# ksahlin/IsoCon

Measured on AMD Instinct MI355X. Metric: read x candidate alignments/sec (NN-graph build, 50k x 2.5kb reads), higher is better.
Workload: dtype u64; 1 GPU; C3: 50000 synthetic CCS reads (50000 unique), ~2500 bp, 10 isoforms, seed 30001; 1-set NN graph; edges=78526, graph_digest=65944c838d76a6c9, parallelism=single GPU

## Files before the change

isocon_amd/csrc/common.hpp:

```cpp
#pragma once
#include <hip/hip_runtime.h>
#include <stdint.h>
#include <string>
#include "../../include/isocon_hip.h"

namespace isocon {

struct DevStore {
    const uint64_t *planes;
    const uint64_t *il;
    const int32_t *lens;
    uint32_t n;
    uint32_t nchunks;
};

struct QMap {
    uint32_t begin, end, stride, block_log2;
    __host__ __device__ __forceinline__ uint32_t block() const { return 1u << block_log2; }
    __host__ __device__ __forceinline__ uint64_t entry(uint32_t s) const
    {
        return (uint64_t)begin + (uint64_t)(s >> block_log2) * stride + (s & (block() - 1u));
    }
    __host__ __device__ __forceinline__ bool slot_of(uint32_t x, uint32_t &s) const
    {
        if (x < begin || x >= end) return false;
        const uint32_t d = x - begin, b = d / stride, r = d - b * stride;
        s = (b << block_log2) + r;
        return r < block();
    }
    __host__ __device__ __forceinline__ bool owns(uint32_t x) const { uint32_t s; return slot_of(x, s); }
    __host__ __device__ __forceinline__ uint32_t count() const
    {
        if (end <= begin) return 0u;
        const uint32_t span = end - begin, full = span / stride, rem = span - full * stride;
        return (full << block_log2) + (rem < block() ? rem : block());
    }
    __host__ __device__ __forceinline__ bool same(const QMap &o) const { return begin == o.begin && end == o.end && stride == o.stride && block_log2 == o.block_log2; }
};

extern thread_local std::string g_last_error;

#define ISO_HIP_CHECK(expr)                                                                    \
    do {                                                                                       \
        hipError_t _e = (expr);                                                                \
        if (_e != hipSuccess) {                                                                \
            g_last_error = std::string(#expr) + ": " + hipGetErrorString(_e);                  \
            return ISOCON_E_HIP;                                                               \
        }                                                                                      \
    } while (0)

__device__ __forceinline__ int32_t wave_min_i32(int32_t v)
{
#pragma unroll
    for (int o = 32; o > 0; o >>= 1) {
        const int32_t w = __shfl_xor(v, o, 64);
        v = w < v ? w : v;
    }
    return v;
}

__device__ __forceinline__ int32_t wave_max_i32(int32_t v)
{
#pragma unroll
    for (int o = 32; o > 0; o >>= 1) {
        const int32_t w = __shfl_xor(v, o, 64);
        v = w > v ? w : v;
    }
    return v;
}

__device__ __forceinline__ unsigned long long block_exscan_1024(unsigned long long s, unsigned long long *wave_sums, unsigned long long *total)
{
    const uint32_t lane = threadIdx.x & 63u, wave = threadIdx.x >> 6;
    unsigned long long inc = s;
#pragma unroll
    for (uint32_t d = 1; d < 64; d <<= 1) {
        const unsigned long long o = __shfl_up(inc, d, 64);
        if (lane >= d) inc += o;
    }
    if (lane == 63) wave_sums[wave] = inc;
    __syncthreads();
    unsigned long long off = inc - s, tot = 0;
    for (uint32_t w = 0; w < 16; ++w) {
        if (w < wave) off += wave_sums[w];
        tot += wave_sums[w];
    }
    *total = tot;
    return off;
}

static constexpr uint32_t SCAN_TILE = 2048;

template <int SHIFT>
__global__ __launch_bounds__(256) void k_scan_tiles(const uint32_t *__restrict__ in, uint32_t n, uint32_t *__restrict__ tmp, unsigned long long *__restrict__ tile_sum)
{
    __shared__ unsigned long long wave_sums[4];
    const uint32_t base = blockIdx.x * SCAN_TILE + threadIdx.x * 8u;
    uint32_t v[8];
#pragma unroll
    for (int j = 0; j < 8; ++j) {
        const uint32_t x = base + j < n ? in[base + j] : 0u;
        v[j] = SHIFT ? (x + (1u << SHIFT) - 1u) >> SHIFT : x;
    }
    uint32_t s = 0;
#pragma unroll
    for (int j = 0; j < 8; ++j) s += v[j];
    const uint32_t lane = threadIdx.x & 63u, wave = threadIdx.x >> 6;
    uint32_t inc = s;
#pragma unroll
    for (uint32_t d = 1; d < 64; d <<= 1) {
        const uint32_t o = __shfl_up(inc, d, 64);
        if (lane >= d) inc += o;
    }
    if (lane == 63) wave_sums[wave] = inc;
    __syncthreads();
    uint32_t off = inc - s;
    for (uint32_t w = 0; w < wave; ++w) off += (uint32_t)wave_sums[w];
#pragma unroll
    for (int j = 0; j < 8; ++j) {
        if (base + j < n) tmp[base + j] = off;
        off += v[j];
    }
    if (threadIdx.x == 255) tile_sum[blockIdx.x] = (unsigned long long)off;
}

template <class OUT>
__global__ __launch_bounds__(256) void k_scan_finish(const uint32_t *__restrict__ tmp, uint32_t n, const unsigned long long *__restrict__ tile_sum, uint32_t n_tiles,
                                                      OUT *__restrict__ out, unsigned long long *__restrict__ total_out)
{
    __shared__ unsigned long long part[4];
    unsigned long long s = 0, all = 0;
    for (uint32_t b = threadIdx.x; b < n_tiles; b += 256u) {
        const unsigned long long t = tile_sum[b];
        if (b < blockIdx.x) s += t;
        all += t;
    }
    const bool last = blockIdx.x + 1 == gridDim.x;
    unsigned long long r = last ? all : s, r2 = s;
#pragma unroll
    for (int o = 32; o > 0; o >>= 1) { r += __shfl_xor(r, o, 64); r2 += __shfl_xor(r2, o, 64); }
    if ((threadIdx.x & 63u) == 0) part[threadIdx.x >> 6] = r2;
    __syncthreads();
    const unsigned long long before = part[0] + part[1] + part[2] + part[3];
    __syncthreads();
    if ((threadIdx.x & 63u) == 0) part[threadIdx.x >> 6] = r;
    __syncthreads();
    const uint32_t base = blockIdx.x * SCAN_TILE + threadIdx.x * 8u;
#pragma unroll
    for (int j = 0; j < 8; ++j)
        if (base + j < n) out[base + j] = (OUT)(before + tmp[base + j]);
    if (last && threadIdx.x == 0) {
        const unsigned long long tot = part[0] + part[1] + part[2] + part[3];
        out[n] = (OUT)tot;
        if (total_out) *total_out = tot;
    }
}

__device__ __forceinline__ int32_t uniform_i32(int32_t v) { return __builtin_amdgcn_readfirstlane(v); }

__device__ __forceinline__ int32_t load_relaxed_agent(const int32_t *p)
{
    return __hip_atomic_load(p, __ATOMIC_RELAXED, __HIP_MEMORY_SCOPE_AGENT);
}

}
```

isocon_amd/csrc/isocon_hip.hip:

```cpp
#include <algorithm>
#include <chrono>
#include <cstdio>
#include <cstdlib>
#include <cstring>
#include <numeric>
#include <string>
#include <memory>
#include <mutex>
#include <thread>
#include <vector>

#include "common.hpp"
#include "ed_band.hpp"
#include "ed_full.hpp"
#include "qgram_mm.hpp"
#include "nn.hpp"
#include "nn_list.hpp"
#include "nn_filter.hpp"
#include "nn_finalize.hpp"
#include "nn_finalize_host.hpp"
#include "partition_host.hpp"
#include "sg.hpp"
#include "msa.hpp"
#include "hw.hpp"
#include "hw_tiles.hpp"
#include "hw_full.hpp"
#include "nw_path.hpp"
#include "ed_lanes.hpp"
#include "ed_bytes.hpp"
#include "nn2_depth.hpp"
#include "readtab.hpp"
#include "edgevar.hpp"
#include "pbound.hpp"

namespace isocon {
thread_local std::string g_last_error;
}

using namespace isocon;

static bool variant_lookup(const char *name, std::string *value)
{
    const char *e = getenv("ISOCON_DEBUG_VARIANT");
    if (!e) return false;
    const size_t ln = strlen(name);
    for (const char *p = e; *p;) {
        const char *q = strchr(p, ',');
        const size_t len = q ? (size_t)(q - p) : strlen(p);
        if (len >= ln && strncmp(p, name, ln) == 0 && (len == ln || p[ln] == '=')) {
            if (value) *value = len > ln ? std::string(p + ln + 1, len - ln - 1) : std::string();
            return true;
        }
        p += len + (q ? 1 : 0);
    }
    return false;
}
static bool variant(const char *name) { return variant_lookup(name, nullptr); }
static const char *variant_value(const char *name)
{
    thread_local std::string ring[8];
    thread_local unsigned at = 0;
    std::string &slot = ring[at++ % 8];
    return variant_lookup(name, &slot) ? slot.c_str() : nullptr;
}

struct BoundTag {
    bool valid = false, has_order = false;
    uint64_t serial = 0;
    QMap map = {0, 0, 0, 0};
    uint32_t depth = 0;
    int32_t kcap = 0;
    unsigned long long lb_total = 0;
};
struct MsaBuilt {
    enum By { NONE, SINGLE, BATCH } by = NONE;
    uint64_t serial = 0;
    uint32_t n_parts = 0, n_rows = 0;
    std::vector<uint32_t> ncols, col_base, first_row;
    std::vector<unsigned long long> m_off;
};
struct HeldHits { uint64_t store_serial = 0; uint64_t rows = 0; };

struct ScratchPool {
    struct Slot { void *p = nullptr; size_t cap = 0; };
    Slot slots[160];
    BoundTag bound_tag;
    HeldHits held_hits;
    MsaBuilt msa;
    void *get(int idx, size_t bytes)
    {
        Slot &s = slots[idx];
        if (bytes == 0) bytes = 16;
        if (s.cap < bytes) {
            if (s.p) (void)hipFree(s.p);
            s.p = nullptr; s.cap = 0;
            const size_t want = bytes + bytes / 8;
            if (hipMalloc(&s.p, want) == hipSuccess) s.cap = want;
            else if (hipMalloc(&s.p, bytes) == hipSuccess) s.cap = bytes;
            else { s.p = nullptr; (void)hipGetLastError(); }
        }
        return s.p;
    }
    void release()
    {
        for (Slot &s : slots) { if (s.p) (void)hipFree(s.p); s.p = nullptr; s.cap = 0; }
        bound_tag = BoundTag();
        held_hits = HeldHits();
        msa = MsaBuilt();
    }
};

enum {
    SLOT_ED_TS = 0, SLOT_ED_IDS, SLOT_ED_K, SLOT_ED_OUT, SLOT_FULL_A, SLOT_FULL_B, SLOT_FULL_K, SLOT_FULL_OUT,
    SLOT_NN_BEST, SLOT_NN_QF, SLOT_NN_TF, SLOT_NN_HITS, SLOT_NN_HITCOUNT, SLOT_NN_STATS, SLOT_NN_TS, SLOT_NN_IDS, SLOT_NN_PLANES2, SLOT_NN_PERM, SLOT_NN_IL, SLOT_NN_IL2, SLOT_NN_HITS2, SLOT_NN_HITCOUNT2, SLOT_NN_QPROF, SLOT_NN_QSUM, SLOT_NN_LB, SLOT_NN_LBROW, SLOT_NN_LBLEN, SLOT_NN_SLOTORDER, SLOT_NN_LBCHUNKS, SLOT_NN_ROWMIN, SLOT_NN_COLMIN, SLOT_NN_SEED_A, SLOT_NN_SEED_B, SLOT_NN_SEED_N, SLOT_NN_LBT, SLOT_NN_LBT_OFF, SLOT_NN_LBT_SLO, SLOT_NN_LBT_LEN, SLOT_NN_LBT_PAD, SLOT_NN_SCORE, SLOT_NN_LDEST, SLOT_NN_FIN_HITS, SLOT_NN_FIN_CNT, SLOT_NN_FIN_START, SLOT_NN_FIN_CUR, SLOT_NN_FIN_NB, SLOT_NN_FIN_LEN2, SLOT_NN_FIN_OUT, SLOT_NN_FIN_FLAG, SLOT_NN_FIN_BEST, SLOT_NN_ACC_HITS, SLOT_NN_LTOT, SLOT_NN_LCHUNKS, SLOT_NN_LIST, SLOT_NN_LPA, SLOT_NN_LPB, SLOT_NN_TEXT2, SLOT_NN_LTASKS, SLOT_NN_RECORD,
    SLOT_NN2_STATE, SLOT_NN2_TPOS, SLOT_NN2_EXC, SLOT_NN2_CTR, SLOT_NN2_PAIRS, SLOT_NN2_WIDE,
    SLOT_SG_PAIRS, SLOT_SG_R, SLOT_SG_TRACE, SLOT_SG_END, SLOT_SG_OPS, SLOT_SG_CNT, SLOT_SG_RES, SLOT_SG_OFF, SLOT_SG_DENSE, SLOT_SG_BOUND, SLOT_SG_AOFF, SLOT_SG_ALNA, SLOT_SG_ALNB,
    SLOT_MSA_IN, SLOT_MSA_OUT, SLOT_MSA_DEG, SLOT_MSA_COUNTS, SLOT_MSA_MAJ, SLOT_MSA_FLAGS, SLOT_MSA_TOT, SLOT_MSA_NCAND, SLOT_MSA_LEN, SLOT_MSA_OFF, SLOT_MSA_PACKED, SLOT_MSA_ROWS, SLOT_MSA_OPS, SLOT_MSA_OPTR, SLOT_MSA_LONGEST, SLOT_MSA_WIDTH, SLOT_MSA_CSLOT, SLOT_MSA_LTOT, SLOT_MSA_WIDE, SLOT_MSA_PROW, SLOT_MSA_PCOL, SLOT_MSA_PPTR, SLOT_MSA_PBYTES, SLOT_MSA_PART, SLOT_MSA_FIRST, SLOT_MSA_LM, SLOT_MSA_SBASE, SLOT_MSA_NCOLS, SLOT_MSA_MOFF, SLOT_MSA_CBASE, SLOT_MSA_CBP, SLOT_MSA_CBC, SLOT_MSA_CBR,
    SLOT_HW_Q, SLOT_HW_T, SLOT_HW_K, SLOT_HW_OUT, SLOT_HW_TRACE, SLOT_HW_CTR, SLOT_HW_TILEQ, SLOT_HW_LANES, SLOT_HW_PQ, SLOT_HW_KEY, SLOT_HW_HIST, SLOT_HW_CURSOR, SLOT_HW_TBASE, SLOT_HW_CLS,
    SLOT_PACK_ASCII, SLOT_PACK_OFF, SLOT_PACK_BAD, SLOT_PACK_HIST, SLOT_PACK_FLAGS, SLOT_EB_A, SLOT_EB_B, SLOT_EB_K, SLOT_EB_OUT, SLOT_EB_ROWS, SLOT_SCAN_TMP, SLOT_SCAN_SUMS,
    SLOT_RT_REF, SLOT_RT_IN, SLOT_RT_OUT,
    SLOT_EV_IN, SLOT_EV_OUT, SLOT_EV_SNIP,
    SLOT_PB_IN, SLOT_PB_OUT,
    SLOT_NWP_Q, SLOT_NWP_T, SLOT_NWP_ED, SLOT_NWP_TOFF, SLOT_NWP_ROFF, SLOT_NWP_REV, SLOT_NWP_RUNS, SLOT_NWP_FOFF, SLOT_NWP_OPS, SLOT_NWP_START, SLOT_NWP_COLS,
    SLOT_COUNT
};
static_assert(SLOT_COUNT <= 160, "ScratchPool::slots too small");

static ScratchPool g_scratch;

static uint64_t g_store_serial = 0;

struct isocon_store {
    uint64_t serial = ++g_store_serial;
    DevStore dev;
    explicit isocon_store(bool private_scratch = false) : own_pool(private_scratch ? new ScratchPool() : nullptr), pool(own_pool ? *own_pool : g_scratch) {}
    std::unique_ptr<ScratchPool> own_pool;
    ScratchPool &pool;
    std::vector<int32_t> lens;
    uint64_t device_bytes = 0;
    uint64_t *d_planes = nullptr;
    char alphabet[4] = {'A', 'C', 'G', 'T'};
    bool acgt = true;
    uint8_t *d_bytes = nullptr;
    uint64_t *d_boff = nullptr;
    uint64_t bytes_base = 0;
    std::vector<uint8_t> exc;
    std::vector<uint32_t> exc_count;
    uint32_t n_exc = 0;
    bool is_exc(uint32_t i) const { return n_exc != 0 && exc[i] != 0; }
    int32_t *d_lens = nullptr;
    int32_t maxlen = 0;
    uint64_t last_host_waits = 0;
};

namespace {

struct PinnedStage {
    void *p = nullptr;
    size_t cap = 0;
    void *get(size_t bytes)
    {
        if (cap < bytes) {
            if (p) (void)hipHostFree(p);
            p = nullptr; cap = 0;
            if (hipHostMalloc(&p, bytes, hipHostMallocDefault) == hipSuccess) cap = bytes;
            else { p = nullptr; (void)hipGetLastError(); }
        }
        return p;
    }
    void release() { if (p) (void)hipHostFree(p); p = nullptr; cap = 0; }
};
static PinnedStage g_stage;
static constexpr size_t kStageBytes = (size_t)32 << 20;
static constexpr uint64_t kPackWaves = (uint64_t)1 << 25;
static constexpr size_t kStageMin = (size_t)32 << 10;

static std::vector<std::pair<const char *, size_t>> g_pinned;
static bool is_pinned(const void *p, size_t bytes)
{
    for (const auto &r : g_pinned)
        if ((const char *)p >= r.first && (const char *)p + bytes <= r.first + r.second) return true;
    return false;
}

static thread_local uint64_t g_host_waits = 0;
static hipError_t memcpy_wait(void *dst, const void *src, size_t bytes, hipMemcpyKind kind) { ++g_host_waits; return hipMemcpy(dst, src, bytes, kind); }
static hipError_t memset_wait(void *dst, int value, size_t bytes) { ++g_host_waits; return hipMemset(dst, value, bytes); }
static hipError_t device_wait() { ++g_host_waits; return hipDeviceSynchronize(); }

static hipError_t copy_d2h(void *dst, const void *dsrc, size_t bytes)
{
    if (bytes < kStageMin || is_pinned(dst, bytes)) return memcpy_wait(dst, dsrc, bytes, hipMemcpyDeviceToHost);
    char *st = static_cast<char *>(g_stage.get(kStageBytes));
    if (!st) return memcpy_wait(dst, dsrc, bytes, hipMemcpyDeviceToHost);
    for (size_t off = 0; off < bytes; off += kStageBytes) {
        const size_t len = std::min(kStageBytes, bytes - off);
        const hipError_t e = memcpy_wait(st, static_cast<const char *>(dsrc) + off, len, hipMemcpyDeviceToHost);
        if (e != hipSuccess) return e;
        memcpy(static_cast<char *>(dst) + off, st, len);
    }
    return hipSuccess;
}

static hipError_t copy_h2d(void *ddst, const void *src, size_t bytes)
{
    if (bytes < kStageMin || is_pinned(src, bytes)) return memcpy_wait(ddst, src, bytes, hipMemcpyHostToDevice);
    char *st = static_cast<char *>(g_stage.get(kStageBytes));
    if (!st) return memcpy_wait(ddst, src, bytes, hipMemcpyHostToDevice);
    for (size_t off = 0; off < bytes; off += kStageBytes) {
        const size_t len = std::min(kStageBytes, bytes - off);
        memcpy(st, static_cast<const char *>(src) + off, len);
        const hipError_t e = memcpy_wait(static_cast<char *>(ddst) + off, st, len, hipMemcpyHostToDevice);
        if (e != hipSuccess) return e;
    }
    return hipSuccess;
}

struct SideUpload {
    hipStream_t stream = nullptr;
    hipEvent_t before = nullptr, done = nullptr;
    PinnedStage pinned;
    bool in_flight = false;
    bool ready()
    {
        if (stream) return true;
        if (hipStreamCreateWithFlags(&stream, hipStreamNonBlocking) != hipSuccess) { stream = nullptr; (void)hipGetLastError(); return false; }
        if (hipEventCreateWithFlags(&before, hipEventDisableTiming) != hipSuccess || hipEventCreateWithFlags(&done, hipEventDisableTiming) != hipSuccess) {
            (void)hipGetLastError();
            release();
            return false;
        }
        return true;
    }
    void settle()
    {
        if (!in_flight) return;
        if (hipEventQuery(done) != hipSuccess || hipStreamQuery(stream) != hipSuccess) { (void)hipGetLastError(); ++g_host_waits; (void)hipStreamSynchronize(stream); }
        in_flight = false;
    }
    void release()
    {
        if (stream) { (void)hipStreamSynchronize(stream); (void)hipStreamDestroy(stream); }
        if (before) (void)hipEventDestroy(before);
        if (done) (void)hipEventDestroy(done);
        stream = nullptr; before = done = nullptr; in_flight = false;
        pinned.release();
    }
};
static SideUpload g_side;

struct DevBuf {
    void *p = nullptr;
    ScratchPool *pool = nullptr;
    int slot = -1;
    DevBuf() {}
    DevBuf(ScratchPool *pl, int sl) : pool(pl), slot(sl) {}
    DevBuf(const DevBuf &) = delete;
    DevBuf &operator=(const DevBuf &) = delete;
    ~DevBuf() { if (p && !pool) (void)hipFree(p); }
    template <class T> T *as() { return static_cast<T *>(p); }
    int alloc(size_t bytes)
    {
        if (pool) {
            p = pool->get(slot, bytes);
            if (!p) { g_last_error = "hipMalloc(scratch slot " + std::to_string(slot) + ", " + std::to_string(bytes) + " B) failed"; return ISOCON_E_HIP; }
            return ISOCON_OK;
        }
        if (p) { (void)hipFree(p); p = nullptr; }
        ISO_HIP_CHECK(hipMalloc(&p, bytes ? bytes : 16));
        return ISOCON_OK;
    }
};

template <int SHIFT, class OUT>
static int device_exscan(ScratchPool *pl, const uint32_t *d_in, uint32_t n, OUT *d_out)
{
    DevBuf d_tmp(pl, SLOT_SCAN_TMP), d_sums(pl, SLOT_SCAN_SUMS);
    const uint32_t tiles = std::max<uint32_t>(1, (n + SCAN_TILE - 1) / SCAN_TILE);
    int rc;
    if ((rc = d_tmp.alloc((size_t)std::max<uint32_t>(n, 1) * 4)) || (rc = d_sums.alloc((size_t)tiles * 8))) return rc;
    hipLaunchKernelGGL((k_scan_tiles<SHIFT>), dim3(tiles), dim3(256), 0, 0, d_in, n, d_tmp.as<uint32_t>(), d_sums.as<unsigned long long>());
    hipLaunchKernelGGL((k_scan_finish<OUT>), dim3(tiles), dim3(256), 0, 0, d_tmp.as<uint32_t>(), n, d_sums.as<unsigned long long>(), tiles, d_out, (unsigned long long *)nullptr);
    ISO_HIP_CHECK(hipGetLastError());
    return ISOCON_OK;
}

struct EventPool {
    std::mutex mu;
    std::vector<hipEvent_t> idle;
    hipEvent_t get()
    {
        {
            std::lock_guard<std::mutex> g(mu);
            if (!idle.empty()) { hipEvent_t e = idle.back(); idle.pop_back(); return e; }
        }
        hipEvent_t e = nullptr;
        if (hipEventCreate(&e) != hipSuccess) { (void)hipGetLastError(); return nullptr; }
        return e;
    }
    void put(hipEvent_t e)
    {
        if (!e) return;
        std::lock_guard<std::mutex> g(mu);
        idle.push_back(e);
    }
    void release()
    {
        std::lock_guard<std::mutex> g(mu);
        for (hipEvent_t e : idle) (void)hipEventDestroy(e);
        idle.clear();
    }
};
static EventPool g_events;

struct EventTimer {
    struct Interval { hipEvent_t e0, em, e1; float *acc, *marked_acc; };
    std::vector<Interval> pending;
    hipEvent_t e0 = nullptr, em = nullptr;
    float total = 0.f;
    float marked_total = 0.f;
    const bool sync_phases = variant("nn_sync_phases");
    EventTimer() {}
    EventTimer(const EventTimer &) = delete;
    EventTimer &operator=(const EventTimer &) = delete;
    ~EventTimer()
    {
        g_events.put(e0); g_events.put(em);
        for (const Interval &iv : pending) { g_events.put(iv.e0); g_events.put(iv.em); g_events.put(iv.e1); }
    }
    void start()
    {
        g_events.put(em); em = nullptr;
        if (!e0) e0 = g_events.get();
        if (e0) (void)hipEventRecord(e0, 0);
    }
    void mark()
    {
        if (!e0) return;
        if (!em) em = g_events.get();
        if (em) (void)hipEventRecord(em, 0);
    }
    void stop_later(float *acc, float *marked_acc = nullptr)
    {
        if (!e0) return;
        hipEvent_t e1 = g_events.get();
        if (!e1) { g_events.put(e0); g_events.put(em); e0 = em = nullptr; return; }
        (void)hipEventRecord(e1, 0);
        pending.push_back(Interval{e0, em, e1, acc, marked_acc});
        e0 = em = nullptr;
        if (sync_phases) resolve(true);
    }
    void resolve(bool wait_counts = false)
    {
        if (pending.empty()) return;
        hipEvent_t last = pending.back().e1;
        if (wait_counts || hipEventQuery(last) != hipSuccess) { (void)hipGetLastError(); ++g_host_waits; (void)hipEventSynchronize(last); }
        for (const Interval &iv : pending) {
            float ms = 0.f, part = 0.f;
            if (hipEventElapsedTime(&ms, iv.e0, iv.e1) != hipSuccess) { (void)hipGetLastError(); ms = 0.f; }
            total += ms;
            if (iv.acc) *iv.acc += ms;
            if (iv.em) {
                if (hipEventElapsedTime(&part, iv.em, iv.e1) != hipSuccess) { (void)hipGetLastError(); part = 0.f; }
                if (iv.marked_acc) *iv.marked_acc += part; else marked_total += part;
            }
            g_events.put(iv.e0); g_events.put(iv.em); g_events.put(iv.e1);
        }
        pending.clear();
    }
    float stop()
    {
        float ms = 0.f;
        stop_later(&ms);
        resolve(true);
        return ms;
    }
};

struct PackMap { uint8_t sym[4]; };

__global__ __launch_bounds__(256) void k_byte_histogram(const uint8_t *__restrict__ ascii, uint64_t total, unsigned long long *__restrict__ hist)
{
    __shared__ uint32_t h[256];
    h[threadIdx.x] = 0;
    __syncthreads();
    for (uint64_t i = (uint64_t)blockIdx.x * 256 + threadIdx.x; i < total; i += (uint64_t)gridDim.x * 256) atomicAdd(&h[ascii[i]], 1u);
    __syncthreads();
    if (h[threadIdx.x]) atomicAdd(hist + threadIdx.x, (unsigned long long)h[threadIdx.x]);
}

__global__ __launch_bounds__(256) void k_pack_planes(const uint8_t *__restrict__ ascii, const uint64_t *__restrict__ offsets, uint64_t base, uint32_t n,
                                                      uint32_t nchunks, uint64_t *__restrict__ planes, unsigned long long *__restrict__ first_bad, PackMap map,
                                                      uint32_t fold, uint64_t w0)
{
    const uint64_t w = w0 + (uint64_t)blockIdx.x * 4 + (threadIdx.x >> 6);
    if (w >= (uint64_t)nchunks * n) return;
    const uint32_t lane = threadIdx.x & 63;
    const uint32_t chunk = (uint32_t)(w / n), seq = (uint32_t)(w % n);
    const uint64_t off = offsets[seq] - base, len = offsets[seq + 1] - offsets[seq];
    const uint64_t pos = (uint64_t)chunk * 64 + lane;
    int cd = 0;
    bool bad = false;
    if (pos < len) {
        uint8_t ch = ascii[off + pos];
        if (fold && ch >= 'a' && ch <= 'z') ch = (uint8_t)(ch - 32);
        cd = ch == map.sym[0] ? 0 : ch == map.sym[1] ? 1 : ch == map.sym[2] ? 2 : ch == map.sym[3] ? 3 : -1;
        bad = cd < 0 && !fold;
    }
    const unsigned long long lo = __ballot(!bad && (cd & 1)), hi = __ballot(!bad && (cd & 2)), bm = __ballot(bad);
    if (lane == 0) {
        planes[((size_t)chunk * n + seq) * 2] = lo;
        planes[((size_t)chunk * n + seq) * 2 + 1] = hi;
        if (bm) atomicMin(first_bad, ((unsigned long long)seq << 32) | ((unsigned long long)chunk * 64 + (unsigned long long)(__ffsll((long long)bm) - 1)));
    }
}

}

extern "C" {

const char *isocon_strerror(int status)
{
    switch (status) {
    case ISOCON_OK: return "ok";
    case ISOCON_E_ARG: return "bad argument";
    case ISOCON_E_ALPHABET: return "sequence contains a symbol outside ACGT";
    case ISOCON_E_HIP: return "HIP runtime error";
    case ISOCON_E_CAPACITY: return "output buffer too small";
    case ISOCON_E_NODEVICE: return "no usable GPU";
    case ISOCON_E_UNSUPPORTED: return "unsupported request";
    default: return "unknown status";
    }
}

const char *isocon_last_error(void) { return g_last_error.c_str(); }
// ... 413 lines not shown
            if (!lanes_p.empty()) {
                const size_t np = lanes_p.size();
                std::vector<uint32_t> la(np), lb2(np);
                std::vector<int32_t> lk(np), res(np, -1);
                for (size_t i = 0; i < np; ++i) {
                    const uint64_t p = lanes_p[i];
                    la[i] = a[p]; lb2[i] = b[p];
                    const int32_t kr = k ? k[p] : -1;
                    lk[i] = kr < 0 ? kcap : std::min(kr, kcap);
                }
                DevBuf d_a(&st->pool, SLOT_ED_TS), d_b(&st->pool, SLOT_ED_IDS), d_k(&st->pool, SLOT_ED_K), d_out(&st->pool, SLOT_ED_OUT);
                int rc;
                if ((rc = d_a.alloc(np * 4)) || (rc = d_b.alloc(np * 4)) || (rc = d_k.alloc(np * 4)) || (rc = d_out.alloc(np * 4))) return rc;
                ISO_HIP_CHECK(copy_h2d(d_a.p, la.data(), np * 4));
                ISO_HIP_CHECK(copy_h2d(d_b.p, lb2.data(), np * 4));
                ISO_HIP_CHECK(copy_h2d(d_k.p, lk.data(), np * 4));
                NNParams none;
                memset(&none, 0, sizeof(none));
                tm.start();
                hipLaunchKernelGGL(k_ed_lanes<false>, dim3((unsigned)((np + 255) / 256)), dim3(256), 0, 0, st->dev, none, d_a.as<uint32_t>(), d_b.as<uint32_t>(),
                                   d_k.as<int32_t>(), (uint64_t)np, d_out.as<int32_t>());
                ISO_HIP_CHECK(hipGetLastError());
                tm.stop();
                ISO_HIP_CHECK(copy_d2h(res.data(), d_out.p, np * 4));
                for (size_t i = 0; i < np; ++i) {
                    const uint64_t p = lanes_p[i];
                    const int32_t kr = k ? k[p] : -1;
                    if (res[i] >= 0) out_ed[p] = res[i];
                    else if (kr >= 0 && kr <= kcap) out_ed[p] = -1;
                    else next.push_back(p);
                }
            }
            todo.swap(tiles_p);
        }
        for (int round = 0; round < 2 && !todo.empty(); ++round) {
            std::vector<uint32_t> ts, ids;
            std::vector<int32_t> ks;
            std::vector<uint64_t> slot_pair;
            size_t i = 0;
            while (i < todo.size()) {
                size_t j = i;
                const uint32_t s0 = sh(todo[i]);
                const size_t lim = round == 0 ? 64 : 1;
                while (j < todo.size() && j - i < lim && sh(todo[j]) == s0) ++j;
                ts.push_back(s0);
                for (size_t l = 0; l < 64; ++l) {
                    if (i + l < j) {
                        const uint64_t p = todo[i + l];
                        ids.push_back(ln(p));
                        const int32_t kr = k ? k[p] : -1;
                        ks.push_back(kr < 0 ? kcap : std::min(kr, kcap));
                        slot_pair.push_back(p);
                    } else {
                        ids.push_back(0xffffffffu);
                        ks.push_back(-1);
                        slot_pair.push_back(~(uint64_t)0);
                    }
                }
                i = j;
            }
            std::vector<int32_t> res;
            int rc = run_band_stage(W, st, st->dev, ts, ids, ks, res, tm);
            if (rc) return rc;
            std::vector<uint64_t> retry;
            for (size_t sidx = 0; sidx < slot_pair.size(); ++sidx) {
                const uint64_t p = slot_pair[sidx];
                if (p == ~(uint64_t)0) continue;
                const int32_t r = res[sidx];
                const int32_t kr = k ? k[p] : -1;
                if (r >= 0) out_ed[p] = r;
                else if (r == -2) retry.push_back(p);
                else if (kr >= 0 && kr <= kcap) out_ed[p] = -1;
                else next.push_back(p);
            }
            todo.swap(retry);
        }
        if (!todo.empty()) { g_last_error = "internal: single-lane tile undetermined"; return ISOCON_E_HIP; }
        pending.swap(next);
    }
    if (full_pairs) *full_pairs = pending.size();
    if (!pending.empty()) {
        std::vector<uint32_t> fa, fb;
        std::vector<int32_t> fk, res;
        for (uint64_t p : pending) { fa.push_back(a[p]); fb.push_back(b[p]); fk.push_back(k ? k[p] : -1); }
        int rc = run_full(st, fa, fb, fk, res, tm);
        if (rc) return rc;
        for (size_t i = 0; i < pending.size(); ++i) out_ed[pending[i]] = res[i];
    }
    if (kernel_ms) *kernel_ms = tm.total;
    return ISOCON_OK;
}

}

__global__ __launch_bounds__(256) void k_store_digest(const uint64_t *__restrict__ planes, size_t n_words, const int32_t *__restrict__ lens, uint32_t n,
                                                      unsigned long long *__restrict__ out)
{
    unsigned long long acc = 0;
    const size_t stride = (size_t)gridDim.x * blockDim.x;
    for (size_t i = (size_t)blockIdx.x * blockDim.x + threadIdx.x; i < n_words + n; i += stride) {
        unsigned long long v = i < n_words ? planes[i] : (unsigned long long)(uint32_t)lens[i - n_words];
        v ^= (unsigned long long)i * 0xD6E8FEB86659FD93ull;
        v ^= v >> 32; v *= 0x9E3779B97F4A7C15ull; v ^= v >> 29; v *= 0xBF58476D1CE4E5B9ull; v ^= v >> 32;
        acc += v;
    }
    for (int o = 32; o > 0; o >>= 1) acc += __shfl_xor(acc, o, 64);
    if ((threadIdx.x & 63) == 0 && acc) atomicAdd(out, acc);
}

extern "C" int isocon_store_digest(const isocon_store *s, uint64_t *out)
{
    if (!s || !out) return ISOCON_E_ARG;
    DevBuf d_acc;
    int rc;
    if ((rc = d_acc.alloc(8))) return rc;
    ISO_HIP_CHECK(hipMemset(d_acc.p, 0, 8));
    const size_t n_words = (size_t)s->dev.nchunks * std::max<uint32_t>(s->dev.n, 1) * 2;
    hipLaunchKernelGGL(k_store_digest, dim3(1024), dim3(256), 0, 0, s->d_planes, n_words, s->d_lens, s->dev.n, d_acc.as<unsigned long long>());
    ISO_HIP_CHECK(hipGetLastError());
    ISO_HIP_CHECK(hipMemcpy(out, d_acc.p, 8, hipMemcpyDeviceToHost));
    return ISOCON_OK;
}

extern "C" int isocon_ed_pairs(isocon_store *s, const uint32_t *a, const uint32_t *b, const int32_t *k, uint64_t n_pairs,
                               int32_t *out_ed, float *kernel_ms)
{
    if (!s || (n_pairs && (!a || !b || !out_ed))) return ISOCON_E_ARG;
    if (kernel_ms) *kernel_ms = 0.f;
    if (!n_pairs) return ISOCON_OK;
    return ed_pairs_impl(s, a, b, k, n_pairs, out_ed, kernel_ms, nullptr, false);
}

extern "C" int isocon_qgram_params(int32_t *out)
{
    if (out) { out[0] = QG_Q; out[1] = QG_B0; out[2] = QG_B1; out[3] = QG_CAP; }
    return QM_K;
}

namespace isocon {
int qgram_bounds_for_pairs(isocon_store *s, const uint32_t *a, const uint32_t *b, uint64_t n_pairs, int32_t *out_bound, float *kernel_ms)
{
    const uint32_t n = s->dev.n;
    const uint32_t n_pad = std::max<uint32_t>(QM_TILE, ((n + QM_TILE - 1) / QM_TILE) * QM_TILE);
    DevBuf d_prof(&s->pool, SLOT_NN_QPROF), d_sum(&s->pool, SLOT_NN_QSUM), d_a(&s->pool, SLOT_ED_TS), d_b(&s->pool, SLOT_ED_IDS), d_out(&s->pool, SLOT_ED_OUT);
    int rc;
    if ((rc = d_prof.alloc((size_t)n_pad * (QM_K / 2))) || (rc = d_sum.alloc((size_t)n * 4)) || (rc = d_a.alloc(n_pairs * 4)) || (rc = d_b.alloc(n_pairs * 4)) ||
        (rc = d_out.alloc(n_pairs * 4)))
        return rc;
    s->pool.bound_tag.valid = false;
    ISO_HIP_CHECK(copy_h2d(d_a.p, a, n_pairs * 4));
    ISO_HIP_CHECK(copy_h2d(d_b.p, b, n_pairs * 4));
    EventTimer tm;
    tm.start();
    hipLaunchKernelGGL(k_qgram_profile4, dim3((n + QP_SEQS - 1) / QP_SEQS), dim3(256), 0, 0, s->dev, d_prof.as<uint8_t>(), d_sum.as<uint32_t>(), n_pad);
    ISO_HIP_CHECK(hipGetLastError());
    for (uint64_t at = 0; at < n_pairs; at += (uint64_t)1 << 24) {
        const uint64_t cnt = std::min<uint64_t>((uint64_t)1 << 24, n_pairs - at);
        hipLaunchKernelGGL(k_qgram_lb_pairs, dim3((unsigned)((cnt + 3) / 4)), dim3(256), 0, 0, d_prof.as<uint8_t>(), d_sum.as<uint32_t>(), n_pad, d_a.as<uint32_t>() + at,
                           d_b.as<uint32_t>() + at, cnt, d_out.as<int32_t>() + at);
        ISO_HIP_CHECK(hipGetLastError());
    }
    const float ms = tm.stop();
    if (kernel_ms) *kernel_ms = ms;
    ISO_HIP_CHECK(copy_d2h(out_bound, d_out.p, n_pairs * 4));
    return ISOCON_OK;
}
}

extern "C" int isocon_qgram_bound_pairs(isocon_store *s, const uint32_t *a, const uint32_t *b, uint64_t n_pairs, int32_t *out_bound)
{
    if (!s || (n_pairs && (!a || !b || !out_bound))) return ISOCON_E_ARG;
    if (!n_pairs) return ISOCON_OK;
    if (s->n_exc) { g_last_error = "q-gram bounds are defined on the 2-bit planes: the set holds more than four distinct symbols"; return ISOCON_E_ALPHABET; }
    const uint32_t n = s->dev.n;
    for (uint64_t i = 0; i < n_pairs; ++i)
        if (a[i] >= n || b[i] >= n) { g_last_error = "pair index out of range"; return ISOCON_E_ARG; }
    return qgram_bounds_for_pairs(s, a, b, n_pairs, out_bound, nullptr);
}

extern "C" int isocon_block_bound_pairs(isocon_store *s, const uint32_t *owner, const uint32_t *partner, uint64_t n_pairs, int32_t probe_stride, int32_t *out_count)
{
    if (probe_stride != 4 && probe_stride != 2) return ISOCON_E_ARG;
    if (!s || (n_pairs && (!owner || !partner || !out_count))) return ISOCON_E_ARG;
    if (!n_pairs) return ISOCON_OK;
    if (s->n_exc) { g_last_error = "block bounds are defined on the 2-bit planes: the set holds more than four distinct symbols"; return ISOCON_E_ALPHABET; }
    const uint32_t n = s->dev.n;
    if (n_pairs >= ((uint64_t)1 << 31)) return ISOCON_E_ARG;
    for (uint64_t i = 0; i < n_pairs; ++i)
        if (owner[i] >= n || partner[i] >= n) { g_last_error = "pair index out of range"; return ISOCON_E_ARG; }
    const uint32_t stride = nnf_text2_stride(s->maxlen);
    DevBuf d_text(&s->pool, SLOT_NN_TEXT2), d_a(&s->pool, SLOT_ED_TS), d_b(&s->pool, SLOT_ED_IDS), d_out(&s->pool, SLOT_ED_OUT);
    int rc;
    if ((rc = d_text.alloc((size_t)n * stride * 4)) || (rc = d_a.alloc(n_pairs * 4)) || (rc = d_b.alloc(n_pairs * 4)) || (rc = d_out.alloc(n_pairs * 4))) return rc;
    ISO_HIP_CHECK(copy_h2d(d_a.p, owner, n_pairs * 4));
    ISO_HIP_CHECK(copy_h2d(d_b.p, partner, n_pairs * 4));
    hipLaunchKernelGGL(k_build_text2, dim3(n), dim3(256), 0, 0, s->dev, d_text.as<uint32_t>(), stride);
    hipLaunchKernelGGL(k_nn_block_count_pairs, dim3((unsigned)n_pairs), dim3(256), 0, 0, d_text.as<uint32_t>(), stride, s->dev.lens, d_a.as<uint32_t>(), d_b.as<uint32_t>(), d_out.as<int32_t>(), probe_stride);
    ISO_HIP_CHECK(hipGetLastError());
    ISO_HIP_CHECK(copy_d2h(out_count, d_out.p, n_pairs * 4));
    return ISOCON_OK;
}

extern "C" int isocon_block_filter_chunks(isocon_store *s, const int32_t *thr, uint32_t n_chunks, const uint32_t *owner, const uint8_t *narrow, const uint64_t *chunk_ptr,
                                          const uint32_t *words, int32_t kcap, uint32_t list_min, int32_t second_pass, uint32_t *out_slot, uint32_t *out_count,
                                          uint64_t *out_begin, uint64_t chunks_cap, uint32_t *out_list, uint64_t list_cap, uint32_t *out_pa, uint32_t *out_pb, uint64_t pairs_cap,
                                          uint64_t *out_counters)
{
    if (!s || !out_counters || (second_pass != 0 && second_pass != 1) || list_min == 0) return ISOCON_E_ARG;
    for (int i = 0; i < 9; ++i) out_counters[i] = 0;
    if (!n_chunks) return ISOCON_OK;
    if (!thr || !owner || !narrow || !chunk_ptr || !words || !out_slot || !out_count || !out_begin || !out_list || !out_pa || !out_pb) return ISOCON_E_ARG;
    if (s->n_exc) { g_last_error = "block bounds are defined on the 2-bit planes: the set holds more than four distinct symbols"; return ISOCON_E_ALPHABET; }
    const uint32_t n = s->dev.n;
    if (n >= (1u << 30) || s->maxlen >= 16384) return ISOCON_E_ARG;
    for (uint32_t i = 0; i < n; ++i)
        if (thr[i] < 0 || thr[i] > 64) { g_last_error = "threshold outside 0 .. 64"; return ISOCON_E_ARG; }
    static_assert(NN_LIST_CHUNK + 63 <= NN_STAGE, "a chunk fits the filter's staging buffer");
    if (chunk_ptr[0] != 0) return ISOCON_E_ARG;
    uint32_t n_narrow = 0;
    for (uint32_t c = 0; c < n_chunks; ++c) {
        if (owner[c] >= n || narrow[c] > 1) { g_last_error = "chunk owner out of range"; return ISOCON_E_ARG; }
        if (chunk_ptr[c + 1] <= chunk_ptr[c] || chunk_ptr[c + 1] - chunk_ptr[c] > NN_LIST_CHUNK + 63) { g_last_error = "chunk count outside 1 .. NN_LIST_CHUNK + 63"; return ISOCON_E_ARG; }
        n_narrow += narrow[c];
    }
    const uint64_t total = chunk_ptr[n_chunks];
    for (uint64_t i = 0; i < total; ++i)
        if ((words[i] & 0x3fffffffu) >= n) { g_last_error = "partner index out of range"; return ISOCON_E_ARG; }
    if (chunks_cap < n_chunks || list_cap < total || pairs_cap < total) { g_last_error = "an output capacity below the worst case (every pair kept)"; return ISOCON_E_ARG; }
    const uint64_t cap_in = n_chunks, cap_out = n_chunks;
    const uint64_t tasks_cap = second_pass ? 2 * cap_in + total / 64 + 1 : 0;
    std::vector<uint32_t> meta((size_t)n + NN_META_PAD, 0u);
    for (uint32_t i = 0; i < n; ++i) meta[i] = ((uint32_t)s->lens[i] & 0x3fffu) | ((uint32_t)thr[i] << 14);
    std::vector<NNChunk> chunks(2 * (size_t)cap_in);
    NNPlanTotals tot;
    memset(&tot, 0, sizeof(tot));
    for (uint32_t c = 0; c < n_chunks; ++c) {
        NNChunk ch; ch.slot = owner[c]; ch.count = (uint32_t)(chunk_ptr[c + 1] - chunk_ptr[c]); ch.begin = chunk_ptr[c];
        chunks[narrow[c] ? cap_in + tot.n_chunks_narrow++ : tot.n_chunks++] = ch;
    }
    const uint32_t stride = nnf_text2_stride(s->maxlen);
    DevBuf d_text(&s->pool, SLOT_NN_TEXT2), d_meta(&s->pool, SLOT_NN_LDEST), d_tot(&s->pool, SLOT_NN_LTOT), d_chunks(&s->pool, SLOT_NN_LCHUNKS), d_list(&s->pool, SLOT_NN_LIST),
        d_pa(&s->pool, SLOT_NN_LPA), d_pb(&s->pool, SLOT_NN_LPB), d_tasks(&s->pool, SLOT_NN_LTASKS);
    int rc;
    if ((rc = d_text.alloc((size_t)n * stride * 4)) || (rc = d_meta.alloc(meta.size() * 4)) || (rc = d_tot.alloc(sizeof(NNPlanTotals))) ||
        (rc = d_chunks.alloc((size_t)(2 * cap_in + 2 * cap_out) * sizeof(NNChunk))) || (rc = d_list.alloc((size_t)total * 4)) || (rc = d_pa.alloc((size_t)total * 4)) ||
        (rc = d_pb.alloc((size_t)total * 4)) || (rc = d_tasks.alloc((size_t)std::max<uint64_t>(tasks_cap, 1) * sizeof(NNFTask))))
        return rc;
    ISO_HIP_CHECK(copy_h2d(d_meta.p, meta.data(), meta.size() * 4));
    ISO_HIP_CHECK(copy_h2d(d_tot.p, &tot, sizeof(tot)));
    ISO_HIP_CHECK(copy_h2d(d_chunks.p, chunks.data(), chunks.size() * sizeof(NNChunk)));
    ISO_HIP_CHECK(copy_h2d(d_list.p, words, (size_t)total * 4));
    NNChunk *left = d_chunks.as<NNChunk>() + 2 * cap_in;
    hipLaunchKernelGGL(k_build_text2, dim3(n), dim3(256), 0, 0, s->dev, d_text.as<uint32_t>(), stride);
    ISO_HIP_CHECK(hipGetLastError());
    ISO_HIP_CHECK(nnf_launch_filter(d_text.as<uint32_t>(), stride, s->dev.lens, d_meta.as<uint32_t>(), kcap, d_list.as<uint32_t>(), d_chunks.as<NNChunk>(), cap_in, left, cap_out,
                                    d_pa.as<uint32_t>(), d_pb.as<uint32_t>(), total, d_tot.as<NNPlanTotals>(), list_min, second_pass ? d_tasks.as<NNFTask>() : (NNFTask *)nullptr,
                                    tasks_cap));
    ISO_HIP_CHECK(memcpy_wait(&tot, d_tot.p, sizeof(tot), hipMemcpyDeviceToHost));
    const uint64_t counters[9] = {tot.f_chunks, tot.f_chunks_narrow, tot.n_small, tot.f_rejected, tot.f_rejected2, tot.f_listed, tot.f_narrow_listed, tot.f_tasks, tot.overflow};
    for (int i = 0; i < 9; ++i) out_counters[i] = counters[i];
    if (tot.overflow || tot.f_chunks > cap_in - n_narrow || tot.f_chunks_narrow > n_narrow || tot.n_small > total) { g_last_error = "the block filter left more than it was given"; return ISOCON_E_HIP; }
    std::vector<NNChunk> out((size_t)(tot.f_chunks + tot.f_chunks_narrow));
    if (tot.f_chunks) ISO_HIP_CHECK(copy_d2h(out.data(), left, (size_t)tot.f_chunks * sizeof(NNChunk)));
    if (tot.f_chunks_narrow) ISO_HIP_CHECK(copy_d2h(out.data() + tot.f_chunks, left + cap_out, (size_t)tot.f_chunks_narrow * sizeof(NNChunk)));
    for (size_t i = 0; i < out.size(); ++i) { out_slot[i] = out[i].slot; out_count[i] = out[i].count; out_begin[i] = out[i].begin; }
    ISO_HIP_CHECK(copy_d2h(out_list, d_list.p, (size_t)total * 4));
    if (tot.n_small) {
        ISO_HIP_CHECK(copy_d2h(out_pa, d_pa.p, (size_t)tot.n_small * 4));
        ISO_HIP_CHECK(copy_d2h(out_pb, d_pb.p, (size_t)tot.n_small * 4));
    }
    return ISOCON_OK;
}

#include "nn_context.inc"
#include "nn_bounds.inc"
#include "nn_lists.inc"
#include "nn_main.inc"
#include "nn_wide.inc"
#include "nn_images.inc"
#include "nn_entry.inc"
#include "nn2_depth.inc"
#include "sg_host.inc"
#include "msa_host.inc"
#include "hw_host.inc"
#include "hw_full_host.inc"
#include "nw_path_host.inc"
#include "hw_path_host.inc"
#include "readtab_host.inc"
#include "edgevar_host.inc"
#include "pbound_host.inc"

extern "C" int isocon_partition_ids(uint32_t n, const int32_t *degree, uint64_t n_edges, const uint32_t *edge_a, const uint32_t *edge_b,
                                    const uint32_t *rank, int32_t nbr_tiebreak, uint32_t *out_centre, int64_t *out_weight,
                                    uint64_t *out_member_ptr, uint32_t *out_members, uint32_t *n_parts)
{
    if (!out_member_ptr || !n_parts || (n && (!degree || !rank || !out_centre || !out_weight || !out_members)) || (n_edges && (!edge_a || !edge_b))) return ISOCON_E_ARG;
    return partition_ids_impl(n, degree, n_edges, edge_a, edge_b, rank, nbr_tiebreak, out_centre, out_weight, out_member_ptr, out_members, n_parts);
}
```

isocon_amd/csrc/nn_bounds.inc:

```

namespace {

int NNContext::build_bounds(const QMap &Q, int32_t kcap, NNParams &P, bool want_seeds)
{
    const uint32_t q_begin = Q.begin, q_end = Q.end;
    P.lb = nullptr;
    P.lb_row = nullptr;
    P.slot_order = nullptr;
    if (variant("nn_no_qgram") || n < 2 || n >= (1u << 30) || q_begin >= q_end) return ISOCON_OK;
    if (!want_seeds && st->pool.bound_tag.valid && st->pool.bound_tag.serial == st->serial && st->pool.bound_tag.map.same(Q) &&
        st->pool.bound_tag.depth == depth && st->pool.bound_tag.kcap == kcap) {
        P.lb = static_cast<const uint8_t *>(st->pool.slots[SLOT_NN_LB].p);
        P.lb_row = static_cast<const unsigned long long *>(st->pool.slots[SLOT_NN_LBROW].p);
        if (st->pool.bound_tag.has_order && use_slot_order(Q.count())) P.slot_order = static_cast<const uint32_t *>(st->pool.slots[SLOT_NN_SLOTORDER].p);
        lb_total = st->pool.bound_tag.lb_total;
        return ISOCON_OK;
    }
    st->pool.bound_tag.valid = false;
    const uint32_t nq = Q.count();
    const std::vector<int32_t> &lens = st->lens;
    const uint32_t n_pad = std::max<uint32_t>(QM_TILE, ((n + QM_TILE - 1) / QM_TILE) * QM_TILE);
    const size_t prof_bytes = (size_t)n_pad * (QM_K / 2);
    d_qprof.pool = d_qsum.pool = &st->pool;
    d_qprof.slot = SLOT_NN_QPROF; d_qsum.slot = SLOT_NN_QSUM;
    HostClock bclk;
    {
        size_t free_b = 0;
        if (!free_mem(free_b) || prof_bytes > free_b / 2 + st->pool.slots[SLOT_NN_QPROF].cap) return ISOCON_OK;
        if (d_qprof.alloc(prof_bytes) || d_qsum.alloc((size_t)n * 4)) return ISOCON_OK;
    }
    bclk.lap("bounds: memory check + profile buffers");
    const bool side = !variant("nn_sync_uploads") && g_side.ready() && hipEventRecord(g_side.before, 0) == hipSuccess;
    tm.start();
    hipLaunchKernelGGL(k_qgram_profile4, dim3((n + QP_SEQS - 1) / QP_SEQS), dim3(256), 0, 0, st->dev, d_qprof.as<uint8_t>(), d_qsum.as<uint32_t>(), n_pad);
    ISO_HIP_CHECK(hipGetLastError());
    struct StopTimer { NNContext &c; bool armed = true; ~StopTimer() { if (armed) c.tm.stop_later(&c.stats.bound_kernel_ms); } } stop_timer{*this};
    std::vector<unsigned long long> &off = lb_off_host;
    std::vector<uint32_t> &rlen = lb_len_host;
    off.assign(nq, 0);
    rlen.assign(nq, 0);
    unsigned long long total = 0, sum_rlen = 0;
    uint64_t hi = 0;
    const uint32_t nrb = (nq + QM_TILE - 1) / QM_TILE;
    std::vector<uint64_t> rb_lo(nrb, ~(uint64_t)0), rb_hi(nrb, 0);
    for (uint32_t s = 0; s < nq; ++s) {
        const uint64_t q = Q.entry(s);
        if (hi < q + 1) hi = q + 1;
        while (hi < n && lens[hi] - lens[q] <= kcap) ++hi;
        uint64_t len = hi - q - 1;
        if (len > depth) len = depth;
        const uint64_t pal = (q + 1) & ~(uint64_t)15;
        off[s] = total + (q + 1 - pal);
        rlen[s] = (uint32_t)len;
        sum_rlen += len;
        if (len) {
            total += ((q + 1 + len + 15) & ~(uint64_t)15) - pal;
            rb_lo[s / QM_TILE] = std::min<uint64_t>(rb_lo[s / QM_TILE], q + 1);
            rb_hi[s / QM_TILE] = std::max<uint64_t>(rb_hi[s / QM_TILE], q + len);
        }
    }
    if (total == 0) return ISOCON_OK;
    bclk.lap("bounds: profile launch + rows (host)");
    const unsigned long long totalT = sum_rlen + 30ull * n;
    bclk.lap("bounds: transposed rows (host)");
    size_t free_b = 0;
    const size_t need = (size_t)total + (size_t)totalT + prof_bytes + (size_t)n * 24 + (size_t)nq * 12;
    if (!free_mem(free_b) || need > free_b / 2 + st->pool.slots[SLOT_NN_LB].cap + st->pool.slots[SLOT_NN_QPROF].cap) return ISOCON_OK;
    bclk.lap("bounds: memory check 2");
    std::vector<uint2> tiles;
    for (uint32_t g = 0; g * 4 < nrb; ++g) {
        uint64_t jmin = ~(uint64_t)0, jmax = 0;
        bool any = false;
        for (uint32_t I = g * 4; I < std::min(nrb, g * 4 + 4); ++I)
            if (rb_lo[I] != ~(uint64_t)0) { any = true; jmin = std::min(jmin, rb_lo[I] / QM_TILE); jmax = std::max(jmax, rb_hi[I] / QM_TILE); }
        if (!any) continue;
        for (uint64_t j0 = jmin; j0 <= jmax; j0 += 8)
            for (uint32_t ri = 0; ri < 4; ++ri)
                for (uint32_t cj = 0; cj < 8; ++cj) {
                    const uint32_t I = g * 4 + ri;
                    const uint64_t J = j0 + cj;
                    const bool have = I < nrb && rb_lo[I] != ~(uint64_t)0 && J >= rb_lo[I] / QM_TILE && J <= rb_hi[I] / QM_TILE;
                    tiles.push_back(have ? make_uint2(I, (uint32_t)J) : make_uint2(0xffffffffu, 0xffffffffu));
                }
    }
    while (tiles.size() % 256) tiles.push_back(make_uint2(0xffffffffu, 0xffffffffu));
    if (tiles.size() > 0x7fffffffull) return ISOCON_OK;
    bclk.lap("bounds: tile table (host)");
    d_lb.pool = d_lbrow.pool = d_lblen.pool = &st->pool;
    d_lb.slot = SLOT_NN_LB; d_lbrow.slot = SLOT_NN_LBROW; d_lblen.slot = SLOT_NN_LBLEN;
    int rc;
    if ((rc = d_lb.alloc((size_t)total + 16)) ||
        (rc = d_lbrow.alloc((size_t)nq * 8)) || (rc = d_lblen.alloc((size_t)nq * 4)))
        return ISOCON_OK;
    d_lbt.pool = d_offT.pool = d_sloT.pool = d_lenT.pool = d_score.pool = &st->pool;
    d_lbt.slot = SLOT_NN_LBT; d_offT.slot = SLOT_NN_LBT_OFF; d_sloT.slot = SLOT_NN_LBT_SLO; d_lenT.slot = SLOT_NN_LBT_LEN; d_score.slot = SLOT_NN_SCORE;
    DevBuf d_padT(&st->pool, SLOT_NN_LBT_PAD);
    if (d_lbt.alloc((size_t)totalT + 16) || d_offT.alloc(((size_t)n + 1) * 8) || d_sloT.alloc((size_t)n * 4) || d_lenT.alloc((size_t)n * 4) || d_score.alloc((size_t)n * 4) ||
        d_padT.alloc((size_t)n * 4))
        return ISOCON_OK;
    ISO_HIP_CHECK(hipMemsetAsync(d_score.p, 0, (size_t)n * 4, 0));
    d_chunks.pool = &st->pool;
    d_chunks.slot = SLOT_NN_LBCHUNKS;
    if (d_chunks.alloc(tiles.size() * sizeof(uint2))) return ISOCON_OK;
    const size_t b_tiles = (tiles.size() * sizeof(uint2) + 15) & ~(size_t)15, b_off = ((size_t)nq * 8 + 15) & ~(size_t)15, b_len = (size_t)nq * 4;
    char *pin = nullptr;
    if (side) { g_side.settle(); pin = static_cast<char *>(g_side.pinned.get(b_tiles + b_off + b_len)); }
    if (pin) {
        memcpy(pin, tiles.data(), tiles.size() * sizeof(uint2));
        memcpy(pin + b_tiles, off.data(), (size_t)nq * 8);
        memcpy(pin + b_tiles + b_off, rlen.data(), (size_t)nq * 4);
        g_side.in_flight = true;
        ISO_HIP_CHECK(hipStreamWaitEvent(g_side.stream, g_side.before, 0));
        ISO_HIP_CHECK(hipMemcpyAsync(d_chunks.p, pin, tiles.size() * sizeof(uint2), hipMemcpyHostToDevice, g_side.stream));
        ISO_HIP_CHECK(hipMemcpyAsync(d_lbrow.p, pin + b_tiles, (size_t)nq * 8, hipMemcpyHostToDevice, g_side.stream));
        ISO_HIP_CHECK(hipMemcpyAsync(d_lblen.p, pin + b_tiles + b_off, (size_t)nq * 4, hipMemcpyHostToDevice, g_side.stream));
        ISO_HIP_CHECK(hipEventRecord(g_side.done, g_side.stream));
        ISO_HIP_CHECK(hipStreamWaitEvent(0, g_side.done, 0));
    } else {
        ISO_HIP_CHECK(copy_h2d(d_chunks.p, tiles.data(), tiles.size() * sizeof(uint2)));
        ISO_HIP_CHECK(copy_h2d(d_lbrow.p, off.data(), (size_t)nq * 8));
        ISO_HIP_CHECK(copy_h2d(d_lblen.p, rlen.data(), (size_t)nq * 4));
    }
    hipLaunchKernelGGL(k_lbt_rows, dim3((n + 255) / 256), dim3(256), 0, 0, Q, nq, d_lblen.as<uint32_t>(), n, d_sloT.as<uint32_t>(), d_lenT.as<uint32_t>(), d_padT.as<uint32_t>());
    if ((rc = device_exscan<0, unsigned long long>(&st->pool, d_padT.as<uint32_t>(), n, d_offT.as<unsigned long long>()))) return ISOCON_OK;
    hipLaunchKernelGGL(k_lbt_offsets, dim3((n + 255) / 256), dim3(256), 0, 0, n, d_sloT.as<uint32_t>(), d_offT.as<unsigned long long>());
    ISO_HIP_CHECK(hipGetLastError());
    bclk.lap("bounds: alloc + uploads");
    if (use_slot_order(nq)) {
        std::vector<uint32_t> order(nq);
        std::iota(order.begin(), order.end(), 0u);
        std::stable_sort(order.begin(), order.end(), [&](uint32_t x, uint32_t y) { return rlen[x] > rlen[y]; });
        d_order.pool = &st->pool;
        d_order.slot = SLOT_NN_SLOTORDER;
        if (d_order.alloc((size_t)nq * 4)) return ISOCON_OK;
        ISO_HIP_CHECK(copy_h2d(d_order.p, order.data(), (size_t)nq * 4));
    }
    unsigned long long *rowmin = nullptr, *colmin = nullptr;
    if (want_seeds) {
        d_rowmin.pool = d_colmin.pool = d_seed_a.pool = d_seed_b.pool = &st->pool;
        d_rowmin.slot = SLOT_NN_ROWMIN; d_colmin.slot = SLOT_NN_COLMIN; d_seed_a.slot = SLOT_NN_SEED_A; d_seed_b.slot = SLOT_NN_SEED_B;
        if (!(d_rowmin.alloc((size_t)nq * 8 * QM_SEEDS) || d_colmin.alloc((size_t)n_pad * 8 * QM_SEEDS) || d_seed_a.alloc((size_t)n * 8 * QM_SEEDS) || d_seed_b.alloc((size_t)n * 8 * QM_SEEDS))) {
            ISO_HIP_CHECK(hipMemsetAsync(d_rowmin.p, 0xff, (size_t)nq * 8 * QM_SEEDS, 0));
            ISO_HIP_CHECK(hipMemsetAsync(d_colmin.p, 0xff, (size_t)n_pad * 8 * QM_SEEDS, 0));
            rowmin = d_rowmin.as<unsigned long long>();
            colmin = d_colmin.as<unsigned long long>();
        }
    }
    bclk.lap("bounds: slot order + seed buffers");
    static bool lds_attr_set = false;
    if (!lds_attr_set) {
        ISO_HIP_CHECK(hipFuncSetAttribute((const void *)k_qgram_mm, hipFuncAttributeMaxDynamicSharedMemorySize, (int)QM_LDS_BYTES));
        lds_attr_set = true;
    }
    tm.mark();
    hipLaunchKernelGGL(k_qgram_mm, dim3((unsigned)tiles.size()), dim3(512), QM_LDS_BYTES, 0, d_qprof.as<uint8_t>(), d_qsum.as<uint32_t>(), n, n_pad,
                       d_chunks.as<uint2>(), d_lbrow.as<unsigned long long>(), d_lblen.as<uint32_t>(), d_lb.as<uint8_t>(), Q, nq,
                       d_qf.as<uint8_t>(), d_tf.as<uint8_t>(), rowmin, colmin, d_offT.as<unsigned long long>(), d_sloT.as<uint32_t>(), d_lenT.as<uint32_t>(),
                       d_lbt.as<uint8_t>(), d_score.as<uint32_t>());
    ISO_HIP_CHECK(hipGetLastError());
    stop_timer.armed = false;
    tm.stop_later(&stats.bound_kernel_ms, &stats.mm_kernel_ms);
    bclk.lap("bounds: k_qgram_mm (enqueued)");
#ifdef ISOCON_QM_TIMELINE
    {
        const size_t nt = std::min<size_t>(tiles.size(), 16384);
        std::vector<unsigned long long> tl(nt * 8);
        ISO_HIP_CHECK(hipMemcpyFromSymbol(tl.data(), HIP_SYMBOL(g_qm_timeline), nt * 64));
        double sum[5] = {0, 0, 0, 0, 0};
        unsigned long long t_min = ~0ull, t_max = 0;
        size_t cnt = 0;
        for (size_t b = 0; b < nt; ++b) {
            if (tiles[b].x == 0xffffffffu) continue;
            const unsigned long long *t = tl.data() + b * 8;
            for (int k = 0; k < 5; ++k) sum[k] += (double)(t[k + 1] - t[k]);
            t_min = std::min(t_min, t[0]); t_max = std::max(t_max, t[5]);
            ++cnt;
        }
        fprintf(stderr, "[qm timeline] %zu tiles: prologue %.2f us, K loop %.2f us, E1 %.2f us, E2 %.2f us, E3 %.2f us per tile; first start to last end %.3f ms\n", cnt,
                sum[0] / cnt / 100.0, sum[1] / cnt / 100.0, sum[2] / cnt / 100.0, sum[3] / cnt / 100.0, sum[4] / cnt / 100.0, (double)(t_max - t_min) / 1e5);
    }
#endif
    for (const uint2 &t : tiles) stats.bound_tiles += t.x != 0xffffffffu;
    P.lb = d_lb.as<uint8_t>();
    P.lb_row = d_lbrow.as<unsigned long long>();
    if (use_slot_order(nq)) P.slot_order = d_order.as<uint32_t>();
    seeds_ready = rowmin != nullptr;
    seed_nq = nq;
    lb_total = total;
    st->pool.bound_tag.valid = true;
    st->pool.bound_tag.lb_total = total;
    st->pool.bound_tag.has_order = use_slot_order(nq);
    st->pool.bound_tag.serial = st->serial;
    st->pool.bound_tag.map = Q; st->pool.bound_tag.depth = depth; st->pool.bound_tag.kcap = kcap;
    return ISOCON_OK;
}

int NNContext::run_bound_seeds(const QMap &Q)
{
    if (!seeds_ready) return ISOCON_OK;
    tm.start();
    const uint64_t np = (uint64_t)2 * QM_SEEDS * n;
    const uint32_t ranks = std::max<uint32_t>(1u, Q.stride >> Q.block_log2);
    uint32_t col_classes = QM_SEEDS;
    while (col_classes > 1 && col_classes * ranks > (uint32_t)QM_SEEDS) col_classes >>= 1;
    if (const char *e = variant_value("nn_seed_classes")) { const int v = atoi(e); if (v == 1 || v == 2 || v == QM_SEEDS) col_classes = (uint32_t)v; }
    DevBuf d_seed_n(&st->pool, SLOT_NN_SEED_N);
    int rc;
    if ((rc = d_seed_n.alloc(8))) return rc;
    ISO_HIP_CHECK(hipMemsetAsync(d_seed_n.p, 0, 8, 0));
    ISO_HIP_CHECK(hipMemsetAsync(d_seed_a.p, 0xff, (size_t)np * 4, 0));
    ISO_HIP_CHECK(hipMemsetAsync(d_seed_b.p, 0xff, (size_t)np * 4, 0));
    hipLaunchKernelGGL(k_qgram_seed_pairs, dim3((n + 255) / 256), dim3(256), 0, 0, d_rowmin.as<unsigned long long>(), d_colmin.as<unsigned long long>(),
                       n, Q, seed_nq, col_classes, d_seed_a.as<uint32_t>(), d_seed_b.as<uint32_t>(), d_seed_n.as<unsigned long long>());
    ISO_HIP_CHECK(hipGetLastError());
    hipLaunchKernelGGL(k_ed_lanes<true>, dim3((unsigned)((np + 255) / 256)), dim3(256), 0, 0, st->dev, params(63), d_seed_a.as<uint32_t>(), d_seed_b.as<uint32_t>(),
                       (const int32_t *)nullptr, np, (int32_t *)nullptr);
    ISO_HIP_CHECK(hipGetLastError());
    tm.stop_later(&stats.seed_kernel_ms);
    return ISOCON_OK;
}

}
```

isocon_amd/csrc/nn_context.inc:

```

namespace {

struct HostClock {
    std::chrono::steady_clock::time_point t0 = std::chrono::steady_clock::now();
    const bool on = getenv("ISOCON_DEBUG") != nullptr;
    void lap(const char *what)
    {
        if (!on) return;
        const auto t1 = std::chrono::steady_clock::now();
        fprintf(stderr, "[isocon] %-28s %8.2f ms\n", what, std::chrono::duration<double, std::milli>(t1 - t0).count());
        t0 = t1;
    }
};

struct NNContext {
    isocon_store *st = nullptr;
    uint32_t n = 0;
    std::vector<uint8_t> qflag, tflag;
    bool two_set = false;
    bool depth_binds = false;
    std::vector<uint8_t> wide_mask;
    int32_t min_d = 1;
    uint32_t depth = 0x7fffffffu;
    DevBuf d_best, d_qf, d_tf, d_hits, d_hit_count, d_stats;
    DevBuf d_text;
    uint32_t text_stride = 0;
    bool text_ready = false;
    DevBuf d_qprof, d_qsum, d_lb, d_lbrow, d_lblen;
    DevBuf d_chunks;
    DevBuf d_lbt, d_offT, d_sloT, d_lenT, d_score;
    DevBuf d_order;
    DevBuf d_rowmin, d_colmin, d_seed_a, d_seed_b;
    uint64_t hits_cap = 0;
    std::vector<int32_t> best;
    std::vector<int32_t> hits;
    isocon_nn_stats stats;
    EventTimer tm;

    size_t free_bytes = 0;
    int free_state = 0;
    bool free_mem(size_t &free_b)
    {
        if (free_state == 0) {
            size_t total_b = 0;
            free_state = hipMemGetInfo(&free_bytes, &total_b) == hipSuccess ? 1 : -1;
            if (free_state < 0) (void)hipGetLastError();
        }
        free_b = free_bytes;
        return free_state > 0;
    }
    bool text_room = false;
    bool text_affordable()
    {
        if (text_ready || text_room) return true;
        text_stride = (uint32_t)NN_TEXT_PAD_FRONT + (uint32_t)((st->maxlen + 7) / 8) + (uint32_t)NN_TEXT_PAD_BACK;
        size_t free_b = 0;
        if (!free_mem(free_b) || (size_t)n * text_stride * 4 > free_b / 2) return false;
        d_text.pool = &st->pool;
        d_text.slot = SLOT_NN_IL;
        if (d_text.alloc((size_t)std::max<uint32_t>(n, 1) * text_stride * 4) != ISOCON_OK) return false;
        text_room = true;
        return true;
    }
    bool build_text()
    {
        if (text_ready) return true;
        if (!text_room) return false;
        hipLaunchKernelGGL(k_build_nibble_text, dim3(std::max<uint32_t>(n, 1)), dim3(256), 0, 0, st->dev, d_text.as<uint32_t>(), text_stride);
        if (hipGetLastError() != hipSuccess) { g_last_error = "k_build_nibble_text: launch failed"; return false; }
        text_ready = true;
        return true;
    }
    bool ensure_text() { return text_affordable() && build_text(); }
    DevBuf d_text2;
    uint32_t text2_stride = 0;
    bool text2_ready = false;
    bool ensure_text2()
    {
        if (text2_ready) return true;
        text2_stride = nnf_text2_stride(st->maxlen);
        size_t free_b = 0;
        if (!free_mem(free_b) || (size_t)n * text2_stride * 4 > free_b / 2 + st->pool.slots[SLOT_NN_TEXT2].cap) return false;
        d_text2.pool = &st->pool;
        d_text2.slot = SLOT_NN_TEXT2;
        if (d_text2.alloc((size_t)std::max<uint32_t>(n, 1) * text2_stride * 4) != ISOCON_OK) return false;
        hipLaunchKernelGGL(k_build_text2, dim3(std::max<uint32_t>(n, 1)), dim3(256), 0, 0, st->dev, d_text2.as<uint32_t>(), text2_stride);
        if (hipGetLastError() != hipSuccess) return false;
        text2_ready = true;
        return true;
    }
    static bool use_slot_order(uint32_t nq)
    {
        if (const char *e = variant_value("nn_order")) return atoi(e) != 0;
        return nq <= 16384;
    }
    int build_bounds(const QMap &Q, int32_t kcap, NNParams &P, bool want_seeds = false);
    std::vector<unsigned long long> lb_off_host;
    std::vector<uint32_t> lb_len_host;
    unsigned long long lb_total = 0;
    bool seeds_ready = false;
    uint32_t seed_nq = 0;
    int run_bound_seeds(const QMap &Q);
    DevBuf d_ltot, d_lchunks, d_list, d_lpa, d_lpb, d_lmeta, d_ltasks;
    struct ListPlan {
        bool listed = false;
        unsigned long long n_chunks = 0, n_chunks_narrow = 0, n_small = 0;
        unsigned long long conv_a = 0, conv_b = 0, conv_pairs = 0;
        NNChunk *a = nullptr, *b = nullptr, *sorted_a = nullptr, *sorted_b = nullptr;
    };
    int plan_lists(const QMap &Q, uint32_t nq, const NNParams &PR, ListPlan &L);
    NNParams params(int32_t kcap)
    {
        NNParams P;
        P.best = d_best.as<int32_t>();
        P.qflag = d_qf.as<uint8_t>();
        P.tflag = d_tf.as<uint8_t>();
        P.hits = d_hits.as<int32_t>();
        P.hit_count = d_hit_count.as<unsigned long long>();
        P.stats = d_stats.as<unsigned long long>();
        P.hits_cap = hits_cap;
        P.kcap = kcap;
        P.min_d = image_pass ? 0 : min_d;
        P.depth = depth;
        P.fixed = fixed ? 1 : 0;
        P.q_list = nullptr;
        P.own = QMap{0u, n, 1u, 0u};
        P.lb = nullptr;
        P.lb_row = nullptr;
        P.slot_order = nullptr;
        P.wg_base = 0;
        P.chunks = nullptr;
        P.list = nullptr;
        return P;
    }

    bool fill_best = false;
    bool best_on_host = true;
    int upload_best()
    {
        if (fill_best) {
            fill_best = false;
            if (n) ISO_HIP_CHECK(hipMemsetD32Async((hipDeviceptr_t)d_best.p, NN_INF, n, 0));
            return ISOCON_OK;
        }
        ISO_HIP_CHECK(copy_h2d(d_best.p, best.data(), (size_t)n * 4));
        return ISOCON_OK;
    }
    int download_best() { ISO_HIP_CHECK(copy_d2h(best.data(), d_best.p, (size_t)n * 4)); best_on_host = true; return ISOCON_OK; }
    static constexpr uint32_t N_COUNTERS = 2 * (NN_COUNTER_SLOTS * 4 + 1);
    int reset_counters()
    {
        ISO_HIP_CHECK(hipMemsetAsync(d_hit_count.p, 0, 8, 0));
        ISO_HIP_CHECK(hipMemsetAsync(d_stats.p, 0, N_COUNTERS * 8, 0));
        return ISOCON_OK;
    }
    void add_counters(const unsigned long long *sc2)
    {
        for (int blk = 0; blk < 2; ++blk) {
            const unsigned long long *sc = sc2 + blk * (NN_COUNTER_SLOTS * 4 + 1);
            stats.pairs_prefiltered += sc[NN_COUNTER_SLOTS * 4];
            for (int i = 0; i < NN_COUNTER_SLOTS; ++i) {
                stats.pairs_evaluated += sc[i * 4 + 0];
                stats.cells_columns += sc[i * 4 + 1];
                stats.tiles += sc[i * 4 + 2];
                stats.live_columns += sc[i * 4 + 3];
                if (blk == 1) stats.narrow_columns += sc[i * 4 + 1];
            }
        }
    }
    bool keep_dev = false;
    const int32_t *dev_hits = nullptr;
    uint64_t dev_hit_count = 0;
    int collect(std::vector<int32_t> &out, uint64_t *needed, bool filter = false, bool to_device = false)
    {
        unsigned long long cnt = 0;
        ISO_HIP_CHECK(memcpy_wait(&cnt, d_hit_count.p, 8, hipMemcpyDeviceToHost));
        unsigned long long sc2[N_COUNTERS];
        ISO_HIP_CHECK(memcpy_wait(sc2, d_stats.p, sizeof(sc2), hipMemcpyDeviceToHost));
        add_counters(sc2);
        if (needed) *needed = cnt;
        if (cnt > hits_cap) return ISOCON_E_CAPACITY;
        stats.hits += cnt;
        const void *src = d_hits.p;
        if (filter && cnt > 4096 && dev_hit_count == 0) {
            DevBuf d_h2(&st->pool, SLOT_NN_HITS2), d_c2(&st->pool, SLOT_NN_HITCOUNT2);
            int rc;
            if ((rc = d_h2.alloc((size_t)cnt * 12)) || (rc = d_c2.alloc(8))) return rc;
            ISO_HIP_CHECK(hipMemsetAsync(d_c2.p, 0, 8, 0));
            const unsigned blocks = (unsigned)std::min<unsigned long long>((cnt + 255) / 256, 4096);
            hipLaunchKernelGGL(k_filter_hits, dim3(blocks), dim3(256), 0, 0, d_hits.as<int32_t>(), cnt, d_best.as<int32_t>(), d_h2.as<int32_t>(),
                               d_c2.as<unsigned long long>());
            ISO_HIP_CHECK(hipGetLastError());
            ISO_HIP_CHECK(memcpy_wait(&cnt, d_c2.p, 8, hipMemcpyDeviceToHost));
            src = d_h2.p;
        }
        if (to_device) {
            dev_hits = static_cast<const int32_t *>(src);
            dev_hit_count = cnt;
            return ISOCON_OK;
        }
        const size_t base = out.size();
        out.resize(base + (size_t)cnt * 3);
        if (cnt) ISO_HIP_CHECK(copy_d2h(out.data() + base, src, (size_t)cnt * 12));
        return ISOCON_OK;
    }
    bool csr_follows = false;
    bool wide_needed = false;
    int collect_record(uint64_t *needed)
    {
        DevBuf d_rec(&st->pool, SLOT_NN_RECORD);
        int rc;
        if ((rc = d_rec.alloc((2 + N_COUNTERS) * 8))) return rc;
        ISO_HIP_CHECK(hipMemsetAsync(d_rec.p, 0, 16, 0));
        hipLaunchKernelGGL(k_nn_step_record, dim3(std::max<uint32_t>(1, (n + 255) / 256)), dim3(256), 0, 0, d_hit_count.as<unsigned long long>(), d_stats.as<unsigned long long>(),
                           N_COUNTERS, d_best.as<int32_t>(), d_qf.as<uint8_t>(), st->dev.lens, n, d_rec.as<unsigned long long>());
        ISO_HIP_CHECK(hipGetLastError());
        unsigned long long rec[2 + N_COUNTERS];
        ISO_HIP_CHECK(memcpy_wait(rec, d_rec.p, sizeof(rec), hipMemcpyDeviceToHost));
        add_counters(rec + 2);
        if (needed) *needed = rec[0];
        if (rec[0] > hits_cap) return ISOCON_E_CAPACITY;
        stats.hits += rec[0];
        wide_needed = rec[1] != 0;
        dev_hits = d_hits.as<int32_t>();
        dev_hit_count = rec[0];
        best_on_host = false;
        return ISOCON_OK;
    }
    int pull_dev_hits()
    {
        if (dev_hit_count) {
            const size_t base = hits.size();
            hits.resize(base + (size_t)dev_hit_count * 3);
            ISO_HIP_CHECK(copy_d2h(hits.data() + base, dev_hits, (size_t)dev_hit_count * 12));
        }
        dev_hits = nullptr;
        dev_hit_count = 0;
        return ISOCON_OK;
    }
    bool is_exc(uint32_t q) const { return st->n_exc != 0 && st->exc[q] != 0; }
    bool mask_exc = true;
    bool image_pass = false;
    bool fixed = false;
    bool dev_excluded(uint32_t q) const { return mask_exc && is_exc(q); }
    bool flags_dirty = false;
    bool roles_uniform = false;
    int upload_flags(bool fresh = false)
    {
        if (!n) return ISOCON_OK;
        if (fresh && roles_uniform && !st->n_exc) {
            ISO_HIP_CHECK(hipMemsetAsync(d_qf.p, 1, n, 0));
            ISO_HIP_CHECK(hipMemsetAsync(d_tf.p, 1, n, 0));
            return ISOCON_OK;
        }
        if (!st->n_exc || !mask_exc) {
            ISO_HIP_CHECK(copy_h2d(d_qf.p, qflag.data(), n));
            ISO_HIP_CHECK(copy_h2d(d_tf.p, tflag.data(), n));
            return ISOCON_OK;
        }
        std::vector<uint8_t> q2(qflag), t2(tflag);
        for (uint32_t i = 0; i < n; ++i)
            if (st->exc[i]) q2[i] = t2[i] = 0;
        ISO_HIP_CHECK(copy_h2d(d_qf.p, q2.data(), n));
        ISO_HIP_CHECK(copy_h2d(d_tf.p, t2.data(), n));
        return ISOCON_OK;
    }
    bool admissible(uint32_t x, uint32_t y) const { return qflag[x] && tflag[y]; }
    void apply(uint32_t s, uint32_t p, int32_t d)
    {
        if (d < min_d) return;
        const int32_t ls = st->lens[s], lp = st->lens[p];
        if (admissible(s, p) && d <= ls && d <= best[s]) { if (!fixed) best[s] = d; hits.push_back((int32_t)s); hits.push_back((int32_t)p); hits.push_back(d); }
        if (admissible(p, s) && d <= lp && d <= best[p]) { if (!fixed) best[p] = d; hits.push_back((int32_t)p); hits.push_back((int32_t)s); hits.push_back(d); }
    }
};

template <int W>
int launch_nn_tiles(NNContext &C, const std::vector<uint32_t> &ts, const std::vector<uint32_t> &ids, int32_t kcap, float *ms_out)
{
    const size_t nt = ts.size();
    if (!nt) return ISOCON_OK;
    DevBuf d_ts(&C.st->pool, SLOT_NN_TS), d_ids(&C.st->pool, SLOT_NN_IDS);
    int rc;
    if ((rc = d_ts.alloc(nt * 4)) || (rc = d_ids.alloc(nt * 64 * 4))) return rc;
    ISO_HIP_CHECK(copy_h2d(d_ts.p, ts.data(), nt * 4));
    ISO_HIP_CHECK(copy_h2d(d_ids.p, ids.data(), nt * 64 * 4));
    C.tm.start();
    hipLaunchKernelGGL(k_nn_tiles<W>, dim3((unsigned)((nt + 3) / 4)), dim3(256), 0, 0, C.st->dev, C.params(kcap),
                       d_ts.as<uint32_t>(), d_ids.as<uint32_t>(), (uint32_t)nt);
    ISO_HIP_CHECK(hipGetLastError());
    const float ms = C.tm.stop();
    if (ms_out) *ms_out += ms;
    return ISOCON_OK;
}

int run_nn_tiles(int W, NNContext &C, const std::vector<uint32_t> &ts, const std::vector<uint32_t> &ids, float *ms_out)
{
    switch (W) {
    case 1: return launch_nn_tiles<1>(C, ts, ids, 63, ms_out);
    case 2: return launch_nn_tiles<2>(C, ts, ids, 127, ms_out);
    case 4: return launch_nn_tiles<4>(C, ts, ids, 255, ms_out);
    case 8: return launch_nn_tiles<8>(C, ts, ids, 511, ms_out);
    default: return ISOCON_E_ARG;
    }
}

void push_tiles(std::vector<uint32_t> &ts, std::vector<uint32_t> &ids, uint32_t shared, const std::vector<uint32_t> &lanes)
{
    for (size_t i = 0; i < lanes.size(); i += 64) {
        ts.push_back(shared);
        for (size_t l = 0; l < 64; ++l) ids.push_back(i + l < lanes.size() ? lanes[i + l] : 0xffffffffu);
    }
}

void length_window(const std::vector<int32_t> &lens, uint32_t x, int32_t w, uint32_t &lo, uint32_t &hi)
{
    const int32_t L = lens[x];
    lo = (uint32_t)(std::lower_bound(lens.begin(), lens.end(), L - w) - lens.begin());
    hi = (uint32_t)(std::upper_bound(lens.begin(), lens.end(), L + w) - lens.begin());
}

int nn_setup(NNContext &C, isocon_store *s, const uint8_t *is_converged, const uint8_t *is_target, uint64_t depth,
             const int32_t *best_in, bool depth_walk = false)
{
    C.st = s;
    C.n = s->dev.n;
    C.d_best.pool = C.d_qf.pool = C.d_tf.pool = C.d_hits.pool = C.d_hit_count.pool = C.d_stats.pool = &s->pool;
    C.d_best.slot = SLOT_NN_BEST; C.d_qf.slot = SLOT_NN_QF; C.d_tf.slot = SLOT_NN_TF; C.d_hits.slot = SLOT_NN_HITS;
    C.d_hit_count.slot = SLOT_NN_HITCOUNT; C.d_stats.slot = SLOT_NN_STATS;
    const uint32_t n = C.n;
    for (uint32_t i = 1; i < n; ++i)
        if (s->lens[i] < s->lens[i - 1]) { g_last_error = "nearest-neighbour entry points need a length-sorted store"; return ISOCON_E_ARG; }
    C.two_set = is_target != nullptr;
    C.roles_uniform = !C.two_set && !is_converged;
    C.min_d = C.two_set ? 0 : 1;
    C.qflag.assign(n, 0);
    C.tflag.assign(n, 0);
    uint64_t n_targets = 0;
    for (uint32_t i = 0; i < n; ++i) {
        if (C.two_set) { C.tflag[i] = is_target[i] ? 1 : 0; C.qflag[i] = is_target[i] ? 0 : 1; n_targets += C.tflag[i]; }
        else { C.tflag[i] = 1; C.qflag[i] = (is_converged && is_converged[i]) ? 0 : 1; }
    }
    if (C.two_set) {
        C.depth_binds = depth < n_targets;
        if (C.depth_binds && !depth_walk) { g_last_error = "2-set search with neighbor_search_depth < number of targets is not supported"; return ISOCON_E_UNSUPPORTED; }
        C.depth = 0x7fffffffu;
    } else {
        if (depth == 0) { g_last_error = "neighbor_search_depth must be >= 1"; return ISOCON_E_ARG; }
        C.depth = depth > 0x7fffffffull ? 0x7fffffffu : (uint32_t)depth;
    }
    HostClock clk;
    C.best.assign(std::max<uint32_t>(n, 1), NN_INF);
    if (best_in) std::copy(best_in, best_in + n, C.best.begin());
    clk.lap("setup: host arrays");
    memset(&C.stats, 0, sizeof(C.stats));
    C.hits_cap = ((uint64_t)1 << 20) + (uint64_t)n * 48;
    if (const char *e = variant_value("hits_cap")) C.hits_cap = std::max<uint64_t>(16, strtoull(e, nullptr, 10));
    int rc;
    if ((rc = C.d_best.alloc((size_t)std::max<uint32_t>(n, 1) * 4)) || (rc = C.d_qf.alloc(std::max<uint32_t>(n, 1))) ||
        (rc = C.d_tf.alloc(std::max<uint32_t>(n, 1))) || (rc = C.d_hits.alloc(C.hits_cap * 12)) || (rc = C.d_hit_count.alloc(8)) ||
        (rc = C.d_stats.alloc(2 * (NN_COUNTER_SLOTS * 4 + 1) * 8)))
        return rc;
    clk.lap("setup: pool");
    if ((rc = C.upload_flags(true))) return rc;
    clk.lap("setup: role flags");
    return ISOCON_OK;
}

bool qmap_args_ok(uint32_t q_stride, uint32_t q_block) { return q_stride != 0 && q_block != 0 && (q_block & (q_block - 1)) == 0 && q_block <= q_stride; }
QMap qmap_of(uint32_t q_begin, uint32_t q_end, uint32_t q_stride, uint32_t q_block)
{
    uint32_t lg = 0;
    while ((1u << lg) < q_block) ++lg;
    return QMap{q_begin, q_end, q_stride, lg};
}

}
```

isocon_amd/csrc/nn_entry.inc:

```

namespace {

int nn_phase_a(NNContext &C, const QMap &Q, bool allow_regroup = false, bool do_seed = true, bool do_main = true, bool seeded_before = false)
{
    if (!C.st->n_exc || !do_main) return nn_phase_a_planes(C, Q, allow_regroup, do_seed, do_main, seeded_before);
    return nn_phase_a_images(C, Q, allow_regroup, do_seed, seeded_before);
}

int nn_phase_b(NNContext &C, const QMap &Q)
{
    return C.st->n_exc ? nn_phase_b_images(C, Q) : nn_phase_b_planes(C, Q);
}


struct WaitScope {
    isocon_store *s;
    explicit WaitScope(isocon_store *st) : s(st) { g_host_waits = 0; }
    ~WaitScope() { if (s) s->last_host_waits = g_host_waits; }
};

int nn_finalize_device_core(ScratchPool *pl, uint32_t n, const int32_t *d_best, const int32_t *best_host, const int32_t *d_hits, uint64_t n_hits,
                            int32_t *out_best, uint64_t *out_row_ptr, uint32_t *out_cols, uint64_t cols_cap, uint64_t *n_cols_needed)
{
    DevBuf d_cnt(pl, SLOT_NN_FIN_CNT), d_start(pl, SLOT_NN_FIN_START), d_cur(pl, SLOT_NN_FIN_CUR), d_nb(pl, SLOT_NN_FIN_NB),
// ... 42 lines not shown
        if (total) ISO_HIP_CHECK(copy_d2h(out_cols, d_cols, (size_t)total * 4));
        if (!best_src) {
            best_tmp.resize(std::max<uint32_t>(n, 1));
            if (n) ISO_HIP_CHECK(copy_d2h(best_tmp.data(), d_best_out, (size_t)n * 4));
            best_src = best_tmp.data();
        }
    }
    for (uint32_t i = 0; i < n; ++i) out_best[i] = out_row_ptr[i + 1] > out_row_ptr[i] ? best_src[i] : -1;
    return ISOCON_OK;
}

int nn_finalize_device(isocon_store *st, uint32_t n, const int32_t *best, const int32_t *hits, uint64_t n_hits, int32_t *out_best,
                       uint64_t *out_row_ptr, uint32_t *out_cols, uint64_t cols_cap, uint64_t *n_cols_needed)
{
    ScratchPool *pl = &st->pool;
    DevBuf d_hits(pl, SLOT_NN_FIN_HITS), d_best(pl, SLOT_NN_FIN_BEST);
    int rc;
    if ((rc = d_hits.alloc((size_t)n_hits * 12)) || (rc = d_best.alloc((size_t)n * 4))) return rc;
    ISO_HIP_CHECK(copy_h2d(d_hits.p, hits, (size_t)n_hits * 12));
    ISO_HIP_CHECK(copy_h2d(d_best.p, best, (size_t)n * 4));
    return nn_finalize_device_core(pl, n, d_best.as<int32_t>(), best, d_hits.as<int32_t>(), n_hits, out_best, out_row_ptr, out_cols, cols_cap, n_cols_needed);
}

int nn2_depth_graph(NNContext &C, uint64_t depth, int32_t *out_best, uint64_t *out_row_ptr, uint32_t *out_cols, uint64_t cols_cap,
                    uint64_t *n_cols_needed, isocon_nn_stats *stats);


}

extern "C" int isocon_nn_partial(isocon_store *s, const uint8_t *is_converged, const uint8_t *is_target, uint64_t depth,
                                 uint32_t q_begin, uint32_t q_end, uint32_t q_stride, uint32_t q_block, int32_t phase, int32_t *best_inout,
                                 int32_t *out_hits, uint64_t hits_cap, uint64_t *n_hits, isocon_nn_stats *stats, const uint8_t *wide_queries)
{
    if (!s || !best_inout || !n_hits || (hits_cap && !out_hits) || phase < 0 || phase > 3 || !qmap_args_ok(q_stride, q_block)) return ISOCON_E_ARG;
    const uint32_t n = s->dev.n;
    if (q_end > n) q_end = n;
    const QMap Q = qmap_of(q_begin, q_end, q_stride, q_block);
    WaitScope waits(s);
    NNContext C;
    int rc = nn_setup(C, s, is_converged, is_target, depth, best_inout);
    if (rc) return rc;
    if (phase == 2 && wide_queries) C.wide_mask.assign(wide_queries, wide_queries + n);
    rc = phase == 2 ? nn_phase_b(C, Q) : nn_phase_a(C, Q, false, phase == 0 || phase == 3, phase == 1 || phase == 3, phase == 1);
    if (rc) return rc;
    C.tm.resolve();
    C.stats.kernel_ms = C.tm.total; C.stats.narrow_kernel_ms = C.tm.marked_total;
    if (stats) *stats = C.stats;
    std::copy(C.best.begin(), C.best.begin() + n, best_inout);
    *n_hits = C.hits.size() / 3;
    if (*n_hits > hits_cap) return ISOCON_E_CAPACITY;
    if (!C.hits.empty()) memcpy(out_hits, C.hits.data(), C.hits.size() * 4);
    return ISOCON_OK;
}

extern "C" int isocon_nn_finalize(uint32_t n, const int32_t *best, const int32_t *hits, uint64_t n_hits,
                                  int32_t *out_best, uint64_t *out_row_ptr, uint32_t *out_cols, uint64_t cols_cap,
                                  uint64_t *n_cols_needed)
{
    if ((n && (!best || !out_best)) || !out_row_ptr || (n_hits && !hits) || (cols_cap && !out_cols)) return ISOCON_E_ARG;
    return nn_finalize_impl(n, best, hits, n_hits, out_best, out_row_ptr, out_cols, cols_cap, n_cols_needed);
}

extern "C" int isocon_nn_partial_dev(isocon_store *s, const uint8_t *is_converged, const uint8_t *is_target, uint64_t depth,
                                     uint32_t q_begin, uint32_t q_end, uint32_t q_stride, uint32_t q_block, int32_t phase, int32_t *best_inout_dev,
                                     int32_t keep_hits, uint64_t *n_hits_held, isocon_nn_stats *stats, const uint8_t *wide_queries)
{
    if (!s || !best_inout_dev || !n_hits_held || phase < 0 || phase > 3 || !qmap_args_ok(q_stride, q_block)) return ISOCON_E_ARG;
    const uint32_t n = s->dev.n;
    if (q_end > n) q_end = n;
    const QMap Q = qmap_of(q_begin, q_end, q_stride, q_block);
    WaitScope waits(s);
    std::vector<int32_t> best(std::max<uint32_t>(n, 1), NN_INF);
    if (n) ISO_HIP_CHECK(copy_d2h(best.data(), best_inout_dev, (size_t)n * 4));
    NNContext C;
    int rc = nn_setup(C, s, is_converged, is_target, depth, best.data());
    if (rc) return rc;
    if (phase == 2 && wide_queries) C.wide_mask.assign(wide_queries, wide_queries + n);
    C.keep_dev = phase != 2;
    rc = phase == 2 ? nn_phase_b(C, Q) : nn_phase_a(C, Q, false, phase == 0 || phase == 3, phase == 1 || phase == 3, phase == 1);
    if (rc) return rc;
    C.tm.resolve();
    C.stats.kernel_ms = C.tm.total; C.stats.narrow_kernel_ms = C.tm.marked_total;
    if (stats) *stats = C.stats;
    if (n) ISO_HIP_CHECK(copy_h2d(best_inout_dev, C.best.data(), (size_t)n * 4));
    if (!keep_hits || s->pool.held_hits.store_serial != s->serial) s->pool.held_hits = HeldHits{s->serial, 0};
    const uint64_t add_host = C.hits.size() / 3, add = add_host + C.dev_hit_count, have = s->pool.held_hits.rows;
    ScratchPool::Slot &slot = s->pool.slots[SLOT_NN_ACC_HITS];
    if ((have + add) * 12 > slot.cap) {
        void *bigger = nullptr;
        const size_t want = (size_t)(have + add) * 12 * 2 + ((size_t)1 << 20);
        ISO_HIP_CHECK(hipMalloc(&bigger, want));
        if (have) ISO_HIP_CHECK(memcpy_wait(bigger, slot.p, (size_t)have * 12, hipMemcpyDeviceToDevice));
        if (slot.p) (void)hipFree(slot.p);
        slot.p = bigger; slot.cap = want;
    }
    if (add_host) ISO_HIP_CHECK(copy_h2d(static_cast<char *>(slot.p) + (size_t)have * 12, C.hits.data(), (size_t)add_host * 12));
    if (C.dev_hit_count)
        ISO_HIP_CHECK(memcpy_wait(static_cast<char *>(slot.p) + (size_t)(have + add_host) * 12, C.dev_hits, (size_t)C.dev_hit_count * 12, hipMemcpyDeviceToDevice));
    s->pool.held_hits.rows = have + add;
    *n_hits_held = s->pool.held_hits.rows;
    return ISOCON_OK;
}

extern "C" int isocon_nn_hits_dev(isocon_store *s, const int32_t *best_dev, int32_t *out_hits_dev, uint64_t cap_rows, uint64_t *n_kept)
{
    if (!s || !best_dev || (cap_rows && !out_hits_dev)) return ISOCON_E_ARG;
    uint64_t rows = s->pool.held_hits.store_serial == s->serial ? s->pool.held_hits.rows : 0;
    if (s->pool.slots[SLOT_NN_ACC_HITS].cap < rows * 12) rows = 0;
    if (rows > cap_rows) return ISOCON_E_CAPACITY;
    if (cap_rows) ISO_HIP_CHECK(hipMemsetAsync(out_hits_dev, 0xff, (size_t)cap_rows * 12, 0));
    unsigned long long kept = 0;
    if (rows) {
        DevBuf d_c(&s->pool, SLOT_NN_HITCOUNT2);
        int rc;
        if ((rc = d_c.alloc(8))) return rc;
        ISO_HIP_CHECK(hipMemsetAsync(d_c.p, 0, 8, 0));
        const unsigned blocks = (unsigned)std::min<unsigned long long>((rows + 255) / 256, 4096);
        hipLaunchKernelGGL(k_filter_hits, dim3(blocks), dim3(256), 0, 0, static_cast<const int32_t *>(s->pool.slots[SLOT_NN_ACC_HITS].p), (unsigned long long)rows,
                           best_dev, out_hits_dev, d_c.as<unsigned long long>());
        ISO_HIP_CHECK(hipGetLastError());
        if (n_kept) ISO_HIP_CHECK(memcpy_wait(&kept, d_c.p, 8, hipMemcpyDeviceToHost));
    }
    if (n_kept) *n_kept = kept;
    return ISOCON_OK;
}

extern "C" int isocon_nn_finalize_dev(isocon_store *s, const int32_t *best_dev, const int32_t *hits_dev, uint64_t n_rows,
                                      int32_t *out_best, uint64_t *out_row_ptr, uint32_t *out_cols, uint64_t cols_cap, uint64_t *n_cols_needed)
{
    if (!s || !out_row_ptr || (n_rows && !hits_dev) || (cols_cap && !out_cols)) return ISOCON_E_ARG;
    const uint32_t n = s->dev.n;
    if (n && (!best_dev || !out_best)) return ISOCON_E_ARG;
    std::vector<int32_t> best(std::max<uint32_t>(n, 1));
    if (n) ISO_HIP_CHECK(copy_d2h(best.data(), best_dev, (size_t)n * 4));
    int rc = nn_finalize_device_core(&s->pool, n, best_dev, best.data(), hits_dev, n_rows, out_best, out_row_ptr, out_cols, cols_cap, n_cols_needed);
    if (rc != ISOCON_E_UNSUPPORTED) return rc;
    std::vector<int32_t> hits((size_t)n_rows * 3);
    if (n_rows) ISO_HIP_CHECK(copy_d2h(hits.data(), hits_dev, (size_t)n_rows * 12));
    return nn_finalize_impl(n, best.data(), hits.data(), n_rows, out_best, out_row_ptr, out_cols, cols_cap, n_cols_needed);
}

extern "C" int isocon_nn_graph(isocon_store *s, const uint8_t *is_converged, const uint8_t *is_target, uint64_t depth,
                               int32_t *out_best, uint64_t *out_row_ptr, uint32_t *out_cols, uint64_t cols_cap,
                               uint64_t *n_cols_needed, isocon_nn_stats *stats)
{
    if (!s || !out_best || !out_row_ptr || (cols_cap && !out_cols)) return ISOCON_E_ARG;
    const uint32_t n = s->dev.n;
    HostClock clk0;
    if (getenv("ISOCON_DEBUG")) { (void)hipDeviceSynchronize(); clk0.lap("sync at entry"); }
    struct Total { std::chrono::steady_clock::time_point t = std::chrono::steady_clock::now();
                   ~Total() { if (getenv("ISOCON_DEBUG")) fprintf(stderr, "[isocon] %-28s %8.2f ms\n", "isocon_nn_graph total", std::chrono::duration<double, std::milli>(std::chrono::steady_clock::now() - t).count()); } } total;
    WaitScope waits(s);
    NNContext C;
    int rc = nn_setup(C, s, is_converged, is_target, depth, nullptr, true);
    if (rc) return rc;
    clk0.lap("setup");
    if (getenv("ISOCON_DEBUG")) { (void)hipDeviceSynchronize(); clk0.lap("sync after setup"); }
    if (C.two_set && (C.depth_binds || variant("nn_2set_walk"))) return nn2_depth_graph(C, depth, out_best, out_row_ptr, out_cols, cols_cap, n_cols_needed, stats);
    C.keep_dev = n >= 1024 && !variant("nn_host_finalize");
    C.csr_follows = C.keep_dev;
    C.fill_best = !s->n_exc;
    if ((rc = nn_phase_a(C, QMap{0u, n, 1u, 0u}, true, true, true))) return rc;
    HostClock clk;
    C.keep_dev = C.csr_follows = C.fill_best = false;
    bool run_b = true;
    if (!C.best_on_host) {
        if (C.wide_needed || !C.dev_hit_count) {
            if ((rc = C.download_best()) || (rc = C.pull_dev_hits())) return rc;
        } else run_b = false;
    }
    if (run_b && (rc = nn_phase_b(C, QMap{0u, n, 1u, 0u}))) return rc;
    clk.lap("phaseB");
    C.tm.resolve();
    if (C.dev_hit_count) {
        if (C.hits.empty()) {
            C.stats.kernel_ms = C.tm.total; C.stats.narrow_kernel_ms = C.tm.marked_total;
            if (stats) *stats = C.stats;
            rc = nn_finalize_device_core(&s->pool, n, C.d_best.as<int32_t>(), C.best_on_host ? C.best.data() : nullptr, C.dev_hits, C.dev_hit_count, out_best, out_row_ptr, out_cols, cols_cap, n_cols_needed);
            clk.lap("finalize (device hits)");
            if (rc != ISOCON_E_UNSUPPORTED && rc != ISOCON_E_HIP) return rc;
        }
        if (!C.best_on_host && (rc = C.download_best())) return rc;
        if ((rc = C.pull_dev_hits())) return rc;
    }
    C.stats.kernel_ms = C.tm.total; C.stats.narrow_kernel_ms = C.tm.marked_total;
    if (stats) *stats = C.stats;
    struct Lap { HostClock &c; ~Lap() { c.lap("finalize"); } } lap{clk};
    if (C.hits.size() / 3 >= 4096 && n >= 1024 && !variant("nn_host_finalize")) {
        rc = nn_finalize_device(s, n, C.best.data(), C.hits.data(), C.hits.size() / 3, out_best, out_row_ptr, out_cols, cols_cap, n_cols_needed);
        if (rc != ISOCON_E_UNSUPPORTED && rc != ISOCON_E_HIP) return rc;
    }
    return nn_finalize_impl(n, C.best.data(), C.hits.data(), C.hits.size() / 3, out_best, out_row_ptr, out_cols, cols_cap, n_cols_needed);
}

extern "C" int isocon_qgram_bound_matrix(isocon_store *s, uint32_t q_begin, uint32_t q_end, uint32_t q_stride, uint32_t q_block, uint64_t depth,
                                         uint64_t *out_row_ptr, uint8_t *out_bounds, uint64_t bounds_cap, uint64_t *n_bounds_needed)
{
    if (!s || !out_row_ptr || !qmap_args_ok(q_stride, q_block) || (bounds_cap && !out_bounds)) return ISOCON_E_ARG;
    if (s->n_exc) { g_last_error = "q-gram bounds are defined on the 2-bit planes: the set holds more than four distinct symbols"; return ISOCON_E_ALPHABET; }
    const uint32_t n = s->dev.n;
    if (q_end > n) q_end = n;
    NNContext C;
    int rc = nn_setup(C, s, nullptr, nullptr, depth, nullptr);
    if (rc) return rc;
    NNParams P = C.params(63);
    s->pool.bound_tag.valid = false;
    const QMap Q = qmap_of(q_begin, q_end, q_stride, q_block);
    const uint32_t nq = Q.count();
    if ((rc = C.build_bounds(Q, 63, P))) return rc;
    ISO_HIP_CHECK(device_wait());
    C.tm.resolve();
    s->pool.bound_tag.valid = false;
    uint64_t total = 0;
    if (P.lb == nullptr) {
        for (uint32_t r = 0; r <= nq; ++r) out_row_ptr[r] = 0;
        if (n_bounds_needed) *n_bounds_needed = 0;
        bool any = false;
        for (uint32_t r = 0; r < C.lb_len_host.size(); ++r) any = any || C.lb_len_host[r] != 0;
        if (any) { g_last_error = "bound matrix not built (memory)"; return ISOCON_E_UNSUPPORTED; }
        return ISOCON_OK;
    }
    for (uint32_t r = 0; r < nq; ++r) { out_row_ptr[r] = total; total += C.lb_len_host[r]; }
    out_row_ptr[nq] = total;
    if (n_bounds_needed) *n_bounds_needed = total;
    if (total > bounds_cap) return ISOCON_E_CAPACITY;
    std::vector<uint8_t> raw((size_t)C.lb_total);
    ISO_HIP_CHECK(copy_d2h(raw.data(), P.lb, (size_t)C.lb_total));
    for (uint32_t r = 0; r < nq; ++r)
        if (C.lb_len_host[r]) memcpy(out_bounds + out_row_ptr[r], raw.data() + C.lb_off_host[r], C.lb_len_host[r]);
    if (C.d_lbt.p != nullptr) {
        std::vector<unsigned long long> offT(n);
        std::vector<uint32_t> sloT(n), lenT(n);
        ISO_HIP_CHECK(copy_d2h(offT.data(), C.d_offT.p, (size_t)n * 8));
        ISO_HIP_CHECK(copy_d2h(sloT.data(), C.d_sloT.p, (size_t)n * 4));
        ISO_HIP_CHECK(copy_d2h(lenT.data(), C.d_lenT.p, (size_t)n * 4));
        unsigned long long endT = 0, cells = 0;
        for (uint32_t p = 0; p < n; ++p) if (lenT[p]) endT = std::max(endT, offT[p] + lenT[p]);
        std::vector<uint8_t> rawT((size_t)endT + 1);
        if (endT) ISO_HIP_CHECK(copy_d2h(rawT.data(), C.d_lbt.p, (size_t)endT));
        for (uint32_t p = 0; p < n; ++p)
            for (uint32_t i = 0; i < lenT[p]; ++i) {
                const uint32_t r = sloT[p] + i;
                const uint64_t q = Q.entry(r);
                if (r >= nq || q >= p || p - q - 1 >= C.lb_len_host[r] || rawT[offT[p] + i] != raw[C.lb_off_host[r] + (p - q - 1)]) {
                    g_last_error = "transposed bound matrix differs from the matrix at entry " + std::to_string(p) + ", slot " + std::to_string(r);
                    return ISOCON_E_HIP;
                }
                ++cells;
            }
        if (cells != total) { g_last_error = "transposed bound matrix holds " + std::to_string(cells) + " cells, the matrix " + std::to_string(total); return ISOCON_E_HIP; }
    }
    return ISOCON_OK;
}
```

isocon_amd/csrc/nn_filter.hpp:

```cpp
#pragma once
#include "nn_list.hpp"

namespace isocon {

static constexpr int NNF_BATCH = 16;
#ifndef ISOCON_NNF_GROUP
#define ISOCON_NNF_GROUP 2
#endif
static constexpr int NNF_GROUP = ISOCON_NNF_GROUP;
static constexpr uint32_t NNF_LIST_MIN = 32;
static constexpr uint32_t NNF_TABLE_CHUNKS = 1024;
static constexpr uint32_t NNF_GRID = 256 * 8;
static constexpr uint32_t NNF_PASS2_MIN = 16;
static constexpr uint32_t NNF_GRID2 = 256 * 4;

struct NNFTask { uint32_t owner, count; unsigned long long begin; };

__host__ __device__ __forceinline__ uint32_t nnf_text2_stride(int32_t maxlen)
{
    const uint32_t dw = ((uint32_t)maxlen + 15u) / 16u;
    return ((dw + NNF_BATCH - 1) / NNF_BATCH + 1u) * NNF_BATCH + 4u;
}

__device__ __forceinline__ uint32_t nnf_spread16(uint32_t x)
{
    x = (x | (x << 8)) & 0x00ff00ffu;
    x = (x | (x << 4)) & 0x0f0f0f0fu;
    x = (x | (x << 2)) & 0x33333333u;
    x = (x | (x << 1)) & 0x55555555u;
    return x;
}

__global__ __launch_bounds__(256) void k_build_text2(DevStore S, uint32_t *__restrict__ text, uint32_t stride)
{
    const uint32_t i = blockIdx.x;
    if (i >= S.n) return;
    const int32_t len = S.lens[i];
    uint32_t *row = text + (size_t)i * stride;
    for (uint32_t j = threadIdx.x; j < stride; j += 256) {
        uint32_t v = 0;
        const int32_t c0 = (int32_t)j * 16;
        if (c0 < len) {
            const size_t at = ((size_t)(c0 >> 6) * S.n + i) * 2;
            const uint32_t lo = (uint32_t)(S.planes[at] >> (c0 & 63)) & 0xffffu, hi = (uint32_t)(S.planes[at + 1] >> (c0 & 63)) & 0xffffu;
            v = nnf_spread16(lo) | (nnf_spread16(hi) << 1);
        }
        row[j] = v;
    }
}

__device__ __forceinline__ unsigned long long nnf_uniform64(unsigned long long v)
{
    return ((unsigned long long)(uint32_t)__builtin_amdgcn_readfirstlane((int)(v >> 32)) << 32) | (uint32_t)__builtin_amdgcn_readfirstlane((int)(uint32_t)v);
}

__device__ __forceinline__ uint32_t nnf_absent(const uint32_t *bitmap, uint32_t c)
{
    const uint32_t word = *reinterpret_cast<const uint32_t *>(reinterpret_cast<const char *>(bitmap) + ((c >> 3) & 0x1ffcu));
    return (word >> (c & 31u)) & 1u;
}

__device__ __forceinline__ void nnf_add_grams(uint32_t *bitmap, const uint32_t *rx, int32_t len, int32_t tid = (int32_t)threadIdx.x, int32_t nthreads = 256)
{
    const int32_t ng = len - 7;
    for (int32_t j = tid; j * 16 < ng; j += nthreads) {
        const uint32_t w0 = rx[j], w1 = rx[j + 1];
        const uint64_t ww = ((uint64_t)w1 << 32) | w0;
#pragma unroll
        for (int t = 0; t < 16; ++t) {
            if (j * 16 + t < ng) {
                const uint32_t code = (uint32_t)(ww >> (2 * t)) & 0xffffu;
                atomicAnd(&bitmap[code >> 5], ~(1u << (code & 31u)));
            }
        }
    }
}

template <int S>
__host__ __device__ __forceinline__ int32_t nnf_dwords(int32_t len) { return len >= 24 - S ? (len - (24 - S)) / 16 + 1 : 0; }

template <int S>
__device__ __forceinline__ uint32_t nnf_count(const uint32_t *bitmap, const uint32_t *row, int32_t nd, int32_t k, bool active)
{
    static_assert(S == 4 || S == 2, "probe stride");
    const int32_t nb = wave_max_i32((nd + NNF_BATCH - 1) / NNF_BATCH);
    uint32_t cnt = 0;
    uint32_t r1 = 0, r2 = 0, r3 = 0;
    auto load17 = [](const uint32_t *p, uint32_t (&d)[17]) {
#pragma unroll
        for (int q = 0; q < 4; ++q) {
            const uint4 t = reinterpret_cast<const uint4 *>(p)[q];
            d[4 * q] = t.x; d[4 * q + 1] = t.y; d[4 * q + 2] = t.z; d[4 * q + 3] = t.w;
        }
        d[16] = p[16];
    };
    auto piece = [&](const uint32_t (&w)[17], int32_t b) {
        int32_t rem = nd - b * NNF_BATCH;
        rem = rem < 0 ? 0 : rem > 16 ? 16 : rem;
        const uint32_t lm = (1u << rem) - 1u;
#pragma unroll
        for (int jj = 0; jj < 16; ++jj) {
            const uint32_t lv = (lm >> jj) & 1u;
            uint32_t sum = 0;
#pragma unroll
            for (int t = 0; t < 16 / S; ++t) {
                const int sh = 2 * S * t;
                const uint32_t c = sh == 0 ? w[jj] : sh <= 16 ? w[jj] >> sh : __builtin_amdgcn_alignbit(w[jj + 1], w[jj], sh);
                const uint32_t a = nnf_absent(bitmap, c);
                const uint32_t h = S == 4 ? a & ~r1 & lv : a & ~(r1 | r2 | r3) & lv;
                r3 = r2; r2 = r1; r1 = h;
                sum += h;
            }
            cnt += sum;
            if ((jj & (S == 4 ? NNF_GROUP - 1 : 0)) == (S == 4 ? NNF_GROUP - 1 : 0)) __builtin_amdgcn_sched_barrier(0);
        }
    };
    uint32_t w[17];
#pragma unroll 1
    for (int32_t b = 0; b < nb; ++b) {
        load17(row + (size_t)b * NNF_BATCH, w);
        piece(w, b);
        if (__ballot(active && (int32_t)cnt <= k) == 0) break;
    }
    return cnt;
}

#ifndef ISOCON_NNF_WAVES
#define ISOCON_NNF_WAVES 4
#endif
__global__ __launch_bounds__(256, ISOCON_NNF_WAVES) void k_nn_block_filter(const uint32_t *__restrict__ text, uint32_t stride, const int32_t *__restrict__ lens, const uint32_t *__restrict__ meta,
                                                          int32_t kcap, uint32_t *__restrict__ list, const NNChunk *__restrict__ chunks_in, unsigned long long cap_in,
                                                          NNChunk *__restrict__ chunks_out, unsigned long long cap_out, uint32_t *__restrict__ pa, uint32_t *__restrict__ pb,
                                                          unsigned long long small_cap, NNPlanTotals *__restrict__ totals, uint32_t list_min, NNFTask *__restrict__ tasks,
                                                          unsigned long long tasks_cap)
{
    __shared__ uint32_t bitmap[2048];
    __shared__ uint32_t pass[NN_STAGE];
    __shared__ uint32_t s_npass;
    __shared__ unsigned long long s_chunk, s_base;
    const int lane = threadIdx.x & 63;
    if (totals->overflow) return;
    const unsigned long long nA = totals->n_chunks < cap_in ? totals->n_chunks : cap_in;
    const unsigned long long nB = totals->n_chunks_narrow < cap_in ? totals->n_chunks_narrow : cap_in;
    for (;;) {
        __syncthreads();
        if (threadIdx.x == 0) { s_chunk = atomicAdd(&totals->f_next, 1ull); s_npass = 0; }
        for (uint32_t i = threadIdx.x; i < 2048; i += 256) bitmap[i] = 0xffffffffu;
        __syncthreads();
        const unsigned long long c = nnf_uniform64(s_chunk);
        if (c >= nA + nB) break;
        const bool narrow = c >= nA;
        const NNChunk ch = narrow ? chunks_in[cap_in + (c - nA)] : chunks_in[c];
        const uint32_t x = ch.slot;
        nnf_add_grams(bitmap, text + (size_t)x * stride, lens[x]);
        __syncthreads();
        const uint32_t mx = meta[x];
        const int32_t kx0 = nn_meta_thr(mx);
        uint32_t rejected = 0;
        auto threshold = [&](uint32_t word) {
            int32_t k = -1;
            if (word & 0x40000000u) k = kx0;
            if (word & 0x80000000u) { const int32_t ky = nn_meta_thr(meta[word & 0x3fffffffu]); k = ky > k ? ky : k; }
            return k > kcap ? kcap : k;
        };
        for (uint32_t i0 = (threadIdx.x >> 6) * 64u; i0 < ch.count; i0 += 256u) {
            const uint32_t i = i0 + (uint32_t)lane;
            const bool active = i < ch.count;
            const uint32_t word = active ? list[ch.begin + i] : 0u;
            const uint32_t y = word & 0x3fffffffu;
            const int32_t k = active ? threshold(word) : -1;
            const uint32_t cnt = nnf_count<4>(bitmap, text + (size_t)y * stride, active ? nnf_dwords<4>(lens[y]) : 0, k, active);
            const bool keep = active && (int32_t)cnt <= k;
            rejected += (uint32_t)__popcll(__ballot(active && !keep));
            if (keep) pass[atomicAdd(&s_npass, 1u)] = word;
        }
        __syncthreads();
        const uint32_t np = (uint32_t)__builtin_amdgcn_readfirstlane((int)s_npass);
        const bool to_table = np >= list_min && (tasks == nullptr || 2u * np >= ch.count);
        if (threadIdx.x == 0) {
            unsigned long long base = 0;
            if (to_table) {
                const unsigned long long ci = atomicAdd(narrow ? &totals->f_chunks_narrow : &totals->f_chunks, 1ull);
                if (ci < cap_out) { NNChunk o; o.slot = x; o.count = np; o.begin = ch.begin; chunks_out[(narrow ? cap_out : 0ull) + ci] = o; }
                else { atomicOr(&totals->overflow, 1ull); base = ~0ull; }
                if (narrow) atomicAdd(&totals->f_narrow_listed, (unsigned long long)np);
                atomicAdd(&totals->f_listed, (unsigned long long)np);
            } else if (tasks != nullptr && np >= NNF_PASS2_MIN) {
                const uint32_t nt = (np + 63u) / 64u;
                base = atomicAdd(&totals->f_tasks, (unsigned long long)nt);
                if (base + nt > tasks_cap) { atomicOr(&totals->overflow, 1ull); base = ~0ull; }
            } else if (np) {
                base = atomicAdd(&totals->n_small, (unsigned long long)np);
                if (base + np > small_cap) { atomicOr(&totals->overflow, 1ull); base = ~0ull; }
            }
            s_base = base;
        }
        if ((threadIdx.x & 63) == 0 && rejected) atomicAdd(&totals->f_rejected, (unsigned long long)rejected);
        __syncthreads();
        const unsigned long long base = nnf_uniform64(s_base);
        if (base != ~0ull) {
            if (to_table) { for (uint32_t i = threadIdx.x; i < np; i += 256) list[ch.begin + i] = pass[i]; }
// ... 112 lines not shown
```

isocon_amd/csrc/nn_finalize.hpp:

```cpp
#pragma once
#include "nn_list.hpp"

namespace isocon {

static constexpr uint32_t NN_FIN_MAX_ROW = 256;

__device__ __forceinline__ bool nn_fin_valid(const int32_t *__restrict__ hits, unsigned long long h, const int32_t *__restrict__ best, uint32_t n,
                                             uint32_t &e, uint32_t &o)
{
    const int32_t a = hits[h * 3], b = hits[h * 3 + 1], d = hits[h * 3 + 2];
    if (a < 0 || b < 0 || (uint32_t)a >= n || (uint32_t)b >= n || d < 0 || d != best[a]) return false;
    e = (uint32_t)a; o = (uint32_t)b;
    return true;
}

__global__ __launch_bounds__(256) void k_fin_count(const int32_t *__restrict__ hits, unsigned long long n_hits, const int32_t *__restrict__ best, uint32_t n,
                                                    uint32_t *__restrict__ cnt)
{
    const unsigned long long h = (unsigned long long)blockIdx.x * 256u + threadIdx.x;
    uint32_t e, o;
    if (h < n_hits && nn_fin_valid(hits, h, best, n, e, o)) atomicAdd(cnt + e, 1u);
}

__global__ __launch_bounds__(256) void k_fin_scatter(const int32_t *__restrict__ hits, unsigned long long n_hits, const int32_t *__restrict__ best, uint32_t n,
                                                      const unsigned long long *__restrict__ start, uint32_t *__restrict__ cursor, uint32_t *__restrict__ nb)
{
    const unsigned long long h = (unsigned long long)blockIdx.x * 256u + threadIdx.x;
    uint32_t e, o;
    if (h < n_hits && nn_fin_valid(hits, h, best, n, e, o)) nb[start[e] + atomicAdd(cursor + e, 1u)] = o;
}

__global__ __launch_bounds__(256) void k_fin_rows(uint32_t n, const unsigned long long *__restrict__ start, uint32_t *__restrict__ nb, uint32_t *__restrict__ len2,
                                                   uint32_t *__restrict__ too_long)
{
    const uint32_t i = blockIdx.x * 256u + threadIdx.x;
    if (i >= n) return;
    uint32_t *b = nb + start[i];
    const uint32_t len = (uint32_t)(start[i + 1] - start[i]);
    if (len > NN_FIN_MAX_ROW) { atomicOr(too_long, 1u); len2[i] = len; return; }
    auto before = [i](uint32_t x, uint32_t y) {
        const uint32_t ox = x > i ? x - i : i - x, oy = y > i ? y - i : i - y;
        return ox != oy ? ox < oy : x < y;
    };
    for (uint32_t a = 1; a < len; ++a) {
        const uint32_t v = b[a];
        uint32_t c = a;
        while (c > 0 && before(v, b[c - 1])) { b[c] = b[c - 1]; --c; }
        b[c] = v;
    }
    uint32_t w = 0;
    for (uint32_t a = 0; a < len; ++a)
        if (a == 0 || b[a] != b[a - 1]) b[w++] = b[a];
    len2[i] = w;
}

__global__ __launch_bounds__(256) void k_fin_gather(uint32_t n, const unsigned long long *__restrict__ start, const uint32_t *__restrict__ nb,
                                                     const unsigned long long *__restrict__ row_ptr, uint32_t *__restrict__ cols)
{
    const uint32_t i = blockIdx.x * 256u + threadIdx.x;
    if (i >= n) return;
    const uint32_t len = (uint32_t)(row_ptr[i + 1] - row_ptr[i]);
    const uint32_t *src = nb + start[i];
    uint32_t *dst = cols + row_ptr[i];
    for (uint32_t a = 0; a < len; ++a) dst[a] = src[a];
}

__global__ __launch_bounds__(256) void k_fin_pack(uint32_t n, const unsigned long long *__restrict__ row_ptr, unsigned long long *__restrict__ rec,
                                                   const int32_t *__restrict__ best, int32_t *__restrict__ best_out)
{
    const uint32_t i = blockIdx.x * 256u + threadIdx.x;
    if (i == 0) rec[1] = row_ptr[n];
    if (best_out != nullptr && i < n) best_out[i] = best[i];
}

__global__ __launch_bounds__(256) void k_nn_step_record(const unsigned long long *__restrict__ hit_count, const unsigned long long *__restrict__ stats, uint32_t n_stats,
                                                         const int32_t *__restrict__ best, const uint8_t *__restrict__ qflag, const int32_t *__restrict__ lens,
                                                         uint32_t n, unsigned long long *__restrict__ rec)
{
    const uint32_t i = blockIdx.x * 256u + threadIdx.x;
    if (blockIdx.x == 0) {
        if (threadIdx.x == 0) rec[0] = *hit_count;
        for (uint32_t k = threadIdx.x; k < n_stats; k += 256u) rec[2 + k] = stats[k];
    }
    const bool wide = i < n && qflag[i] != 0 && best[i] == NN_INF && lens[i] > 63;
    if (__ballot(wide) != 0 && (threadIdx.x & 63u) == 0) atomicOr(rec + 1, 1ull);
}

}
```

isocon_amd/csrc/nn_lists.inc:

```

namespace {

int NNContext::plan_lists(const QMap &Q, uint32_t nq, const NNParams &PR, ListPlan &L)
{
    L = ListPlan();
    if (PR.lb == nullptr || nq == 0 || variant("nn_no_list") || st->pool.slots[SLOT_NN_LBT].p == nullptr || st->maxlen >= 16384) return ISOCON_OK;
    unsigned long long pairs_cap = std::min<unsigned long long>(lb_total, std::max<unsigned long long>(1ull << 22, lb_total / 8));
    if (const char *e = variant_value("nn_list_cap")) pairs_cap = std::max<unsigned long long>(1, strtoull(e, nullptr, 10));
    const bool filter = !variant("nn_no_block_filter") && ensure_text2();
    uint32_t list_min = NN_LIST_MIN;
    if (const char *e = variant_value("nn_list_min")) list_min = (uint32_t)std::max(1, atoi(e));
    const uint32_t build_min = filter ? std::min<uint32_t>(list_min, NNF_LIST_MIN) : list_min;
    const unsigned long long cap_in = pairs_cap / build_min + 1, cap_out = filter ? pairs_cap / list_min + 1 : cap_in;
    size_t free_b = 0;
    if (!free_mem(free_b) || pairs_cap * 12 > free_b / 2 + st->pool.slots[SLOT_NN_LIST].cap * 3) return ISOCON_OK;
    DevBuf *bufs[] = {&d_ltot, &d_lchunks, &d_list, &d_lpa, &d_lpb, &d_lmeta, &d_ltasks};
    const int slots[] = {SLOT_NN_LTOT, SLOT_NN_LCHUNKS, SLOT_NN_LIST, SLOT_NN_LPA, SLOT_NN_LPB, SLOT_NN_LDEST, SLOT_NN_LTASKS};
    for (int i = 0; i < 7; ++i) { bufs[i]->pool = &st->pool; bufs[i]->slot = slots[i]; }
    const bool second = filter && !variant("nn_filter_one_pass");
    const unsigned long long tasks_cap = second ? 2 * cap_in + pairs_cap / 64 + 1 : 0;
    if (second && d_ltasks.alloc((size_t)tasks_cap * sizeof(NNFTask))) return ISOCON_OK;
    const size_t n_records = (size_t)(filter ? 2 * cap_in : 0) + 4 * (size_t)cap_out;
    if (d_lmeta.alloc(((size_t)n + NN_META_PAD) * 4) || d_ltot.alloc(sizeof(NNPlanTotals)) || d_lchunks.alloc(n_records * sizeof(NNChunk)) || d_list.alloc((size_t)pairs_cap * 4) ||
        d_lpa.alloc((size_t)pairs_cap * 4) || d_lpb.alloc((size_t)pairs_cap * 4))
        return ISOCON_OK;
    NNChunk *built = d_lchunks.as<NNChunk>();
    L.a = built + (filter ? 2 * cap_in : 0);
    L.b = L.a + cap_out;
    L.sorted_a = L.b + cap_out;
    L.sorted_b = L.sorted_a + cap_out;
    ISO_HIP_CHECK(hipMemsetAsync(d_ltot.p, 0, sizeof(NNPlanTotals), 0));
    NNBoundRows B;
    B.lb = PR.lb; B.row_off = PR.lb_row; B.row_len = static_cast<const uint32_t *>(st->pool.slots[SLOT_NN_LBLEN].p);
    B.lbT = static_cast<const uint8_t *>(st->pool.slots[SLOT_NN_LBT].p);
    B.offT = static_cast<const unsigned long long *>(st->pool.slots[SLOT_NN_LBT_OFF].p);
    B.sloT = static_cast<const uint32_t *>(st->pool.slots[SLOT_NN_LBT_SLO].p);
    B.lenT = static_cast<const uint32_t *>(st->pool.slots[SLOT_NN_LBT_LEN].p);
    B.score = static_cast<const uint32_t *>(st->pool.slots[SLOT_NN_SCORE].p);
    tm.start();
    int32_t class_mode = 0;
    if (const char *e = variant_value("nn_narrow")) class_mode = atoi(e) > 0 ? 1 : -1;
    hipLaunchKernelGGL(k_nn_entry_meta, dim3((n + NN_META_PAD + 255) / 256), dim3(256), 0, 0, st->dev, PR, B.score, d_lmeta.as<uint32_t>(), d_ltot.as<NNPlanTotals>());
    ISO_HIP_CHECK(hipGetLastError());
    hipLaunchKernelGGL(k_nn_survivors, dim3((n + NN_SURV_WAVES - 1) / NN_SURV_WAVES), dim3(64 * NN_SURV_WAVES), 0, 0, st->dev, PR, B, d_lmeta.as<uint32_t>(), Q, nq, d_list.as<uint32_t>(), pairs_cap,
                       filter ? built : L.a, cap_in, d_lpa.as<uint32_t>(), d_lpb.as<uint32_t>(), pairs_cap, d_ltot.as<NNPlanTotals>(), build_min, class_mode);
    ISO_HIP_CHECK(hipGetLastError());
    if (filter) {
        tm.mark();
        ISO_HIP_CHECK(nnf_launch_filter(d_text2.as<uint32_t>(), text2_stride, st->dev.lens, d_lmeta.as<uint32_t>(), PR.kcap, d_list.as<uint32_t>(), built, cap_in, L.a, cap_out,
                                        d_lpa.as<uint32_t>(), d_lpb.as<uint32_t>(), pairs_cap, d_ltot.as<NNPlanTotals>(), list_min,
                                        second ? d_ltasks.as<NNFTask>() : (NNFTask *)nullptr, tasks_cap));
    }
    tm.stop_later(&stats.list_kernel_ms, &stats.filter_kernel_ms);
    NNPlanTotals tot;
    ISO_HIP_CHECK(memcpy_wait(&tot, d_ltot.p, sizeof(tot), hipMemcpyDeviceToHost));
    if (tot.overflow) return ISOCON_OK;
    stats.pairs_prefiltered += tot.n_filtered;
    stats.pairs_block_rejected += tot.f_rejected + tot.f_rejected2;
    L.listed = true;
    L.n_chunks = filter ? tot.f_chunks : tot.n_chunks;
    L.n_chunks_narrow = filter ? tot.f_chunks_narrow : tot.n_chunks_narrow;
    L.n_small = tot.n_small;
    stats.pairs_wide_to_lanes += tot.n_wide_pairs;
    unsigned long long table_chunks = NNF_TABLE_CHUNKS;
    if (const char *e = variant_value("nn_table_chunks")) table_chunks = strtoull(e, nullptr, 10);
    if (filter && L.n_chunks + L.n_chunks_narrow > 0 && L.n_chunks + L.n_chunks_narrow < table_chunks) {
        if (tot.n_small + tot.f_listed > pairs_cap) return ISOCON_OK;
        L.conv_a = L.n_chunks; L.conv_b = L.n_chunks_narrow; L.conv_pairs = tot.f_listed;
        L.n_chunks = L.n_chunks_narrow = 0;
        return ISOCON_OK;
    }
    stats.pairs_narrow += filter ? tot.f_narrow_listed : tot.n_narrow_listed;
    return ISOCON_OK;
}

}
```

isocon_amd/csrc/nn_main.inc:

```

namespace {

template <int NW, bool HALF>
int launch_refill_as(NNContext &C, const NNRefillShape &sh, unsigned grid, const NNParams &P, const QMap &Q, int32_t first_tile)
{
    if (sh.raise_limit) ISO_HIP_CHECK(hipFuncSetAttribute((const void *)k_nn_scan_refill<NW, 1, HALF>, hipFuncAttributeMaxDynamicSharedMemorySize, (int)sh.lds));
    hipLaunchKernelGGL((k_nn_scan_refill<NW, 1, HALF>), dim3(grid), dim3(NW * 64), sh.lds, 0, C.st->dev, P, C.d_text.as<uint32_t>(), C.text_stride, Q, first_tile);
    ISO_HIP_CHECK(hipGetLastError());
    return ISOCON_OK;
}

int launch_refill(NNContext &C, const NNRefillShape &sh, bool half, unsigned grid, const NNParams &P, const QMap &Q, int32_t first_tile)
{
    switch (sh.waves) {
    case 4: return half ? launch_refill_as<4, true>(C, sh, grid, P, Q, first_tile) : launch_refill_as<4, false>(C, sh, grid, P, Q, first_tile);
    case 8: return half ? launch_refill_as<8, true>(C, sh, grid, P, Q, first_tile) : launch_refill_as<8, false>(C, sh, grid, P, Q, first_tile);
    default: return half ? launch_refill_as<16, true>(C, sh, grid, P, Q, first_tile) : launch_refill_as<16, false>(C, sh, grid, P, Q, first_tile);
    }
}

struct Regrouped {
    std::vector<uint32_t> perm;
    std::vector<int32_t> seed_got;
    bool seed_collected = false;
// ... 156 lines not shown

int run_unlisted_pass(NNContext &C, const QMap &Q, const PhaseAPass &P, bool refill)
{
    const uint32_t nq = Q.count();
    const int32_t first_tile = (P.G.perm.empty() && ((P.do_seed && !P.bound_seeded) || (P.seeded_before && !P.bounds_wanted))) ? 1 : 0;
    if (refill) {
        if (!C.build_text()) return ISOCON_E_HIP;
        const char *wv = variant_value("nn_waves");
        const bool four = wv ? atoi(wv) == 4 : P.PR.lb != nullptr;
        return launch_refill(C, nn_refill_shape(C.st->maxlen, four ? 4 : 8, false), false, nq, P.PR, Q, first_tile);
    }
    DevStore S = C.st->dev;
    if (P.G.planes) S.planes = P.G.planes;
    const NNTileScan kernel = nn_tile_scan(C.st->maxlen);
    const size_t lds = nn_tile_scan_lds(C.st->maxlen);
    if (kernel == NN_SCAN_WINDOW) {
        hipLaunchKernelGGL(k_nn_scan_up<1>, dim3(nq), dim3(256), 0, 0, S, C.params(63), Q, first_tile, 0x7fffffff, 4);
        return ISOCON_OK;
    }
    DevBuf d_il(&C.st->pool, SLOT_NN_IL2);
    const size_t total = (size_t)C.n * C.st->dev.nchunks;
    int rc;
    if ((rc = d_il.alloc(total * 16))) return rc;
    hipLaunchKernelGGL(k_interleave_planes, dim3(2048), dim3(256), 0, 0, reinterpret_cast<const ulonglong2 *>(S.planes), d_il.as<ulonglong2>(), total);
    S.il = d_il.as<uint64_t>();
    if (kernel == NN_SCAN_LDS8) {
        hipLaunchKernelGGL(k_nn_scan_lds<8>, dim3(nq), dim3(512), lds, 0, S, C.params(63), Q, first_tile, 0x7fffffff);
    } else {
        ISO_HIP_CHECK(hipFuncSetAttribute((const void *)k_nn_scan_lds<16>, hipFuncAttributeMaxDynamicSharedMemorySize, (int)lds));
        hipLaunchKernelGGL(k_nn_scan_lds<16>, dim3(nq), dim3(1024), lds, 0, S, C.params(63), Q, first_tile, 0x7fffffff);
    }
    return ISOCON_OK;
}

int phase_a_main(NNContext &C, const QMap &Q, PhaseAPass &P, HostClock &clk)
{
    int rc;
    if (C.n >= (1u << 30)) { g_last_error = "store too large for the packed neighbour queue"; return ISOCON_E_ARG; }
    C.tm.start();
    const bool refill = P.refill_main && P.G.perm.empty() && C.text_affordable();
    NNParams &PR = P.PR;
    if (refill && P.bounds_wanted && !P.bounds_built) {
        C.tm.stop_later(&C.stats.scan_kernel_ms);
        if ((rc = C.build_bounds(Q, 63, PR))) return rc;
        clk.lap("phaseA: q-gram bounds");
        C.tm.start();
    }
    if (!refill) { PR.lb = nullptr; PR.lb_row = nullptr; PR.slot_order = nullptr; }
    NNContext::ListPlan LP;
    if (refill && PR.lb != nullptr) {
        C.tm.stop_later(&C.stats.scan_kernel_ms);
        if ((rc = C.plan_lists(Q, Q.count(), PR, LP))) return rc;
        clk.lap("phaseA: survivor lists");
        C.tm.start();
    }
    P.no_markers = LP.listed && P.seeds_clean;
    if ((rc = LP.listed ? run_listed_pass(C, Q, PR, LP) : run_unlisted_pass(C, Q, P, refill))) return rc;
    ISO_HIP_CHECK(hipGetLastError());
    C.tm.stop_later(&C.stats.scan_kernel_ms);
    C.stats.scan_launches += 1;
    return ISOCON_OK;
}

int phase_a_two_set_unbounded(NNContext &C, const QMap &Q)
{
    C.tm.start();
    if (!C.build_text()) return ISOCON_E_HIP;
    int rc;
    if ((rc = launch_refill(C, nn_refill_shape(C.st->maxlen, 8, false), false, Q.count(), C.params(63), Q, 0))) return rc;
    C.tm.stop_later(&C.stats.scan_kernel_ms);
    C.stats.scan_launches += 1;
    return ISOCON_OK;
}

int phase_a_two_set_tiles(NNContext &C, const QMap &Q, bool do_main)
{
    std::vector<uint32_t> ts, ids, lanes;
    for (uint32_t c = 0; c < C.n && do_main; ++c) {
        if (!C.tflag[c] || C.dev_excluded(c)) continue;
        uint32_t lo, hi;
        length_window(C.st->lens, c, 63, lo, hi);
        lo = std::max(lo, Q.begin);
        hi = std::min(hi, Q.end);
        lanes.clear();
        for (uint32_t p = lo; p < hi; ++p)
            if (C.qflag[p] && !C.dev_excluded(p) && Q.owns(p)) lanes.push_back(p);
        push_tiles(ts, ids, c, lanes);
    }
    float ms = 0.f;
    int rc;
    if ((rc = run_nn_tiles(1, C, ts, ids, &ms))) return rc;
    C.stats.scan_launches += 1;
    C.stats.scan_kernel_ms += ms;
    return ISOCON_OK;
}

int nn_end_pass(NNContext &C, int32_t kcap, bool no_markers, const Regrouped &G, HostClock *clk, bool &again)
{
    auto lap = [&](const char *what) { if (clk) clk->lap(what); };
    again = false;
    uint64_t needed = 0;
    std::vector<int32_t> got;
    const bool in_place = G.perm.empty();
    const bool dev_ok = C.keep_dev && no_markers && in_place && !G.seed_collected && C.hits.empty();
    const bool one_record = dev_ok && C.csr_follows && !C.st->n_exc && !C.flags_dirty;
    int rc = one_record ? C.collect_record(&needed) : C.collect(got, &needed, in_place, dev_ok);
    C.tm.resolve();
    if (rc == ISOCON_E_CAPACITY) {
        C.hits_cap = needed + needed / 2 + 1024;
        if ((rc = C.d_hits.alloc(C.hits_cap * 12))) return rc;
        again = true;
        if (in_place) return C.download_best();
        C.best = *G.best_at_entry;
        return C.upload_flags();
    }
    if (rc) return rc;
    if (one_record) { lap("phaseA: hits and bounds stay on the device"); return ISOCON_OK; }
    if ((rc = C.download_best())) return rc;
    if (dev_ok) { lap("phaseA: hits stay on the device"); return ISOCON_OK; }
    if (!in_place && (rc = G.unpermute(C, got))) return rc;
    if (G.seed_collected) got.insert(got.end(), G.seed_got.begin(), G.seed_got.end());
    lap("phaseA: collect+unpermute");
    std::vector<uint32_t> ra, rb;
    for (size_t i = 0; i + 2 < got.size(); i += 3) {
        if (got[i + 2] == -2) { ra.push_back((uint32_t)got[i]); rb.push_back((uint32_t)got[i + 1]); }
        else C.hits.insert(C.hits.end(), got.begin() + i, got.begin() + i + 3);
    }
    if (!ra.empty()) {
        std::vector<int32_t> kk(ra.size(), kcap), dd(ra.size(), -1);
        float ems = 0.f;
        if ((rc = ed_pairs_impl(C.st, ra.data(), rb.data(), kk.data(), ra.size(), dd.data(), &ems, nullptr, C.image_pass))) return rc;
        C.tm.total += ems;
        for (size_t i = 0; i < ra.size(); ++i)
            if (dd[i] >= 0) C.apply(ra[i], rb[i], dd[i]);
    }
    lap("phaseA: markers");
    return ISOCON_OK;
}

int nn_phase_a_planes(NNContext &C, const QMap &Q, bool allow_regroup = false,
                      bool do_seed = true, bool do_main = true, bool seeded_before = false)
{
    const uint32_t n = C.n;
    if (Q.begin >= Q.end) return ISOCON_OK;
    const std::vector<int32_t> best0 = C.best;
    HostClock clk;
    const bool fits = nn_refill64_fits(C.st->maxlen);
    const bool two_set_many = C.two_set && do_main && !variant("nn_tiles") && n < (1u << 30) && fits &&
                              (size_t)std::count(C.tflag.begin(), C.tflag.end(), (uint8_t)1) > 512;
    const bool two_set_lists = two_set_many && !variant("nn_no_qgram");
    const bool whole_set = Q.begin == 0 && Q.end == n && Q.stride == 1 && Q.block_log2 == 0 && C.depth >= n;
    for (;;) {
        int rc;
        if ((rc = C.upload_best()) || (rc = C.reset_counters())) return rc;
        clk.lap("phaseA: upload/reset");
        PhaseAPass P(do_seed, do_main, seeded_before);
        if (!C.two_set || two_set_lists) {
            P.refill_main = !variant("nn_tiles") && fits;
            P.bounds_wanted = P.refill_main && !variant("nn_no_qgram");
            P.PR = C.params(63);
            if (do_seed && (rc = phase_a_seeds(C, Q, P, clk))) return rc;
            if (allow_regroup && !P.refill_main && do_seed && do_main && whole_set && n > 128 && (rc = regroup_by_seed_hits(C, best0, P.G, clk))) return rc;
            if (do_main && (rc = phase_a_main(C, Q, P, clk))) return rc;
            if (!do_main) P.no_markers = do_seed && P.seeds_clean;
            clk.lap("phaseA: main kernel");
        } else if (two_set_many && C.text_affordable()) {
            if ((rc = phase_a_two_set_unbounded(C, Q))) return rc;
        } else if ((rc = phase_a_two_set_tiles(C, Q, do_main))) return rc;
        bool again = false;
        if ((rc = nn_end_pass(C, 63, P.no_markers, P.G, &clk, again))) return rc;
        if (!again) return ISOCON_OK;
    }
}

}
```

isocon_amd/csrc/qgram_mm.hpp:

```cpp
#pragma once
#include "common.hpp"

namespace isocon {

#ifndef ISOCON_QG_Q
#define ISOCON_QG_Q 9
#endif
static constexpr int QG_Q = ISOCON_QG_Q;
#ifndef ISOCON_QG_B0
#define ISOCON_QG_B0 12288
#endif
static constexpr int QG_B0 = ISOCON_QG_B0;
#ifndef ISOCON_QG_B1
#define ISOCON_QG_B1 2048
#endif
#ifndef ISOCON_QG_CAP
#define ISOCON_QG_CAP 2
#endif
static constexpr int QG_B1 = ISOCON_QG_B1;
static constexpr int QG_CAP = ISOCON_QG_CAP;
static constexpr int QM_K = QG_B0 + QG_B1 * QG_CAP;
static constexpr int QM_KBE = 128;
static constexpr int QM_ROWB = QM_KBE / 2;
static constexpr int QM_SLOTS = QM_ROWB / 16;
static constexpr int QM_NKB = QM_K / QM_KBE;
static constexpr int QM_TILE = 256;
static constexpr int QM_STAGES = 4;
static constexpr int QM_STAGE_BYTES = 2 * QM_TILE * QM_ROWB;
static constexpr int QM_OUT_STRIDE = QM_TILE + 8;
static constexpr int QM_OUTT_STRIDE = QM_TILE + 32;
static constexpr int QM_EPI_BYTES = QM_TILE * (QM_OUT_STRIDE + QM_OUTT_STRIDE);
static constexpr int QM_META_BYTES = 256 * (4 + 4 + 4 + 4 + 8 + 4) + 3 * 16 * 2 + 256 * (4 + 4 + 8) + 4 * 256 * 4;
#ifndef ISOCON_QM_SEEDS
#define ISOCON_QM_SEEDS 4
#endif
static constexpr int QM_SEEDS = ISOCON_QM_SEEDS;
static constexpr uint32_t QM_HUB_BOUND = 36;
static constexpr int QM_META_OFF = QM_STAGES * QM_STAGE_BYTES > QM_EPI_BYTES ? QM_STAGES * QM_STAGE_BYTES : QM_EPI_BYTES;
static constexpr size_t QM_LDS_BYTES = (size_t)QM_META_OFF + QM_META_BYTES;
static_assert(QG_B0 % 128 == 0 && QG_B1 % 256 == 0 && QG_B0 % QG_B1 == 0, "K-blocks of 128 elements; excess bin = presence bin mod QG_B1");
static_assert(QM_K % QM_KBE == 0 && QM_NKB >= QM_STAGES && QM_STAGES == 4, "whole K-blocks; the K loop's tail is written for a ring of four");
static_assert(QM_META_OFF % 16 == 0 && QM_LDS_BYTES <= 160 * 1024, "the epilogue's byte tiles reuse the ring; the tile's row / column tables sit behind both");

__host__ __device__ __forceinline__ uint32_t qg_bin(uint32_t g)
{
    return (QG_B0 == (1 << (2 * QG_Q))) ? g : ((g * 0x9E3779B1u) >> 7) % (uint32_t)QG_B0;
}

__device__ __forceinline__ uint32_t qg_spread8(uint32_t x)
{
    uint32_t y = (x | (x << 12)) & 0x000F000Fu;
    y = (y | (y << 6)) & 0x03030303u;
    y = (y | (y << 3)) & 0x11111111u;
    return y << 1;
}

static constexpr int QP_SEQS = 4;

__global__ __launch_bounds__(256) void k_qgram_profile4(DevStore S, uint8_t *__restrict__ prof4, uint32_t *__restrict__ psum, uint32_t n_pad)
{
    __shared__ uint32_t bits[QP_SEQS][QM_K / 32];
    __shared__ uint32_t exh[QG_B1];
    __shared__ uint32_t s_sum[QP_SEQS];
    const uint32_t i0 = blockIdx.x * (uint32_t)QP_SEQS;
    if (i0 >= S.n) return;
    const uint32_t cnt = S.n - i0 < (uint32_t)QP_SEQS ? S.n - i0 : (uint32_t)QP_SEQS;
    for (int e = threadIdx.x; e < QP_SEQS * (QM_K / 32); e += 256) (&bits[0][0])[e] = 0;
    if (threadIdx.x < QP_SEQS) s_sum[threadIdx.x] = 0;
    for (uint32_t r = 0; r < cnt; ++r) {
        const uint32_t i = i0 + r;
        for (int e = threadIdx.x; e < QG_B1; e += 256) exh[e] = 0;
        __syncthreads();
        const int32_t ngrams = S.lens[i] - QG_Q + 1;
        for (int32_t j = threadIdx.x; j < ngrams; j += 256) {
            const int32_t c = j >> 6, o = j & 63;
            const size_t at = ((size_t)c * S.n + i) * 2;
            uint64_t lo = S.planes[at] >> o, hi = S.planes[at + 1] >> o;
            if (o > 64 - QG_Q) {
                const size_t at2 = ((size_t)(c + 1) * S.n + i) * 2;
                lo |= S.planes[at2] << (64 - o);
                hi |= S.planes[at2 + 1] << (64 - o);
            }
            const uint32_t mask = (1u << QG_Q) - 1u;
            const uint32_t bin = qg_bin(((uint32_t)lo & mask) | (((uint32_t)hi & mask) << QG_Q));
            const uint32_t bit = 1u << (bin & 31u);
            const uint32_t old = atomicOr(&bits[r][bin >> 5], bit);
            if (old & bit) atomicAdd(&exh[bin % (uint32_t)QG_B1], 1u);
        }
        __syncthreads();
        for (int j0 = (threadIdx.x & ~63); j0 < QG_B1; j0 += 256) {
            const uint32_t v = exh[j0 + (threadIdx.x & 63)];
#pragma unroll
            for (int t = 0; t < QG_CAP; ++t) {
                const unsigned long long m = __ballot(v > (uint32_t)t);
                if ((threadIdx.x & 63) == 0) {
                    bits[r][(QG_B0 + t * QG_B1 + j0) / 32] = (uint32_t)m;
                    bits[r][(QG_B0 + t * QG_B1 + j0) / 32 + 1] = (uint32_t)(m >> 32);
                }
            }
        }
        __syncthreads();
    }
    uint32_t local[QP_SEQS];
#pragma unroll
    for (int r = 0; r < QP_SEQS; ++r) local[r] = 0;
    for (int e = threadIdx.x; e < QP_SEQS * (QM_K / 32); e += 256) {
        const int kb = e / (QP_SEQS * QM_SLOTS), r = (e / QM_SLOTS) % QP_SEQS, sl = e % QM_SLOTS;
        const uint32_t w = bits[r][kb * QM_SLOTS + sl];
#pragma unroll
        for (int rr = 0; rr < QP_SEQS; ++rr) local[rr] += rr == r ? (uint32_t)__popc(w) : 0u;
        if ((uint32_t)r < cnt) {
            uint4 o;
            o.x = qg_spread8(w & 0xffu); o.y = qg_spread8((w >> 8) & 0xffu); o.z = qg_spread8((w >> 16) & 0xffu); o.w = qg_spread8(w >> 24);
            *reinterpret_cast<uint4 *>(prof4 + ((size_t)kb * n_pad + i0 + (uint32_t)r) * QM_ROWB + (size_t)sl * 16) = o;
        }
    }
#pragma unroll
    for (int r = 0; r < QP_SEQS; ++r) if (local[r]) atomicAdd(&s_sum[r], local[r]);
    __syncthreads();
    if (threadIdx.x < cnt) psum[i0 + threadIdx.x] = s_sum[threadIdx.x];
}

#ifdef ISOCON_QM_TIMELINE
__device__ unsigned long long g_qm_timeline[16384 * 8];
#define QM_STAMP(k) do { if (threadIdx.x == 0 && blockIdx.x < 16384u) g_qm_timeline[blockIdx.x * 8u + (k)] = __builtin_amdgcn_s_memtime(); } while (0)
#else
#define QM_STAMP(k) do { } while (0)
#endif

typedef int qm_v8i __attribute__((ext_vector_type(8)));
typedef float qm_v16f __attribute__((ext_vector_type(16)));

__device__ __forceinline__ void qm_glds16(const uint8_t *gsrc, uint32_t lds_dst)
{
    uint32_t keep;
    asm volatile("s_mov_b32 %0, m0\n\ts_mov_b32 m0, %2\n\ts_nop 0\n\tglobal_load_lds_dwordx4 %1, off\n\ts_mov_b32 m0, %0"
                 : "=&s"(keep) : "v"(gsrc), "s"(lds_dst) : "memory");
}

typedef unsigned short qm_us2 __attribute__((ext_vector_type(2)));

template <int S> __device__ __forceinline__ uint32_t qm_quad_bcast(uint32_t w)
{
    return (uint32_t)__builtin_amdgcn_update_dpp(0, (int)w, S * 0x55, 0xf, 0xf, true);
}
template <int CTRL> __device__ __forceinline__ uint32_t qm_dpp_min(uint32_t x)
{
    const uint32_t y = (uint32_t)__builtin_amdgcn_update_dpp(-1, (int)x, CTRL, 0xf, 0xf, false);
    return y < x ? y : x;
}
template <int CTRL> __device__ __forceinline__ uint32_t qm_dpp_add(uint32_t x)
{
    return x + (uint32_t)__builtin_amdgcn_update_dpp(0, (int)x, CTRL, 0xf, 0xf, false);
}
__device__ __forceinline__ uint32_t qm_row_min(uint32_t x) { x = qm_dpp_min<0x111>(x); x = qm_dpp_min<0x112>(x); x = qm_dpp_min<0x114>(x); return qm_dpp_min<0x118>(x); }
__device__ __forceinline__ uint32_t qm_row_add(uint32_t x) { x = qm_dpp_add<0x111>(x); x = qm_dpp_add<0x112>(x); x = qm_dpp_add<0x114>(x); return qm_dpp_add<0x118>(x); }

__device__ __forceinline__ void qm_chunk_stats(const uint4 v, uint32_t inside, uint32_t eligible, uint32_t base, uint32_t &key, uint32_t &hub)
{
    const uint32_t wv[4] = {v.x, v.y, v.z, v.w};
    if (inside == 0xffffu) {
        uint32_t cnt = 0;
#pragma unroll
        for (int d = 0; d < 4; ++d) {
            const uint32_t w = wv[d];
            const uint32_t gt = (((w & 0x7f7f7f7fu) + 0x01010101u * (127u - QM_HUB_BOUND)) | w) & 0x80808080u;
            cnt += (uint32_t)__builtin_popcount(gt ^ 0x80808080u);
        }
        hub += cnt;
    } else {
#pragma unroll
        for (int k = 0; k < 16; ++k) {
            const uint32_t bd = (wv[k >> 2] >> (8 * (k & 3))) & 0xffu;
            hub += ((inside >> k) & 1u) && bd <= QM_HUB_BOUND ? 1u : 0u;
        }
    }
    if (eligible == 0xffffu) {
        qm_us2 m = {0xffff, 0xffff};
#pragma unroll
        for (int d = 0; d < 4; ++d) {
            const uint32_t w = wv[d];
            const uint32_t b4 = base + 4u * (uint32_t)d;
            const uint32_t ke = ((w << 8) & 0xff00ff00u) | (b4 | ((b4 + 2u) << 16)), ko = (w & 0xff00ff00u) | ((b4 + 1u) | ((b4 + 3u) << 16));
            qm_us2 e, o;
            __builtin_memcpy(&e, &ke, 4);
            __builtin_memcpy(&o, &ko, 4);
            m = __builtin_elementwise_min(m, __builtin_elementwise_min(e, o));
        }
        const uint32_t k16 = m.x < m.y ? m.x : m.y;
        key = k16 < key ? k16 : key;
    } else if (eligible != 0u) {
#pragma unroll
        for (int k = 0; k < 16; ++k) {
            const uint32_t bd = (wv[k >> 2] >> (8 * (k & 3))) & 0xffu;
            const uint32_t cand = (bd << 8) | (base + (uint32_t)k);
            if ((eligible >> k) & 1u) key = cand < key ? cand : key;
        }
    }
}

__global__ __launch_bounds__(512, 2) void k_qgram_mm(const uint8_t *__restrict__ prof4, const uint32_t *__restrict__ psum, uint32_t n, uint32_t n_pad,
                                                      const uint2 *__restrict__ tiles, const unsigned long long *__restrict__ row_off,
                                                      const uint32_t *__restrict__ row_len, uint8_t *__restrict__ lb, QMap Q, uint32_t nq,
                                                      const uint8_t *__restrict__ qflag, const uint8_t *__restrict__ tflag,
                                                      unsigned long long *__restrict__ rowmin, unsigned long long *__restrict__ colmin,
                                                      const unsigned long long *__restrict__ offT, const uint32_t *__restrict__ sloT, const uint32_t *__restrict__ lenT,
                                                      uint8_t *__restrict__ lbT, uint32_t *__restrict__ score)
{
    extern __shared__ __attribute__((aligned(16))) uint8_t qm_lds[];
    const uint32_t b = blockIdx.x;
    const uint2 tl = tiles[(((b >> 3) >> 5) * 8u + (b & 7u)) * 32u + ((b >> 3) & 31u)];
    if (tl.x == 0xffffffffu) return;
    const uint32_t I = tl.x, J = tl.y;
    const int tid = threadIdx.x;
    const int lane = tid & 63;
    const int wave = __builtin_amdgcn_readfirstlane(tid >> 6);
    const int wp = wave & 1, wq = wave >> 1;
    QM_STAMP(0);
    const int r = lane & 31, h = lane >> 5;

    uint8_t *meta = qm_lds + (size_t)QM_META_OFF;
    float *m_sA = reinterpret_cast<float *>(meta);
    float *m_sB = m_sA + 256;
    uint32_t *m_q = reinterpret_cast<uint32_t *>(m_sB + 256);
    uint32_t *m_len = m_q + 256;
    unsigned long long *m_off = reinterpret_cast<unsigned long long *>(m_len + 256);
    uint32_t *m_flB = reinterpret_cast<uint32_t *>(m_off + 256);
    uint16_t *m_tA = reinterpret_cast<uint16_t *>(m_flB + 256);
    uint16_t *m_qA = m_tA + 16;
    uint16_t *m_tB = m_qA + 16;
    uint32_t *m_slo = reinterpret_cast<uint32_t *>(m_tB + 16);
    uint32_t *m_lenT = m_slo + 256;
    unsigned long long *m_offT = reinterpret_cast<unsigned long long *>(m_lenT + 256);
    uint32_t *m_rkey = reinterpret_cast<uint32_t *>(m_offT + 256);
    uint32_t *m_rhub = m_rkey + 256;
    uint32_t *m_ckey = m_rhub + 256;
    uint32_t *m_chub = m_ckey + 256;

    const uint32_t lds0 = (uint32_t)(uintptr_t)(__attribute__((address_space(3))) uint8_t *)qm_lds;
    const uint8_t *gsrc[4];
    uint32_t ldst[4];
#pragma unroll
    for (int it = 0; it < 4; ++it) {
        const int c = (it & 1) * 512 + tid;
        const int row = c >> 2, ps = c & 3, ls = ps ^ ((row >> 2) & 3);
        uint64_t ent;
        if (it < 2) ent = (uint64_t)J * QM_TILE + row;
        else {
            ent = Q.entry(I * QM_TILE + (uint32_t)row);
            if (ent >= n_pad) ent = n_pad - 1;
        }
#ifdef ISOCON_QM_SAMEPANEL
        ent = (uint64_t)row;
#endif
        gsrc[it] = prof4 + ent * QM_ROWB + ls * 16;
        ldst[it] = lds0 + (uint32_t)((it >> 1) * (QM_TILE * QM_ROWB) + ((it & 1) * 512 + wave * 64) * 16);
    }
    const size_t kb_stride = (size_t)n_pad * QM_ROWB;
    auto issue = [&](int kb) {
        const uint32_t st = (uint32_t)(kb % QM_STAGES) * QM_STAGE_BYTES;
#pragma unroll
        for (int it = 0; it < 4; ++it) qm_glds16(gsrc[it] + (size_t)kb * kb_stride, (uint32_t)__builtin_amdgcn_readfirstlane((int)(ldst[it] + st)));
    };
#pragma unroll
    for (int kb = 0; kb < QM_STAGES - 1; ++kb) issue(kb);

    if (tid < 256) {
        const uint64_t p = (uint64_t)J * QM_TILE + tid;
        m_sA[tid] = p < n ? (float)psum[p] : 0.f;
        const bool tp = lbT != nullptr && p < n;
        m_slo[tid] = tp ? sloT[p] : 0u;
// ... 77 lines not shown
        }
    } else {
        for (int kb = 0; kb < QM_NKB - (QM_STAGES - 1); ++kb) {
            dma_piece(kb + 3, 0); mfma_group(0);
            dma_piece(kb + 3, 1); mfma_group(1);
            asm volatile("s_waitcnt vmcnt(6)" ::: "memory");
            __builtin_amdgcn_s_barrier();
            asm volatile("" ::: "memory");
            read_frags(kb + 1, 0);
            dma_piece(kb + 3, 2); mfma_group(2);
            dma_piece(kb + 3, 3); mfma_group(3);
            read_frags(kb + 1, 1);
        }
    }
#pragma unroll
    for (int t = 3; t >= 1; --t) {
        const int kb = QM_NKB - t;
        mfma_group(0);
        mfma_group(1);
        if (t > 1) {
            if (t == 3) asm volatile("s_waitcnt vmcnt(4)" ::: "memory");
            else asm volatile("s_waitcnt vmcnt(0)" ::: "memory");
            __builtin_amdgcn_s_barrier();
            asm volatile("" ::: "memory");
            read_frags(kb + 1, 0);
        }
        mfma_group(2);
        mfma_group(3);
        if (t > 1) read_frags(kb + 1, 1);
    }
    __syncthreads();
    QM_STAMP(2);

    uint32_t *out32 = reinterpret_cast<uint32_t *>(qm_lds);
    uint32_t *outT32 = reinterpret_cast<uint32_t *>(qm_lds + QM_TILE * QM_OUT_STRIDE);
    {
        const uint32_t t4 = (uint32_t)lane & 3u;
        const uint32_t sel_lo = 0x0c0c0000u | ((4u + t4) << 8) | t4, sel_hi = 0x00000c0cu | ((4u + t4) << 24) | (t4 << 16);
        const uint32_t *m_sAu = reinterpret_cast<const uint32_t *>(m_sA), *m_sBu = reinterpret_cast<const uint32_t *>(m_sB);
        uint32_t sbf[2];
#pragma unroll
        for (int j = 0; j < 2; ++j) sbf[j] = m_sBu[wq * 64 + j * 32 + r];
#pragma unroll
        for (int i = 0; i < 4; ++i) {
#pragma unroll
            for (int g = 0; g < 4; ++g) {
                const int pl = wp * 128 + i * 32 + 8 * g + 4 * h;
                const uint4 sa = *reinterpret_cast<const uint4 *>(m_sAu + pl);
                const uint32_t sav[4] = {sa.x, sa.y, sa.z, sa.w};
#pragma unroll
                for (int j = 0; j < 2; ++j) {
                    const int ql = wq * 64 + j * 32 + r;
                    uint32_t w = 0;
#pragma unroll
                    for (int k = 0; k < 4; ++k) {
                        const float t = __uint_as_float(sav[k] > sbf[j] ? sav[k] : sbf[j]) - acc[i][j][4 * g + k];
                        const float z = __builtin_fmaf(t, 1.0f / (float)QG_Q, (((float)QG_Q - 0.5f) / (float)QG_Q) - 0.5f);
                        w = __builtin_amdgcn_cvt_pk_u8_f32(z, (uint32_t)k, w);
                    }
                    out32[ql * (QM_OUT_STRIDE / 4) + (pl >> 2)] = w;
                    const uint32_t a0 = qm_quad_bcast<0>(w), a1 = qm_quad_bcast<1>(w), a2 = qm_quad_bcast<2>(w), a3 = qm_quad_bcast<3>(w);
                    outT32[(pl + (int)t4) * (QM_OUTT_STRIDE / 4) + ((ql & ~3) >> 2)] = __builtin_amdgcn_perm(a1, a0, sel_lo) | __builtin_amdgcn_perm(a3, a2, sel_hi);
                }
            }
        }
    }
    __syncthreads();
    QM_STAMP(3);

    {
        const int chunk = tid & 15;
        const int32_t p0 = (int32_t)(J * QM_TILE) + chunk * 16;
        const uint32_t tmask = m_tA[chunk];
        const int32_t nn = (int32_t)n - p0;
        for (int rr = 0; rr < 8; ++rr) {
            const int ql = rr * 32 + (tid >> 4);
            const uint32_t qe = m_q[ql];
            int32_t lo = 0, hi = 0;
            if (qe != 0xffffffffu) {
                const int32_t first = (int32_t)qe + 1 - p0, last = first + (int32_t)m_len[ql];
                lo = first < 0 ? 0 : (first > 16 ? 16 : first);
                hi = last < nn ? last : nn;
                hi = hi < 0 ? 0 : (hi > 16 ? 16 : hi);
            }
            uint32_t key = 0xffffffffu, hub = 0;
            if (hi > lo) {
                const uint2 v0 = *reinterpret_cast<const uint2 *>(qm_lds + ql * QM_OUT_STRIDE + chunk * 16);
                const uint2 v1 = *reinterpret_cast<const uint2 *>(qm_lds + ql * QM_OUT_STRIDE + chunk * 16 + 8);
                uint4 v; v.x = v0.x; v.y = v0.y; v.z = v1.x; v.w = v1.y;
                *reinterpret_cast<uint4 *>(lb + (m_off[ql] + (unsigned long long)(long long)(p0 - (int32_t)qe - 1))) = v;
                const uint32_t inside = ((1u << hi) - 1u) & ~((1u << lo) - 1u);
                qm_chunk_stats(v, inside, (m_flB[ql] & 1u) ? (inside & tmask) : 0u, (uint32_t)(chunk * 16), key, hub);
            }
            key = qm_row_min(key);
            hub = qm_row_add(hub);
            if (chunk == 15) { m_rkey[ql] = key; m_rhub[ql] = hub; }
        }
    }
#ifdef ISOCON_QM_TIMELINE
    __syncthreads();
    QM_STAMP(4);
#endif
    const bool columns = lbT != nullptr || colmin != nullptr;
    if (columns) {
        const int chunk = tid & 15;
        const int32_t s0 = (int32_t)(I * QM_TILE) + chunk * 16;
        const uint32_t tmask = m_tB[chunk];
        const uint8_t *outT = qm_lds + QM_TILE * QM_OUT_STRIDE;
        for (int rr = 0; rr < 8; ++rr) {
            const int pl = rr * 32 + (tid >> 4);
            const int32_t slo = (int32_t)m_slo[pl];
            const int32_t first = slo - s0, last = first + (int32_t)m_lenT[pl];
            const int32_t lo = first < 0 ? 0 : (first > 16 ? 16 : first), hi = last < 0 ? 0 : (last > 16 ? 16 : last);
            uint32_t key = 0xffffffffu, hub = 0;
            if (hi > lo) {
                const uint4 v = *reinterpret_cast<const uint4 *>(outT + pl * QM_OUTT_STRIDE + chunk * 16);
                if (lbT != nullptr) *reinterpret_cast<uint4 *>(lbT + (m_offT[pl] + (unsigned long long)(long long)(s0 - slo))) = v;
                const uint32_t inside = ((1u << hi) - 1u) & ~((1u << lo) - 1u);
                const bool p_isq = colmin != nullptr && ((m_qA[pl >> 4] >> (pl & 15)) & 1u) != 0;
                qm_chunk_stats(v, inside, p_isq ? (inside & tmask) : 0u, (uint32_t)(chunk * 16), key, hub);
            }
            key = qm_row_min(key);
            hub = qm_row_add(hub);
            if (chunk == 15) { m_ckey[pl] = key; m_chub[pl] = hub; }
        }
    }
    __syncthreads();
    if (tid < 256) {
        const uint32_t key = m_rkey[tid], hub = m_rhub[tid], qe = m_q[tid];
        if (rowmin != nullptr && key != 0xffffffffu) {
            const uint64_t e = (uint64_t)J * QM_TILE + (key & 0xffu) - (uint64_t)qe - 1;
            atomicMin(rowmin + ((size_t)I * QM_TILE + (uint32_t)tid) * QM_SEEDS + (J % QM_SEEDS), ((unsigned long long)(key >> 8) << 32) | (unsigned long long)e);
        }
        if (score != nullptr && hub) atomicAdd(score + qe, hub);
    } else if (columns) {
        const int pl = tid - 256;
        const uint32_t key = m_ckey[pl], hub = m_chub[pl];
        const uint64_t p = (uint64_t)J * QM_TILE + (uint64_t)pl;
        if (colmin != nullptr && key != 0xffffffffu)
            atomicMin(colmin + p * QM_SEEDS + (I % QM_SEEDS), ((unsigned long long)(key >> 8) << 32) | (unsigned long long)m_q[key & 0xffu]);
        if (score != nullptr && hub && p < n) atomicAdd(score + p, hub);
    }
#ifdef ISOCON_QM_TIMELINE
    __syncthreads();
    QM_STAMP(5);
    if (threadIdx.x == 0 && blockIdx.x < 16384u) {
        uint32_t hw;
        asm volatile("s_getreg_b32 %0, hwreg(HW_REG_HW_ID)" : "=s"(hw));
        g_qm_timeline[blockIdx.x * 8u + 6] = hw;
    }
#endif
}

__global__ __launch_bounds__(256) void k_lbt_rows(QMap Q, uint32_t nq, const uint32_t *__restrict__ row_len, uint32_t n, uint32_t *__restrict__ sloT,
                                                   uint32_t *__restrict__ lenT, uint32_t *__restrict__ padT)
{
    const uint32_t p = blockIdx.x * 256u + threadIdx.x;
    if (p >= n) return;
    QMap below = Q;
    below.end = Q.end < p ? Q.end : p;
    uint32_t b = below.count();
    if (b > nq) b = nq;
    uint32_t lo = 0, hi = b;
    while (lo < hi) {
        const uint32_t mid = (lo + hi) >> 1;
        if (Q.entry(mid) + row_len[mid] < (uint64_t)p) lo = mid + 1; else hi = mid;
    }
    sloT[p] = lo;
    lenT[p] = b - lo;
    padT[p] = b > lo ? ((b + 15u) & ~15u) - (lo & ~15u) : 0u;
}

__global__ __launch_bounds__(256) void k_lbt_offsets(uint32_t n, const uint32_t *__restrict__ sloT, unsigned long long *__restrict__ offT)
{
    const uint32_t p = blockIdx.x * 256u + threadIdx.x;
    if (p < n) offT[p] += sloT[p] & 15u;
}

__global__ __launch_bounds__(256) void k_qgram_seed_pairs(const unsigned long long *__restrict__ rowmin, const unsigned long long *__restrict__ colmin,
                                                           uint32_t n, QMap Q, uint32_t nq, uint32_t col_classes,
                                                           uint32_t *__restrict__ pa, uint32_t *__restrict__ pb, unsigned long long *__restrict__ count)
{
    const uint32_t x = blockIdx.x * 256u + threadIdx.x;
    const int lane = threadIdx.x & 63;
    uint32_t sa[2 * QM_SEEDS], sb[2 * QM_SEEDS];
    uint32_t m = 0;
    if (x < n) {
        uint32_t s = 0u;
        const bool has_row = Q.slot_of(x, s) && s < nq;
        if (has_row) {
#pragma unroll
            for (int c = 0; c < QM_SEEDS; ++c) {
                const unsigned long long kr = rowmin[(size_t)s * QM_SEEDS + c];
                if (kr != ~0ull) { sa[m] = x; sb[m] = x + 1u + (uint32_t)kr; ++m; }
            }
        }
        const uint32_t per = (uint32_t)QM_SEEDS / col_classes;
        for (uint32_t g = 0; g < col_classes; ++g) {
            unsigned long long kc = ~0ull;
            for (uint32_t c = g; c < g + per * col_classes; c += col_classes) {
                const unsigned long long v = colmin[(size_t)x * QM_SEEDS + c];
                kc = v < kc ? v : kc;
            }
            if (kc != ~0ull) {
                const uint32_t q = (uint32_t)kc;
                uint32_t sq = 0u;
                (void)Q.slot_of(q, sq);
                const unsigned long long kq = rowmin[(size_t)sq * QM_SEEDS + (x / QM_TILE) % QM_SEEDS];
                if (kq == ~0ull || q + 1u + (uint32_t)kq != x) { sa[m] = q; sb[m] = x; ++m; }
            }
        }
    }
    uint32_t inc = m;
#pragma unroll
    for (uint32_t d = 1; d < 64; d <<= 1) {
        const uint32_t o = (uint32_t)__shfl_up((int)inc, d, 64);
        if ((uint32_t)lane >= d) inc += o;
    }
    const uint32_t wave_total = (uint32_t)__shfl((int)inc, 63, 64);
    if (wave_total == 0) return;
    unsigned long long base = 0;
    if (lane == 63) base = atomicAdd(count, (unsigned long long)wave_total);
    base = ((unsigned long long)(uint32_t)__shfl((int)(uint32_t)(base >> 32), 63, 64) << 32) | (uint32_t)__shfl((int)(uint32_t)base, 63, 64);
    const unsigned long long at = base + (inc - m);
#pragma unroll
    for (uint32_t i = 0; i < 2 * QM_SEEDS; ++i)
        if (i < m) { pa[at + i] = sa[i]; pb[at + i] = sb[i]; }
}

__global__ __launch_bounds__(256) void k_qgram_lb_pairs(const uint8_t *__restrict__ prof4, const uint32_t *__restrict__ psum, uint32_t n_pad,
                                                         const uint32_t *__restrict__ a, const uint32_t *__restrict__ b, uint64_t n_pairs,
                                                         int32_t *__restrict__ out)
{
    const uint64_t pr = (uint64_t)blockIdx.x * 4u + (threadIdx.x >> 6);
    const int lane = threadIdx.x & 63;
    if (pr >= n_pairs) return;
    const uint32_t x = a[pr], y = b[pr];
    uint32_t m = 0;
    for (int c = lane; c < QM_K / 8; c += 64) {
        const size_t at = ((size_t)(c / (QM_ROWB / 4)) * n_pad) * QM_ROWB + (size_t)(c % (QM_ROWB / 4)) * 4;
        const uint32_t u = *reinterpret_cast<const uint32_t *>(prof4 + at + (size_t)x * QM_ROWB);
        const uint32_t v = *reinterpret_cast<const uint32_t *>(prof4 + at + (size_t)y * QM_ROWB);
        m += (uint32_t)__popc(u & v);
    }
#pragma unroll
    for (int o = 32; o > 0; o >>= 1) m += (uint32_t)__shfl_xor((int)m, o, 64);
    if (lane == 0) {
        const uint32_t sx = psum[x], sy = psum[y];
        out[pr] = (int32_t)(((sx > sy ? sx : sy) - m + (uint32_t)QG_Q - 1u) / (uint32_t)QG_Q);
    }
}

}
```

Before: 78.63 billion alignments/s.

## Overlap bound-table setup on side stream and fuse text2 build into profile kernel

Moves the bound-row layout work (uploads, row kernel, exscan, offsets) and a new fused fill kernel that replaces several memsets onto a side stream, so it overlaps with the q-gram profile kernel on the main stream. The text2 encoding is now written inside the profile kernel rather than by a separate launch. The three host-to-device uploads are merged into one pinned copy, the per-pass init is fused into a single step-init kernel, and flag uploads are deferred. The profile popcount loop is simplified to one counter per thread. This adds cross-stream event dependencies and more scratch slots, with some risk of ordering mistakes.

```diff
diff --git a/isocon_amd/csrc/common.hpp b/isocon_amd/csrc/common.hpp
--- a/isocon_amd/csrc/common.hpp
+++ b/isocon_amd/csrc/common.hpp
@@ -37,6 +37,24 @@
     }
     __host__ __device__ __forceinline__ bool same(const QMap &o) const { return begin == o.begin && end == o.end && stride == o.stride && block_log2 == o.block_log2; }
 };
+
+__device__ __forceinline__ uint32_t spread16(uint32_t x)
+{
+    x = (x | (x << 8)) & 0x00ff00ffu;
+    x = (x | (x << 4)) & 0x0f0f0f0fu;
+    x = (x | (x << 2)) & 0x33333333u;
+    x = (x | (x << 1)) & 0x55555555u;
+    return x;
+}
+
+__device__ __forceinline__ uint32_t text2_word(const DevStore &S, uint32_t i, int32_t len, uint32_t j)
+{
+    const int32_t c0 = (int32_t)j * 16;
+    if (c0 >= len) return 0u;
+    const size_t at = ((size_t)(c0 >> 6) * S.n + i) * 2;
+    const uint32_t lo = (uint32_t)(S.planes[at] >> (c0 & 63)) & 0xffffu, hi = (uint32_t)(S.planes[at + 1] >> (c0 & 63)) & 0xffffu;
+    return spread16(lo) | (spread16(hi) << 1);
+}
 
 extern thread_local std::string g_last_error;
 
diff --git a/isocon_amd/csrc/isocon_hip.hip b/isocon_amd/csrc/isocon_hip.hip
--- a/isocon_amd/csrc/isocon_hip.hip
+++ b/isocon_amd/csrc/isocon_hip.hip
@@ -71,6 +71,8 @@
     uint32_t depth = 0;
     int32_t kcap = 0;
     unsigned long long lb_total = 0;
+    const unsigned long long *lb_row = nullptr;
+    const uint32_t *lb_len = nullptr;
 };
 struct MsaBuilt {
     enum By { NONE, SINGLE, BATCH } by = NONE;
@@ -112,12 +114,12 @@
 
 enum {
     SLOT_ED_TS = 0, SLOT_ED_IDS, SLOT_ED_K, SLOT_ED_OUT, SLOT_FULL_A, SLOT_FULL_B, SLOT_FULL_K, SLOT_FULL_OUT,
-    SLOT_NN_BEST, SLOT_NN_QF, SLOT_NN_TF, SLOT_NN_HITS, SLOT_NN_HITCOUNT, SLOT_NN_STATS, SLOT_NN_TS, SLOT_NN_IDS, SLOT_NN_PLANES2, SLOT_NN_PERM, SLOT_NN_IL, SLOT_NN_IL2, SLOT_NN_HITS2, SLOT_NN_HITCOUNT2, SLOT_NN_QPROF, SLOT_NN_QSUM, SLOT_NN_LB, SLOT_NN_LBROW, SLOT_NN_LBLEN, SLOT_NN_SLOTORDER, SLOT_NN_LBCHUNKS, SLOT_NN_ROWMIN, SLOT_NN_COLMIN, SLOT_NN_SEED_A, SLOT_NN_SEED_B, SLOT_NN_SEED_N, SLOT_NN_LBT, SLOT_NN_LBT_OFF, SLOT_NN_LBT_SLO, SLOT_NN_LBT_LEN, SLOT_NN_LBT_PAD, SLOT_NN_SCORE, SLOT_NN_LDEST, SLOT_NN_FIN_HITS, SLOT_NN_FIN_CNT, SLOT_NN_FIN_START, SLOT_NN_FIN_CUR, SLOT_NN_FIN_NB, SLOT_NN_FIN_LEN2, SLOT_NN_FIN_OUT, SLOT_NN_FIN_FLAG, SLOT_NN_FIN_BEST, SLOT_NN_ACC_HITS, SLOT_NN_LTOT, SLOT_NN_LCHUNKS, SLOT_NN_LIST, SLOT_NN_LPA, SLOT_NN_LPB, SLOT_NN_TEXT2, SLOT_NN_LTASKS, SLOT_NN_RECORD,
+    SLOT_NN_BEST, SLOT_NN_QF, SLOT_NN_TF, SLOT_NN_HITS, SLOT_NN_HITCOUNT, SLOT_NN_STATS, SLOT_NN_TS, SLOT_NN_IDS, SLOT_NN_PLANES2, SLOT_NN_PERM, SLOT_NN_IL, SLOT_NN_IL2, SLOT_NN_HITS2, SLOT_NN_HITCOUNT2, SLOT_NN_QPROF, SLOT_NN_QSUM, SLOT_NN_LB, SLOT_NN_SLOTORDER, SLOT_NN_LBCHUNKS, SLOT_NN_ROWMIN, SLOT_NN_COLMIN, SLOT_NN_SEED_A, SLOT_NN_SEED_B, SLOT_NN_SEED_N, SLOT_NN_LBT, SLOT_NN_LBT_OFF, SLOT_NN_LBT_SLO, SLOT_NN_LBT_LEN, SLOT_NN_LBT_PAD, SLOT_NN_SCORE, SLOT_NN_LDEST, SLOT_NN_FIN_HITS, SLOT_NN_FIN_CNT, SLOT_NN_FIN_START, SLOT_NN_FIN_CUR, SLOT_NN_FIN_NB, SLOT_NN_FIN_LEN2, SLOT_NN_FIN_OUT, SLOT_NN_FIN_FLAG, SLOT_NN_FIN_BEST, SLOT_NN_ACC_HITS, SLOT_NN_LTOT, SLOT_NN_LCHUNKS, SLOT_NN_LIST, SLOT_NN_LPA, SLOT_NN_LPB, SLOT_NN_TEXT2, SLOT_NN_LTASKS, SLOT_NN_RECORD,
     SLOT_NN2_STATE, SLOT_NN2_TPOS, SLOT_NN2_EXC, SLOT_NN2_CTR, SLOT_NN2_PAIRS, SLOT_NN2_WIDE,
     SLOT_SG_PAIRS, SLOT_SG_R, SLOT_SG_TRACE, SLOT_SG_END, SLOT_SG_OPS, SLOT_SG_CNT, SLOT_SG_RES, SLOT_SG_OFF, SLOT_SG_DENSE, SLOT_SG_BOUND, SLOT_SG_AOFF, SLOT_SG_ALNA, SLOT_SG_ALNB,
     SLOT_MSA_IN, SLOT_MSA_OUT, SLOT_MSA_DEG, SLOT_MSA_COUNTS, SLOT_MSA_MAJ, SLOT_MSA_FLAGS, SLOT_MSA_TOT, SLOT_MSA_NCAND, SLOT_MSA_LEN, SLOT_MSA_OFF, SLOT_MSA_PACKED, SLOT_MSA_ROWS, SLOT_MSA_OPS, SLOT_MSA_OPTR, SLOT_MSA_LONGEST, SLOT_MSA_WIDTH, SLOT_MSA_CSLOT, SLOT_MSA_LTOT, SLOT_MSA_WIDE, SLOT_MSA_PROW, SLOT_MSA_PCOL, SLOT_MSA_PPTR, SLOT_MSA_PBYTES, SLOT_MSA_PART, SLOT_MSA_FIRST, SLOT_MSA_LM, SLOT_MSA_SBASE, SLOT_MSA_NCOLS, SLOT_MSA_MOFF, SLOT_MSA_CBASE, SLOT_MSA_CBP, SLOT_MSA_CBC, SLOT_MSA_CBR,
     SLOT_HW_Q, SLOT_HW_T, SLOT_HW_K, SLOT_HW_OUT, SLOT_HW_TRACE, SLOT_HW_CTR, SLOT_HW_TILEQ, SLOT_HW_LANES, SLOT_HW_PQ, SLOT_HW_KEY, SLOT_HW_HIST, SLOT_HW_CURSOR, SLOT_HW_TBASE, SLOT_HW_CLS,
-    SLOT_PACK_ASCII, SLOT_PACK_OFF, SLOT_PACK_BAD, SLOT_PACK_HIST, SLOT_PACK_FLAGS, SLOT_EB_A, SLOT_EB_B, SLOT_EB_K, SLOT_EB_OUT, SLOT_EB_ROWS, SLOT_SCAN_TMP, SLOT_SCAN_SUMS,
+    SLOT_PACK_ASCII, SLOT_PACK_OFF, SLOT_PACK_BAD, SLOT_PACK_HIST, SLOT_PACK_FLAGS, SLOT_EB_A, SLOT_EB_B, SLOT_EB_K, SLOT_EB_OUT, SLOT_EB_ROWS, SLOT_SCAN_TMP, SLOT_SCAN_SUMS, SLOT_SCAN_TMP_SIDE, SLOT_SCAN_SUMS_SIDE,
     SLOT_RT_REF, SLOT_RT_IN, SLOT_RT_OUT,
     SLOT_EV_IN, SLOT_EV_OUT, SLOT_EV_SNIP,
     SLOT_PB_IN, SLOT_PB_OUT,
@@ -273,14 +275,14 @@
 };
 
 template <int SHIFT, class OUT>
-static int device_exscan(ScratchPool *pl, const uint32_t *d_in, uint32_t n, OUT *d_out)
-{
-    DevBuf d_tmp(pl, SLOT_SCAN_TMP), d_sums(pl, SLOT_SCAN_SUMS);
+static int device_exscan(ScratchPool *pl, const uint32_t *d_in, uint32_t n, OUT *d_out, hipStream_t stream = 0)
+{
+    DevBuf d_tmp(pl, stream ? SLOT_SCAN_TMP_SIDE : SLOT_SCAN_TMP), d_sums(pl, stream ? SLOT_SCAN_SUMS_SIDE : SLOT_SCAN_SUMS);
     const uint32_t tiles = std::max<uint32_t>(1, (n + SCAN_TILE - 1) / SCAN_TILE);
     int rc;
     if ((rc = d_tmp.alloc((size_t)std::max<uint32_t>(n, 1) * 4)) || (rc = d_sums.alloc((size_t)tiles * 8))) return rc;
-    hipLaunchKernelGGL((k_scan_tiles<SHIFT>), dim3(tiles), dim3(256), 0, 0, d_in, n, d_tmp.as<uint32_t>(), d_sums.as<unsigned long long>());
-    hipLaunchKernelGGL((k_scan_finish<OUT>), dim3(tiles), dim3(256), 0, 0, d_tmp.as<uint32_t>(), n, d_sums.as<unsigned long long>(), tiles, d_out, (unsigned long long *)nullptr);
+    hipLaunchKernelGGL((k_scan_tiles<SHIFT>), dim3(tiles), dim3(256), 0, stream, d_in, n, d_tmp.as<uint32_t>(), d_sums.as<unsigned long long>());
+    hipLaunchKernelGGL((k_scan_finish<OUT>), dim3(tiles), dim3(256), 0, stream, d_tmp.as<uint32_t>(), n, d_sums.as<unsigned long long>(), tiles, d_out, (unsigned long long *)nullptr);
     ISO_HIP_CHECK(hipGetLastError());
     return ISOCON_OK;
 }
@@ -1000,7 +1002,8 @@
     ISO_HIP_CHECK(copy_h2d(d_b.p, b, n_pairs * 4));
     EventTimer tm;
     tm.start();
-    hipLaunchKernelGGL(k_qgram_profile4, dim3((n + QP_SEQS - 1) / QP_SEQS), dim3(256), 0, 0, s->dev, d_prof.as<uint8_t>(), d_sum.as<uint32_t>(), n_pad);
+    hipLaunchKernelGGL(k_qgram_profile4, dim3((n + QP_SEQS - 1) / QP_SEQS), dim3(256), 0, 0, s->dev, d_prof.as<uint8_t>(), d_sum.as<uint32_t>(), n_pad,
+                       (uint32_t *)nullptr, 0u);
     ISO_HIP_CHECK(hipGetLastError());
     for (uint64_t at = 0; at < n_pairs; at += (uint64_t)1 << 24) {
         const uint64_t cnt = std::min<uint64_t>((uint64_t)1 << 24, n_pairs - at);
diff --git a/isocon_amd/csrc/nn_bounds.inc b/isocon_amd/csrc/nn_bounds.inc
--- a/isocon_amd/csrc/nn_bounds.inc
+++ b/isocon_amd/csrc/nn_bounds.inc
@@ -11,7 +11,8 @@
     if (!want_seeds && st->pool.bound_tag.valid && st->pool.bound_tag.serial == st->serial && st->pool.bound_tag.map.same(Q) &&
         st->pool.bound_tag.depth == depth && st->pool.bound_tag.kcap == kcap) {
         P.lb = static_cast<const uint8_t *>(st->pool.slots[SLOT_NN_LB].p);
-        P.lb_row = static_cast<const unsigned long long *>(st->pool.slots[SLOT_NN_LBROW].p);
+        P.lb_row = lb_row_dev = st->pool.bound_tag.lb_row;
+        lb_len_dev = st->pool.bound_tag.lb_len;
         if (st->pool.bound_tag.has_order && use_slot_order(Q.count())) P.slot_order = static_cast<const uint32_t *>(st->pool.slots[SLOT_NN_SLOTORDER].p);
         lb_total = st->pool.bound_tag.lb_total;
         return ISOCON_OK;
@@ -29,12 +30,46 @@
         if (!free_mem(free_b) || prof_bytes > free_b / 2 + st->pool.slots[SLOT_NN_QPROF].cap) return ISOCON_OK;
         if (d_qprof.alloc(prof_bytes) || d_qsum.alloc((size_t)n * 4)) return ISOCON_OK;
     }
+    uint32_t *text2 = !text2_ready && filter_wanted() && text2_room() ? d_text2.as<uint32_t>() : nullptr;
     bclk.lap("bounds: memory check + profile buffers");
+    g_side.settle();
     const bool side = !variant("nn_sync_uploads") && g_side.ready() && hipEventRecord(g_side.before, 0) == hipSuccess;
     tm.start();
-    hipLaunchKernelGGL(k_qgram_profile4, dim3((n + QP_SEQS - 1) / QP_SEQS), dim3(256), 0, 0, st->dev, d_qprof.as<uint8_t>(), d_qsum.as<uint32_t>(), n_pad);
-    ISO_HIP_CHECK(hipGetLastError());
+    hipLaunchKernelGGL(k_qgram_profile4, dim3((n + QP_SEQS - 1) / QP_SEQS), dim3(256), 0, 0, st->dev, d_qprof.as<uint8_t>(), d_qsum.as<uint32_t>(), n_pad,
+                       text2, text2_stride);
+    ISO_HIP_CHECK(hipGetLastError());
+    if (text2) text2_ready = true;
     struct StopTimer { NNContext &c; bool armed = true; ~StopTimer() { if (armed) c.tm.stop_later(&c.stats.bound_kernel_ms); } } stop_timer{*this};
+    hipStream_t ls = 0;
+    struct SideGuard { bool armed = false; ~SideGuard() { if (armed) g_side.settle(); } } side_guard;
+    if (side) {
+        g_side.in_flight = side_guard.armed = true;
+        ISO_HIP_CHECK(hipStreamWaitEvent(g_side.stream, g_side.before, 0));
+        ls = g_side.stream;
+    }
+    d_score.pool = &st->pool;
+    d_score.slot = SLOT_NN_SCORE;
+    if (d_score.alloc((size_t)n * 4)) return ISOCON_OK;
+    QMFills fills = {};
+    fills.r[0] = {d_score.as<uint32_t>(), n, 0u};
+    unsigned long long *rowmin = nullptr, *colmin = nullptr;
+    if (want_seeds) {
+        const uint64_t n_seed_words = (uint64_t)2 * QM_SEEDS * n;
+        d_rowmin.pool = d_colmin.pool = d_seed_a.pool = d_seed_b.pool = d_seed_n.pool = &st->pool;
+        d_rowmin.slot = SLOT_NN_ROWMIN; d_colmin.slot = SLOT_NN_COLMIN; d_seed_a.slot = SLOT_NN_SEED_A; d_seed_b.slot = SLOT_NN_SEED_B; d_seed_n.slot = SLOT_NN_SEED_N;
+        if (!(d_rowmin.alloc((size_t)nq * 8 * QM_SEEDS) || d_colmin.alloc((size_t)n_pad * 8 * QM_SEEDS) || d_seed_a.alloc((size_t)n_seed_words * 4) || d_seed_b.alloc((size_t)n_seed_words * 4) ||
+              d_seed_n.alloc(8))) {
+            fills.r[1] = {d_rowmin.as<uint32_t>(), (unsigned long long)nq * 2 * QM_SEEDS, 0xffffffffu};
+            fills.r[2] = {d_colmin.as<uint32_t>(), (unsigned long long)n_pad * 2 * QM_SEEDS, 0xffffffffu};
+            fills.r[3] = {d_seed_a.as<uint32_t>(), n_seed_words, 0xffffffffu};
+            fills.r[4] = {d_seed_b.as<uint32_t>(), n_seed_words, 0xffffffffu};
+            fills.r[5] = {d_seed_n.as<uint32_t>(), 2, 0u};
+            rowmin = d_rowmin.as<unsigned long long>();
+            colmin = d_colmin.as<unsigned long long>();
+        }
+    }
+    hipLaunchKernelGGL(k_qm_fills, dim3(1024), dim3(256), 0, ls, fills);
+    ISO_HIP_CHECK(hipGetLastError());
     std::vector<unsigned long long> &off = lb_off_host;
     std::vector<uint32_t> &rlen = lb_len_host;
     off.assign(nq, 0);
@@ -86,46 +121,40 @@
     while (tiles.size() % 256) tiles.push_back(make_uint2(0xffffffffu, 0xffffffffu));
     if (tiles.size() > 0x7fffffffull) return ISOCON_OK;
     bclk.lap("bounds: tile table (host)");
-    d_lb.pool = d_lbrow.pool = d_lblen.pool = &st->pool;
-    d_lb.slot = SLOT_NN_LB; d_lbrow.slot = SLOT_NN_LBROW; d_lblen.slot = SLOT_NN_LBLEN;
+    d_lb.pool = &st->pool;
+    d_lb.slot = SLOT_NN_LB;
     int rc;
-    if ((rc = d_lb.alloc((size_t)total + 16)) ||
-        (rc = d_lbrow.alloc((size_t)nq * 8)) || (rc = d_lblen.alloc((size_t)nq * 4)))
-        return ISOCON_OK;
-    d_lbt.pool = d_offT.pool = d_sloT.pool = d_lenT.pool = d_score.pool = &st->pool;
-    d_lbt.slot = SLOT_NN_LBT; d_offT.slot = SLOT_NN_LBT_OFF; d_sloT.slot = SLOT_NN_LBT_SLO; d_lenT.slot = SLOT_NN_LBT_LEN; d_score.slot = SLOT_NN_SCORE;
+    if ((rc = d_lb.alloc((size_t)total + 16))) return ISOCON_OK;
+    d_lbt.pool = d_offT.pool = d_sloT.pool = d_lenT.pool = &st->pool;
+    d_lbt.slot = SLOT_NN_LBT; d_offT.slot = SLOT_NN_LBT_OFF; d_sloT.slot = SLOT_NN_LBT_SLO; d_lenT.slot = SLOT_NN_LBT_LEN;
     DevBuf d_padT(&st->pool, SLOT_NN_LBT_PAD);
-    if (d_lbt.alloc((size_t)totalT + 16) || d_offT.alloc(((size_t)n + 1) * 8) || d_sloT.alloc((size_t)n * 4) || d_lenT.alloc((size_t)n * 4) || d_score.alloc((size_t)n * 4) ||
+    if (d_lbt.alloc((size_t)totalT + 16) || d_offT.alloc(((size_t)n + 1) * 8) || d_sloT.alloc((size_t)n * 4) || d_lenT.alloc((size_t)n * 4) ||
         d_padT.alloc((size_t)n * 4))
         return ISOCON_OK;
-    ISO_HIP_CHECK(hipMemsetAsync(d_score.p, 0, (size_t)n * 4, 0));
     d_chunks.pool = &st->pool;
     d_chunks.slot = SLOT_NN_LBCHUNKS;
-    if (d_chunks.alloc(tiles.size() * sizeof(uint2))) return ISOCON_OK;
     const size_t b_tiles = (tiles.size() * sizeof(uint2) + 15) & ~(size_t)15, b_off = ((size_t)nq * 8 + 15) & ~(size_t)15, b_len = (size_t)nq * 4;
+    if (d_chunks.alloc(b_tiles + b_off + b_len)) return ISOCON_OK;
+    unsigned long long *const d_lbrow = reinterpret_cast<unsigned long long *>(d_chunks.as<char>() + b_tiles);
+    uint32_t *const d_lblen = reinterpret_cast<uint32_t *>(d_chunks.as<char>() + b_tiles + b_off);
     char *pin = nullptr;
-    if (side) { g_side.settle(); pin = static_cast<char *>(g_side.pinned.get(b_tiles + b_off + b_len)); }
+    if (side) pin = static_cast<char *>(g_side.pinned.get(b_tiles + b_off + b_len));
     if (pin) {
         memcpy(pin, tiles.data(), tiles.size() * sizeof(uint2));
         memcpy(pin + b_tiles, off.data(), (size_t)nq * 8);
         memcpy(pin + b_tiles + b_off, rlen.data(), (size_t)nq * 4);
-        g_side.in_flight = true;
-        ISO_HIP_CHECK(hipStreamWaitEvent(g_side.stream, g_side.before, 0));
-        ISO_HIP_CHECK(hipMemcpyAsync(d_chunks.p, pin, tiles.size() * sizeof(uint2), hipMemcpyHostToDevice, g_side.stream));
-        ISO_HIP_CHECK(hipMemcpyAsync(d_lbrow.p, pin + b_tiles, (size_t)nq * 8, hipMemcpyHostToDevice, g_side.stream));
-        ISO_HIP_CHECK(hipMemcpyAsync(d_lblen.p, pin + b_tiles + b_off, (size_t)nq * 4, hipMemcpyHostToDevice, g_side.stream));
-        ISO_HIP_CHECK(hipEventRecord(g_side.done, g_side.stream));
-        ISO_HIP_CHECK(hipStreamWaitEvent(0, g_side.done, 0));
+        ISO_HIP_CHECK(hipMemcpyAsync(d_chunks.p, pin, b_tiles + b_off + b_len, hipMemcpyHostToDevice, ls));
     } else {
         ISO_HIP_CHECK(copy_h2d(d_chunks.p, tiles.data(), tiles.size() * sizeof(uint2)));
-        ISO_HIP_CHECK(copy_h2d(d_lbrow.p, off.data(), (size_t)nq * 8));
-        ISO_HIP_CHECK(copy_h2d(d_lblen.p, rlen.data(), (size_t)nq * 4));
-    }
-    hipLaunchKernelGGL(k_lbt_rows, dim3((n + 255) / 256), dim3(256), 0, 0, Q, nq, d_lblen.as<uint32_t>(), n, d_sloT.as<uint32_t>(), d_lenT.as<uint32_t>(), d_padT.as<uint32_t>());
-    if ((rc = device_exscan<0, unsigned long long>(&st->pool, d_padT.as<uint32_t>(), n, d_offT.as<unsigned long long>()))) return ISOCON_OK;
-    hipLaunchKernelGGL(k_lbt_offsets, dim3((n + 255) / 256), dim3(256), 0, 0, n, d_sloT.as<uint32_t>(), d_offT.as<unsigned long long>());
-    ISO_HIP_CHECK(hipGetLastError());
-    bclk.lap("bounds: alloc + uploads");
+        ISO_HIP_CHECK(copy_h2d(d_lbrow, off.data(), (size_t)nq * 8));
+        ISO_HIP_CHECK(copy_h2d(d_lblen, rlen.data(), (size_t)nq * 4));
+    }
+    hipLaunchKernelGGL(k_lbt_rows, dim3((n + 255) / 256), dim3(256), 0, ls, Q, nq, d_lblen, n, d_sloT.as<uint32_t>(), d_lenT.as<uint32_t>(), d_padT.as<uint32_t>());
+    if ((rc = device_exscan<0, unsigned long long>(&st->pool, d_padT.as<uint32_t>(), n, d_offT.as<unsigned long long>(), ls))) return ISOCON_OK;
+    hipLaunchKernelGGL(k_lbt_offsets, dim3((n + 255) / 256), dim3(256), 0, ls, n, d_sloT.as<uint32_t>(), d_offT.as<unsigned long long>());
+    ISO_HIP_CHECK(hipGetLastError());
+    if (ls) ISO_HIP_CHECK(hipEventRecord(g_side.done, ls));
+    bclk.lap("bounds: alloc + uploads + row layout (enqueued)");
     if (use_slot_order(nq)) {
         std::vector<uint32_t> order(nq);
         std::iota(order.begin(), order.end(), 0u);
@@ -135,26 +164,19 @@
         if (d_order.alloc((size_t)nq * 4)) return ISOCON_OK;
         ISO_HIP_CHECK(copy_h2d(d_order.p, order.data(), (size_t)nq * 4));
     }
-    unsigned long long *rowmin = nullptr, *colmin = nullptr;
-    if (want_seeds) {
-        d_rowmin.pool = d_colmin.pool = d_seed_a.pool = d_seed_b.pool = &st->pool;
-        d_rowmin.slot = SLOT_NN_ROWMIN; d_colmin.slot = SLOT_NN_COLMIN; d_seed_a.slot = SLOT_NN_SEED_A; d_seed_b.slot = SLOT_NN_SEED_B;
-        if (!(d_rowmin.alloc((size_t)nq * 8 * QM_SEEDS) || d_colmin.alloc((size_t)n_pad * 8 * QM_SEEDS) || d_seed_a.alloc((size_t)n * 8 * QM_SEEDS) || d_seed_b.alloc((size_t)n * 8 * QM_SEEDS))) {
-            ISO_HIP_CHECK(hipMemsetAsync(d_rowmin.p, 0xff, (size_t)nq * 8 * QM_SEEDS, 0));
-            ISO_HIP_CHECK(hipMemsetAsync(d_colmin.p, 0xff, (size_t)n_pad * 8 * QM_SEEDS, 0));
-            rowmin = d_rowmin.as<unsigned long long>();
-            colmin = d_colmin.as<unsigned long long>();
-        }
-    }
-    bclk.lap("bounds: slot order + seed buffers");
+    bclk.lap("bounds: slot order");
     static bool lds_attr_set = false;
     if (!lds_attr_set) {
         ISO_HIP_CHECK(hipFuncSetAttribute((const void *)k_qgram_mm, hipFuncAttributeMaxDynamicSharedMemorySize, (int)QM_LDS_BYTES));
         lds_attr_set = true;
     }
+    if (ls) {
+        ISO_HIP_CHECK(hipStreamWaitEvent(0, g_side.done, 0));
+        side_guard.armed = false;
+    }
     tm.mark();
     hipLaunchKernelGGL(k_qgram_mm, dim3((unsigned)tiles.size()), dim3(512), QM_LDS_BYTES, 0, d_qprof.as<uint8_t>(), d_qsum.as<uint32_t>(), n, n_pad,
-                       d_chunks.as<uint2>(), d_lbrow.as<unsigned long long>(), d_lblen.as<uint32_t>(), d_lb.as<uint8_t>(), Q, nq,
+                       d_chunks.as<uint2>(), d_lbrow, d_lblen, d_lb.as<uint8_t>(), Q, nq,
                        d_qf.as<uint8_t>(), d_tf.as<uint8_t>(), rowmin, colmin, d_offT.as<unsigned long long>(), d_sloT.as<uint32_t>(), d_lenT.as<uint32_t>(),
                        d_lbt.as<uint8_t>(), d_score.as<uint32_t>());
     ISO_HIP_CHECK(hipGetLastError());
@@ -182,13 +204,16 @@
 #endif
     for (const uint2 &t : tiles) stats.bound_tiles += t.x != 0xffffffffu;
     P.lb = d_lb.as<uint8_t>();
-    P.lb_row = d_lbrow.as<unsigned long long>();
+    P.lb_row = lb_row_dev = d_lbrow;
+    lb_len_dev = d_lblen;
     if (use_slot_order(nq)) P.slot_order = d_order.as<uint32_t>();
     seeds_ready = rowmin != nullptr;
     seed_nq = nq;
     lb_total = total;
     st->pool.bound_tag.valid = true;
     st->pool.bound_tag.lb_total = total;
+    st->pool.bound_tag.lb_row = d_lbrow;
+    st->pool.bound_tag.lb_len = d_lblen;
     st->pool.bound_tag.has_order = use_slot_order(nq);
     st->pool.bound_tag.serial = st->serial;
     st->pool.bound_tag.map = Q; st->pool.bound_tag.depth = depth; st->pool.bound_tag.kcap = kcap;
@@ -204,12 +229,6 @@
     uint32_t col_classes = QM_SEEDS;
     while (col_classes > 1 && col_classes * ranks > (uint32_t)QM_SEEDS) col_classes >>= 1;
     if (const char *e = variant_value("nn_seed_classes")) { const int v = atoi(e); if (v == 1 || v == 2 || v == QM_SEEDS) col_classes = (uint32_t)v; }
-    DevBuf d_seed_n(&st->pool, SLOT_NN_SEED_N);
-    int rc;
-    if ((rc = d_seed_n.alloc(8))) return rc;
-    ISO_HIP_CHECK(hipMemsetAsync(d_seed_n.p, 0, 8, 0));
-    ISO_HIP_CHECK(hipMemsetAsync(d_seed_a.p, 0xff, (size_t)np * 4, 0));
-    ISO_HIP_CHECK(hipMemsetAsync(d_seed_b.p, 0xff, (size_t)np * 4, 0));
     hipLaunchKernelGGL(k_qgram_seed_pairs, dim3((n + 255) / 256), dim3(256), 0, 0, d_rowmin.as<unsigned long long>(), d_colmin.as<unsigned long long>(),
                        n, Q, seed_nq, col_classes, d_seed_a.as<uint32_t>(), d_seed_b.as<uint32_t>(), d_seed_n.as<unsigned long long>());
     ISO_HIP_CHECK(hipGetLastError());
diff --git a/isocon_amd/csrc/nn_context.inc b/isocon_amd/csrc/nn_context.inc
--- a/isocon_amd/csrc/nn_context.inc
+++ b/isocon_amd/csrc/nn_context.inc
@@ -26,11 +26,13 @@
     DevBuf d_text;
     uint32_t text_stride = 0;
     bool text_ready = false;
-    DevBuf d_qprof, d_qsum, d_lb, d_lbrow, d_lblen;
+    DevBuf d_qprof, d_qsum, d_lb;
     DevBuf d_chunks;
+    const unsigned long long *lb_row_dev = nullptr;
+    const uint32_t *lb_len_dev = nullptr;
     DevBuf d_lbt, d_offT, d_sloT, d_lenT, d_score;
     DevBuf d_order;
-    DevBuf d_rowmin, d_colmin, d_seed_a, d_seed_b;
+    DevBuf d_rowmin, d_colmin, d_seed_a, d_seed_b, d_seed_n;
     uint64_t hits_cap = 0;
     std::vector<int32_t> best;
     std::vector<int32_t> hits;
@@ -75,15 +77,22 @@
     DevBuf d_text2;
     uint32_t text2_stride = 0;
     bool text2_ready = false;
-    bool ensure_text2()
-    {
-        if (text2_ready) return true;
+    bool filter_wanted() const { return !variant("nn_no_block_filter") && !variant("nn_no_list") && st->maxlen < 16384; }
+    bool text2_room()
+    {
+        if (d_text2.p) return true;
         text2_stride = nnf_text2_stride(st->maxlen);
         size_t free_b = 0;
         if (!free_mem(free_b) || (size_t)n * text2_stride * 4 > free_b / 2 + st->pool.slots[SLOT_NN_TEXT2].cap) return false;
         d_text2.pool = &st->pool;
         d_text2.slot = SLOT_NN_TEXT2;
-        if (d_text2.alloc((size_t)std::max<uint32_t>(n, 1) * text2_stride * 4) != ISOCON_OK) return false;
+        if (d_text2.alloc((size_t)std::max<uint32_t>(n, 1) * text2_stride * 4) != ISOCON_OK) { d_text2.p = nullptr; return false; }
+        return true;
+    }
+    bool ensure_text2()
+    {
+        if (text2_ready) return true;
+        if (!text2_room()) return false;
         hipLaunchKernelGGL(k_build_text2, dim3(std::max<uint32_t>(n, 1)), dim3(256), 0, 0, st->dev, d_text2.as<uint32_t>(), text2_stride);
         if (hipGetLastError() != hipSuccess) return false;
         text2_ready = true;
@@ -154,6 +163,19 @@
         ISO_HIP_CHECK(hipMemsetAsync(d_stats.p, 0, N_COUNTERS * 8, 0));
         return ISOCON_OK;
     }
+    int begin_pass()
+    {
+        if (flags_deferred && fill_best && n) {
+            flags_deferred = fill_best = false;
+            hipLaunchKernelGGL(k_nn_step_init, dim3((std::max<uint32_t>(n, N_COUNTERS) + 255) / 256), dim3(256), 0, 0, d_best.as<int32_t>(), d_qf.as<uint8_t>(), d_tf.as<uint8_t>(), n,
+                               (int32_t)NN_INF, d_hit_count.as<unsigned long long>(), d_stats.as<unsigned long long>(), N_COUNTERS);
+            ISO_HIP_CHECK(hipGetLastError());
+            return ISOCON_OK;
+        }
+        int rc;
+        if ((rc = flush_flags()) || (rc = upload_best())) return rc;
+        return reset_counters();
+    }
     void add_counters(const unsigned long long *sc2)
     {
         for (int blk = 0; blk < 2; ++blk) {
@@ -245,10 +267,21 @@
     bool dev_excluded(uint32_t q) const { return mask_exc && is_exc(q); }
     bool flags_dirty = false;
     bool roles_uniform = false;
+    bool defer_flags = false, flags_deferred = false;
+    int flush_flags()
+    {
+        if (!flags_deferred) return ISOCON_OK;
+        flags_deferred = false;
+        ISO_HIP_CHECK(hipMemsetAsync(d_qf.p, 1, n, 0));
+        ISO_HIP_CHECK(hipMemsetAsync(d_tf.p, 1, n, 0));
+        return ISOCON_OK;
+    }
     int upload_flags(bool fresh = false)
     {
         if (!n) return ISOCON_OK;
+        flags_deferred = false;
         if (fresh && roles_uniform && !st->n_exc) {
+            if (defer_flags) { flags_deferred = true; return ISOCON_OK; }
             ISO_HIP_CHECK(hipMemsetAsync(d_qf.p, 1, n, 0));
             ISO_HIP_CHECK(hipMemsetAsync(d_tf.p, 1, n, 0));
             return ISOCON_OK;
diff --git a/isocon_amd/csrc/nn_entry.inc b/isocon_amd/csrc/nn_entry.inc
--- a/isocon_amd/csrc/nn_entry.inc
+++ b/isocon_amd/csrc/nn_entry.inc
@@ -218,11 +218,12 @@
                    ~Total() { if (getenv("ISOCON_DEBUG")) fprintf(stderr, "[isocon] %-28s %8.2f ms\n", "isocon_nn_graph total", std::chrono::duration<double, std::milli>(std::chrono::steady_clock::now() - t).count()); } } total;
     WaitScope waits(s);
     NNContext C;
+    C.defer_flags = true;
     int rc = nn_setup(C, s, is_converged, is_target, depth, nullptr, true);
     if (rc) return rc;
     clk0.lap("setup");
     if (getenv("ISOCON_DEBUG")) { (void)hipDeviceSynchronize(); clk0.lap("sync after setup"); }
-    if (C.two_set && (C.depth_binds || variant("nn_2set_walk"))) return nn2_depth_graph(C, depth, out_best, out_row_ptr, out_cols, cols_cap, n_cols_needed, stats);
+    if (C.two_set && (C.depth_binds || variant("nn_2set_walk"))) return (rc = C.flush_flags()) ? rc : nn2_depth_graph(C, depth, out_best, out_row_ptr, out_cols, cols_cap, n_cols_needed, stats);
     C.keep_dev = n >= 1024 && !variant("nn_host_finalize");
     C.csr_follows = C.keep_dev;
     C.fill_best = !s->n_exc;
diff --git a/isocon_amd/csrc/nn_filter.hpp b/isocon_amd/csrc/nn_filter.hpp
--- a/isocon_amd/csrc/nn_filter.hpp
+++ b/isocon_amd/csrc/nn_filter.hpp
@@ -22,31 +22,13 @@
     return ((dw + NNF_BATCH - 1) / NNF_BATCH + 1u) * NNF_BATCH + 4u;
 }
 
-__device__ __forceinline__ uint32_t nnf_spread16(uint32_t x)
-{
-    x = (x | (x << 8)) & 0x00ff00ffu;
-    x = (x | (x << 4)) & 0x0f0f0f0fu;
-    x = (x | (x << 2)) & 0x33333333u;
-    x = (x | (x << 1)) & 0x55555555u;
-    return x;
-}
-
 __global__ __launch_bounds__(256) void k_build_text2(DevStore S, uint32_t *__restrict__ text, uint32_t stride)
 {
     const uint32_t i = blockIdx.x;
     if (i >= S.n) return;
     const int32_t len = S.lens[i];
     uint32_t *row = text + (size_t)i * stride;
-    for (uint32_t j = threadIdx.x; j < stride; j += 256) {
-        uint32_t v = 0;
-        const int32_t c0 = (int32_t)j * 16;
-        if (c0 < len) {
-            const size_t at = ((size_t)(c0 >> 6) * S.n + i) * 2;
-            const uint32_t lo = (uint32_t)(S.planes[at] >> (c0 & 63)) & 0xffffu, hi = (uint32_t)(S.planes[at + 1] >> (c0 & 63)) & 0xffffu;
-            v = nnf_spread16(lo) | (nnf_spread16(hi) << 1);
-        }
-        row[j] = v;
-    }
+    for (uint32_t j = threadIdx.x; j < stride; j += 256) row[j] = text2_word(S, i, len, j);
 }
 
 __device__ __forceinline__ unsigned long long nnf_uniform64(unsigned long long v)
diff --git a/isocon_amd/csrc/nn_finalize.hpp b/isocon_amd/csrc/nn_finalize.hpp
--- a/isocon_amd/csrc/nn_finalize.hpp
+++ b/isocon_amd/csrc/nn_finalize.hpp
@@ -73,6 +73,15 @@
     if (best_out != nullptr && i < n) best_out[i] = best[i];
 }
 
+__global__ __launch_bounds__(256) void k_nn_step_init(int32_t *__restrict__ best, uint8_t *__restrict__ qflag, uint8_t *__restrict__ tflag, uint32_t n, int32_t inf,
+                                                       unsigned long long *__restrict__ hit_count, unsigned long long *__restrict__ stats, uint32_t n_stats)
+{
+    const uint32_t i = blockIdx.x * 256u + threadIdx.x;
+    if (i < n) { best[i] = inf; qflag[i] = 1; tflag[i] = 1; }
+    if (i < n_stats) stats[i] = 0;
+    if (i == 0) *hit_count = 0;
+}
+
 __global__ __launch_bounds__(256) void k_nn_step_record(const unsigned long long *__restrict__ hit_count, const unsigned long long *__restrict__ stats, uint32_t n_stats,
                                                          const int32_t *__restrict__ best, const uint8_t *__restrict__ qflag, const int32_t *__restrict__ lens,
                                                          uint32_t n, unsigned long long *__restrict__ rec)
diff --git a/isocon_amd/csrc/nn_lists.inc b/isocon_amd/csrc/nn_lists.inc
--- a/isocon_amd/csrc/nn_lists.inc
+++ b/isocon_amd/csrc/nn_lists.inc
@@ -31,7 +31,7 @@
     L.sorted_b = L.sorted_a + cap_out;
     ISO_HIP_CHECK(hipMemsetAsync(d_ltot.p, 0, sizeof(NNPlanTotals), 0));
     NNBoundRows B;
-    B.lb = PR.lb; B.row_off = PR.lb_row; B.row_len = static_cast<const uint32_t *>(st->pool.slots[SLOT_NN_LBLEN].p);
+    B.lb = PR.lb; B.row_off = PR.lb_row; B.row_len = lb_len_dev;
     B.lbT = static_cast<const uint8_t *>(st->pool.slots[SLOT_NN_LBT].p);
     B.offT = static_cast<const unsigned long long *>(st->pool.slots[SLOT_NN_LBT_OFF].p);
     B.sloT = static_cast<const uint32_t *>(st->pool.slots[SLOT_NN_LBT_SLO].p);
diff --git a/isocon_amd/csrc/nn_main.inc b/isocon_amd/csrc/nn_main.inc
--- a/isocon_amd/csrc/nn_main.inc
+++ b/isocon_amd/csrc/nn_main.inc
@@ -332,7 +332,7 @@
     const bool whole_set = Q.begin == 0 && Q.end == n && Q.stride == 1 && Q.block_log2 == 0 && C.depth >= n;
     for (;;) {
         int rc;
-        if ((rc = C.upload_best()) || (rc = C.reset_counters())) return rc;
+        if ((rc = C.begin_pass())) return rc;
         clk.lap("phaseA: upload/reset");
         PhaseAPass P(do_seed, do_main, seeded_before);
         if (!C.two_set || two_set_lists) {
diff --git a/isocon_amd/csrc/qgram_mm.hpp b/isocon_amd/csrc/qgram_mm.hpp
--- a/isocon_amd/csrc/qgram_mm.hpp
+++ b/isocon_amd/csrc/qgram_mm.hpp
@@ -55,9 +55,14 @@
     return y << 1;
 }
 
-static constexpr int QP_SEQS = 4;
-
-__global__ __launch_bounds__(256) void k_qgram_profile4(DevStore S, uint8_t *__restrict__ prof4, uint32_t *__restrict__ psum, uint32_t n_pad)
+#ifndef ISOCON_QP_SEQS
+#define ISOCON_QP_SEQS 4
+#endif
+static constexpr int QP_SEQS = ISOCON_QP_SEQS;
+static_assert(QP_SEQS >= 1 && QP_SEQS <= 16 && (QP_SEQS & (QP_SEQS - 1)) == 0, "QP_SEQS x (2 KB of bitsets) + the excess counters stay below 64 KB of LDS");
+
+__global__ __launch_bounds__(256) void k_qgram_profile4(DevStore S, uint8_t *__restrict__ prof4, uint32_t *__restrict__ psum, uint32_t n_pad,
+                                                        uint32_t *__restrict__ text2, uint32_t text2_stride)
 {
     __shared__ uint32_t bits[QP_SEQS][QM_K / 32];
     __shared__ uint32_t exh[QG_B1];
@@ -70,8 +75,13 @@
     for (uint32_t r = 0; r < cnt; ++r) {
         const uint32_t i = i0 + r;
         for (int e = threadIdx.x; e < QG_B1; e += 256) exh[e] = 0;
+        const int32_t len = S.lens[i];
+        if (text2) {
+            uint32_t *row = text2 + (size_t)i * text2_stride;
+            for (uint32_t j = threadIdx.x; j < text2_stride; j += 256) row[j] = text2_word(S, i, len, j);
+        }
         __syncthreads();
-        const int32_t ngrams = S.lens[i] - QG_Q + 1;
+        const int32_t ngrams = len - QG_Q + 1;
         for (int32_t j = threadIdx.x; j < ngrams; j += 256) {
             const int32_t c = j >> 6, o = j & 63;
             const size_t at = ((size_t)c * S.n + i) * 2;
@@ -101,22 +111,20 @@
         }
         __syncthreads();
     }
-    uint32_t local[QP_SEQS];
-#pragma unroll
-    for (int r = 0; r < QP_SEQS; ++r) local[r] = 0;
+    static_assert(256 % (QP_SEQS * QM_SLOTS) == 0, "a thread's elements of the write loop share their sequence");
+    const int r = (threadIdx.x / QM_SLOTS) % QP_SEQS, sl = threadIdx.x % QM_SLOTS;
+    uint32_t local = 0;
     for (int e = threadIdx.x; e < QP_SEQS * (QM_K / 32); e += 256) {
-        const int kb = e / (QP_SEQS * QM_SLOTS), r = (e / QM_SLOTS) % QP_SEQS, sl = e % QM_SLOTS;
+        const int kb = e / (QP_SEQS * QM_SLOTS);
         const uint32_t w = bits[r][kb * QM_SLOTS + sl];
-#pragma unroll
-        for (int rr = 0; rr < QP_SEQS; ++rr) local[rr] += rr == r ? (uint32_t)__popc(w) : 0u;
+        local += (uint32_t)__popc(w);
         if ((uint32_t)r < cnt) {
             uint4 o;
             o.x = qg_spread8(w & 0xffu); o.y = qg_spread8((w >> 8) & 0xffu); o.z = qg_spread8((w >> 16) & 0xffu); o.w = qg_spread8(w >> 24);
             *reinterpret_cast<uint4 *>(prof4 + ((size_t)kb * n_pad + i0 + (uint32_t)r) * QM_ROWB + (size_t)sl * 16) = o;
         }
     }
-#pragma unroll
-    for (int r = 0; r < QP_SEQS; ++r) if (local[r]) atomicAdd(&s_sum[r], local[r]);
+    if (local) atomicAdd(&s_sum[r], local);
     __syncthreads();
     if (threadIdx.x < cnt) psum[i0 + threadIdx.x] = s_sum[threadIdx.x];
 }
@@ -500,6 +508,16 @@
 #endif
 }
 
+struct QMFillRange { uint32_t *p; unsigned long long words; uint32_t value; };
+struct QMFills { QMFillRange r[6]; };
+__global__ __launch_bounds__(256) void k_qm_fills(QMFills F)
+{
+    const unsigned long long first = (unsigned long long)blockIdx.x * 256u + threadIdx.x, step = (unsigned long long)gridDim.x * 256u;
+#pragma unroll
+    for (int k = 0; k < 6; ++k)
+        for (unsigned long long i = first; i < F.r[k].words; i += step) F.r[k].p[i] = F.r[k].value;
+}
+
 __global__ __launch_bounds__(256) void k_lbt_rows(QMap Q, uint32_t nq, const uint32_t *__restrict__ row_len, uint32_t n, uint32_t *__restrict__ sloT,
                                                    uint32_t *__restrict__ lenT, uint32_t *__restrict__ padT)
 {
```

Result: faster. 79.84 billion alignments/s (median of 6 runs) (+1.5%).
